# xmengli/H-DenseUNet

Hardware: AMD Instinct MI355X
Metric: CT slices/sec fwd+bwd (2D 512^2) (higher is better)
Workload: dtype bf16

## Files before the change

h-denseunet_amd/csrc/rowops.hip:

```cpp
#include "hdu_host.h"

enum { RED_STATS = 0, RED_BNBWD = 1, RED_COLSUM = 2 };
enum { ROW_UNROLL = 4 };

struct FinK {
  int kind;
  const float* shift_f32;
  const float* gamma; const float* beta; const float* sgamma; const float* sbeta;
  float eps, momentum, invM;
  int batch_stats;
  float* a; float* b; float* rstd; float* mov_mean; float* mov_var;
  const float* rstd_in;
  float* k1; float* k2; float* k3; float* dgamma; float* dbeta; float* dsgamma; float* dsbeta;
  const float* mean_in; float* corr3; float* corr4;
  int skip_lo, skip_hi;
};

__device__ __forceinline__ void fin_reduce32(double& a1, double& a2, double (*red)[4][8]) {
  const int cl = threadIdx.x & 7, wave = threadIdx.x >> 6;
#pragma unroll
  for (int mask = 8; mask < 64; mask <<= 1) {
    a1 += __shfl_xor(a1, mask);
    a2 += __shfl_xor(a2, mask);
  }
// ... 37 lines not shown
  const float sg = sgamma ? sgamma[c] : 1.f;
  const float sb = sbeta ? sbeta[c] : 0.f;
  const float inv = g * r;
  *a = sg * inv;
  *b = sg * (be - mu * inv) + sb;
  *r_out = r;
}

__device__ __forceinline__ void bn_fold_channel(int c, float mu, float v, const float* gamma, const float* beta,
                                                float eps, const float* sgamma, const float* sbeta, float* a, float* b,
                                                float* rstd, float* mov_mean, float* mov_var, float momentum) {
  float ac, bc, r;
  bn_fold_coef(c, mu, v, gamma, beta, eps, sgamma, sbeta, &ac, &bc, &r);
  a[c] = ac;
  b[c] = bc;
  if (rstd) rstd[c] = r;
  if (mov_mean) mov_mean[c] -= (mov_mean[c] - mu) * (1.f - momentum);
  if (mov_var) mov_var[c] -= (mov_var[c] - v) * (1.f - momentum);
}

__device__ __forceinline__ void bn_coef_channel(int c, float invM, int batch_stats, float S1, float S2,
                                                const float* gamma, const float* beta, const float* sgamma,
                                                const float* rstd, float* k1, float* k2, float* k3, float* dgamma,
                                                float* dbeta, float* dsgamma, float* dsbeta) {
  const float g = gamma ? gamma[c] : 1.f;
  const float be = beta ? beta[c] : 0.f;
  const float sg = sgamma ? sgamma[c] : 1.f;
  const float r = rstd[c];
  const float kk = sg * g * r;
  k1[c] = kk;
  k2[c] = batch_stats ? kk * S1 * invM : 0.f;
  k3[c] = batch_stats ? kk * r * S2 * invM : 0.f;
  if (dgamma) dgamma[c] = sg * S2;
  if (dbeta) dbeta[c] = sg * S1;
  if (dsgamma) dsgamma[c] = g * S2 + be * S1;
  if (dsbeta) dsbeta[c] = S1;
}

template <typename T, int MODE>
__device__ __forceinline__ void finalize_channel(int c, double a1, double a2, long long M, const void* x, float* o1,
                                                 float* o2, const FinK& fin, const FinPre& pre) {
  if (MODE == 0) {
    const double shift = fin.shift_f32 ? (double)fin.shift_f32[c] : (double)Chunk<T>::load1((const T*)x + c);
    const double m1 = a1 / (double)M;
    double var = a2 / (double)M - m1 * m1;
    if (var < 0.0) var = 0.0;
    o1[c] = (float)(shift + m1);
    o2[c] = (float)var;
    if (fin.kind == 1) bn_fold_channel_pre(c, (float)(shift + m1), (float)var, fin, pre);
  } else {
    if (o1) o1[c] = (float)a1;
    if (o2) o2[c] = (float)a2;
    if (MODE == 1 && (fin.kind == 2 || fin.kind == 3)) {
      const float S1 = (float)a1, S2 = (float)a2;
      const float kk = pre.sg * pre.g * pre.rs;
      const float k2 = fin.batch_stats ? kk * S1 * fin.invM : 0.f;
      const float k3 = fin.batch_stats ? kk * pre.rs * S2 * fin.invM : 0.f;
      if (fin.dgamma) fin.dgamma[c] = pre.sg * S2;
      if (fin.dbeta) fin.dbeta[c] = pre.sg * S1;
      if (fin.dsgamma) fin.dsgamma[c] = pre.g * S2 + pre.be * S1;
      if (fin.dsbeta) fin.dsbeta[c] = S1;
      if (fin.kind == 2) {
        fin.k1[c] = kk; fin.k2[c] = k2; fin.k3[c] = k3;
      } else if (fin.batch_stats && !(c >= fin.skip_lo && c < fin.skip_hi)) {
        fin.corr3[c] += k3;
        fin.corr4[c] += k3 * pre.mu - k2;
      }
    }
  }
}

struct RedK {
  const void* x;
  const void* dz;
  long long ldx, lddz, M, rows_per_block;
  int C;
  int relu;
  const float* a;
  const float* b;
  const float* mean;
  const float* rstd;
  float* partial;
  int slots;
};

template <typename T, int MODE, int COLS>
__global__ __launch_bounds__(256) void reduce_rows_kernel(RedK p) {
  constexpr int CH = Chunk<T>::CH;
  constexpr int ROWS = 256 / COLS;
  __shared__ float red[2][ROWS][COLS * CH];
  const int tid = threadIdx.x;
  const int cc = tid % COLS;
  const int rl = tid / COLS;
  const int c0 = (blockIdx.y * COLS + cc) * CH;
  const bool active = c0 < p.C;
  const T* __restrict__ xp = (const T*)p.x;
  const T* __restrict__ dzp = (const T*)p.dz;

  float s1[CH], s2[CH], k0[CH], k1[CH], k2[CH], k3[CH];
#pragma unroll
  for (int j = 0; j < CH; ++j) { s1[j] = 0.f; s2[j] = 0.f; k0[j] = 0.f; k1[j] = 0.f; k2[j] = 0.f; k3[j] = 0.f; }
  if (active) {
    if (MODE == RED_STATS) {
      Chunk<T>::unpack(*(const u32x4*)(xp + c0), k0);
    } else if (MODE == RED_BNBWD) {
#pragma unroll
      for (int j = 0; j < CH; ++j) {
        k0[j] = p.a[c0 + j]; k1[j] = p.b[c0 + j]; k2[j] = p.mean[c0 + j]; k3[j] = p.rstd[c0 + j];
      }
    }
    const long long r_begin = (long long)blockIdx.x * p.rows_per_block;
    long long r_end = r_begin + p.rows_per_block;
    if (r_end > p.M) r_end = p.M;
    auto body = [&](const u32x4& xv, const u32x4& gv) {
      float f[CH];
      Chunk<T>::unpack(xv, f);
      if (MODE == RED_STATS) {
#pragma unroll
        for (int j = 0; j < CH; ++j) { const float d = f[j] - k0[j]; s1[j] += d; s2[j] += d * d; }
      } else if (MODE == RED_BNBWD) {
        float g[CH];
        Chunk<T>::unpack(gv, g);
#pragma unroll
        for (int j = 0; j < CH; ++j) {
          const float s = k0[j] * f[j] + k1[j];
          const float gg = (!p.relu || s > 0.f) ? g[j] : 0.f;
          s1[j] += gg;
          s2[j] += gg * ((f[j] - k2[j]) * k3[j]);
        }
      } else {
#pragma unroll
        for (int j = 0; j < CH; ++j) s1[j] += f[j];
      }
    };
    long long r = r_begin + rl;
    for (; r + (ROW_UNROLL - 1) * ROWS < r_end; r += ROW_UNROLL * ROWS) {
      u32x4 xv[ROW_UNROLL], gv[ROW_UNROLL];
#pragma unroll
      for (int u = 0; u < ROW_UNROLL; ++u) xv[u] = *(const u32x4*)(xp + (r + u * ROWS) * p.ldx + c0);
      if (MODE == RED_BNBWD) {
#pragma unroll
        for (int u = 0; u < ROW_UNROLL; ++u) gv[u] = *(const u32x4*)(dzp + (r + u * ROWS) * p.lddz + c0);
      }
      HDU_SCHED_BARRIER();
#pragma unroll
      for (int u = 0; u < ROW_UNROLL; ++u) body(xv[u], gv[u]);
    }
    for (; r < r_end; r += ROWS) {
      u32x4 gv = u32x4{0u, 0u, 0u, 0u};
      if (MODE == RED_BNBWD) gv = *(const u32x4*)(dzp + r * p.lddz + c0);
      body(*(const u32x4*)(xp + r * p.ldx + c0), gv);
    }
  }
#pragma unroll
  for (int j = 0; j < CH; ++j) { red[0][rl][cc * CH + j] = s1[j]; red[1][rl][cc * CH + j] = s2[j]; }
  __syncthreads();
  for (int q = tid; q < 2 * COLS * CH; q += 256) {
    const int s = q / (COLS * CH);
    const int col = q % (COLS * CH);
    const int c = blockIdx.y * COLS * CH + col;
    if (c < p.C) {
      float t = 0.f;
#pragma unroll 4
      for (int r = 0; r < ROWS; ++r) t += red[s][r][col];
      if (p.slots > 0) atomicAdd(p.partial + ((long long)(blockIdx.x % (unsigned)p.slots) * 2 + s) * p.C + c, t);
      else p.partial[((long long)blockIdx.x * 2 + s) * p.C + c] = t;
    }
  }
}

template <typename T, int MODE>
__global__ __launch_bounds__(256) void reduce_finalize_kernel(const float* __restrict__ partial, int nblk, int C,
                                                              long long M, const void* x, float* __restrict__ o1,
                                                              float* __restrict__ o2, FinK fin) {
  __shared__ double red[2][4][8];
  const int cl = threadIdx.x & 7, pl = threadIdx.x >> 3;
  const int c = blockIdx.x * 8 + cl;
  const FinPre pre = fin_prefetch(fin, c < C ? c : 0, pl == 0 && c < C && fin.kind != 0);
  double a1 = 0.0, a2 = 0.0;
  if (c < C) {
    int b = pl;
    for (; b + 7 * 32 < nblk; b += 8 * 32) {
      float v1[8], v2[8];
#pragma unroll
      for (int u = 0; u < 8; ++u) {
        v1[u] = partial[((long long)(b + u * 32) * 2 + 0) * C + c];
        v2[u] = MODE != RED_COLSUM ? partial[((long long)(b + u * 32) * 2 + 1) * C + c] : 0.f;
      }
      HDU_SCHED_BARRIER();
#pragma unroll
      for (int u = 0; u < 8; ++u) { a1 += (double)v1[u]; a2 += (double)v2[u]; }
    }
    for (; b < nblk; b += 32) {
      a1 += (double)partial[((long long)b * 2 + 0) * C + c];
      if (MODE != RED_COLSUM) a2 += (double)partial[((long long)b * 2 + 1) * C + c];
    }
  }
  fin_reduce32(a1, a2, red);
  if (pl == 0 && c < C) finalize_channel<T, MODE>(c, a1, a2, M, x, o1, o2, fin, pre);
}

static int red_cols_for(int nchunks) {
  int cols = 4;
  while (cols < nchunks && cols < 32) cols <<= 1;
  return cols;
}
static void red_geometry(int dtype, long long M, int C, int* cols, unsigned* gx, unsigned* gy, long long* rpb) {
  const int ch = dtype == HDU_BF16 ? 8 : 4;
  const int nchunks = (C + ch - 1) / ch;
  *cols = red_cols_for(nchunks);
  *gy = (unsigned)((nchunks + *cols - 1) / *cols);
  const int rows = 256 / *cols;
  long long want = (g_tuning[HDU_TUNE_RED_WGS] > 0 ? g_tuning[HDU_TUNE_RED_WGS] : 512) / *gy;
  if (want < 1) want = 1;
  long long maxb = (M + (long long)rows * 4 - 1) / ((long long)rows * 4);
  if (maxb < 1) maxb = 1;
  if (want > maxb) want = maxb;
  *rpb = (M + want - 1) / want;
  if (*rpb < 1) *rpb = 1;
  *gx = (unsigned)((M + *rpb - 1) / *rpb);
  if (*gx < 1) *gx = 1;
}

extern "C" size_t hdu_reduce_ws_bytes(int64_t M, int C) {
  size_t best = 0;
  for (int dt = 0; dt < 2; ++dt) {
    int cols; unsigned gx, gy; long long rpb;
    red_geometry(dt, M, C, &cols, &gx, &gy, &rpb);
    size_t b = (size_t)gx * 2 * (size_t)C * sizeof(float);
    if (b > best) best = b;
  }
  return best + 256;
}

template <typename T, int MODE>
static int run_reduce(RedK k, int cols, unsigned gx, unsigned gy, hipStream_t s) {
  switch (cols) {
    case 4: HDU_LAUNCH((reduce_rows_kernel<T, MODE, 4>), dim3(gx, gy), dim3(256), 0, s, k); break;
    case 8: HDU_LAUNCH((reduce_rows_kernel<T, MODE, 8>), dim3(gx, gy), dim3(256), 0, s, k); break;
    case 16: HDU_LAUNCH((reduce_rows_kernel<T, MODE, 16>), dim3(gx, gy), dim3(256), 0, s, k); break;
    default: HDU_LAUNCH((reduce_rows_kernel<T, MODE, 32>), dim3(gx, gy), dim3(256), 0, s, k); break;
  }
  return 0;
}

template <int MODE>
static int reduce_entry(int dtype, RedK k, float* o1, float* o2, void* ws, size_t ws_bytes, hipStream_t s,
                        const char* what, FinK fin = FinK{}) {
  if (dtype != HDU_BF16 && dtype != HDU_F32) return hdu_set_error(HDU_ERR_ARG, "reduce: bad dtype");
  const int ch = dtype == HDU_BF16 ? 8 : 4;
  if (k.C <= 0 || k.C % ch || k.ldx % ch || (k.dz && k.lddz % ch))
    return hdu_set_error(HDU_ERR_ARG, "reduce: C and pixel strides must be multiples of the 16-byte chunk");
  if (k.M <= 0) return hdu_set_error(HDU_ERR_ARG, "reduce: M must be positive");
  int cols; unsigned gx, gy; long long rpb;
  red_geometry(dtype, k.M, k.C, &cols, &gx, &gy, &rpb);
  if (!ws || ws_bytes < (size_t)gx * 2 * (size_t)k.C * sizeof(float))
    return hdu_set_error(HDU_ERR_WORKSPACE, "reduce: workspace too small (see hdu_reduce_ws_bytes)");
  k.rows_per_block = rpb;
  k.partial = (float*)ws;
  const unsigned fb = (unsigned)((k.C + 7) / 8);
  if (dtype == HDU_BF16) {
    run_reduce<bf16_t, MODE>(k, cols, gx, gy, s);
    HDU_LAUNCH((reduce_finalize_kernel<bf16_t, MODE>), dim3(fb), dim3(256), 0, s, (const float*)ws, (int)gx, k.C,
               k.M, k.x, o1, o2, fin);
  } else {
    run_reduce<float, MODE>(k, cols, gx, gy, s);
    HDU_LAUNCH((reduce_finalize_kernel<float, MODE>), dim3(fb), dim3(256), 0, s, (const float*)ws, (int)gx, k.C, k.M,
               k.x, o1, o2, fin);
  }
  return hdu_check_launch(what);
}

extern "C" int hdu_bn_stats(int dtype, const void* x, int64_t ldx, int64_t M, int C, float* mean, float* var,
                            void* ws, size_t ws_bytes, void* stream) {
  if (!x || !mean || !var) return hdu_set_error(HDU_ERR_ARG, "bn_stats: null pointer");
  RedK k{};
  k.x = x; k.ldx = ldx; k.M = M; k.C = C;
  return reduce_entry<RED_STATS>(dtype, k, mean, var, ws, ws_bytes, (hipStream_t)stream, "bn_stats");
}

extern "C" int hdu_bn_stats_fold(int dtype, const void* x, int64_t ldx, int64_t M, int C, float* mean, float* var,
                                 const float* gamma, const float* beta, float eps, const float* sgamma,
                                 const float* sbeta, float* a, float* b, float* rstd, float* mov_mean, float* mov_var,
                                 float momentum, void* ws, size_t ws_bytes, void* stream) {
  if (!x || !mean || !var || !a || !b) return hdu_set_error(HDU_ERR_ARG, "bn_stats_fold: null pointer");
  RedK k{};
  k.x = x; k.ldx = ldx; k.M = M; k.C = C;
  FinK f{};
  f.kind = 1; f.gamma = gamma; f.beta = beta; f.sgamma = sgamma; f.sbeta = sbeta; f.eps = eps; f.momentum = momentum;
  f.a = a; f.b = b; f.rstd = rstd; f.mov_mean = mov_mean; f.mov_var = mov_var;
  return reduce_entry<RED_STATS>(dtype, k, mean, var, ws, ws_bytes, (hipStream_t)stream, "bn_stats_fold", f);
}

extern "C" int hdu_bn_stats_finalize(const float* partial, int slots, int64_t M, int C, const float* shift, float* mean,
                                     float* var, const float* gamma, const float* beta, float eps, const float* sgamma,
                                     const float* sbeta, float* a, float* b, float* rstd, float* mov_mean, float* mov_var,
                                     float momentum, void* stream) {
  if (!partial || slots <= 0 || M <= 0 || C <= 0 || !shift || !mean || !var || ((a == nullptr) != (b == nullptr)))
    return hdu_set_error(HDU_ERR_ARG, "bn_stats_finalize: bad args");
  FinK f{};
  f.shift_f32 = shift;
  if (a) {
    f.kind = 1; f.gamma = gamma; f.beta = beta; f.sgamma = sgamma; f.sbeta = sbeta; f.eps = eps; f.momentum = momentum;
    f.a = a; f.b = b; f.rstd = rstd; f.mov_mean = mov_mean; f.mov_var = mov_var;
  }
  HDU_LAUNCH((reduce_finalize_kernel<float, RED_STATS>), dim3((unsigned)((C + 7) / 8)), dim3(256), 0, (hipStream_t)stream,
             partial, slots, C, (long long)M, (const void*)nullptr, mean, var, f);
  return hdu_check_launch("bn_stats_finalize");
}

__global__ __launch_bounds__(256) void finalize_fold_next_kernel(const float* __restrict__ partial, int slots, int Cseg,
                                                                 int seg_c0, int C_all, long long M,
                                                                 const float* __restrict__ shift_all,
                                                                 float* __restrict__ mean_all, float* __restrict__ var_all,
                                                                 FinK fin) {
  __shared__ double red[2][4][8];
  const int cl = threadIdx.x & 7, pl = threadIdx.x >> 3;
  const int c = blockIdx.x * 8 + cl;
  const bool in_seg = c >= seg_c0 && c < seg_c0 + Cseg;
  const bool wg_has_seg = (int)blockIdx.x * 8 + 7 >= seg_c0 && (int)blockIdx.x * 8 < seg_c0 + Cseg;
  const bool mine = pl == 0 && c < C_all;
  const FinPre pre = fin_prefetch(fin, mine ? c : 0, mine);
  const float mean_old = mine ? (in_seg ? shift_all[c] : mean_all[c]) : 0.f;
  const float var_old = mine ? var_all[c] : 0.f;
// ... 88 lines not shown
                          size_t ws_bytes, void* stream) {
  if (!x || !out) return hdu_set_error(HDU_ERR_ARG, "colsum: null pointer");
  RedK k{};
  k.x = x; k.ldx = ldx; k.M = M; k.C = C;
  return reduce_entry<RED_COLSUM>(dtype, k, out, nullptr, ws, ws_bytes, (hipStream_t)stream, "colsum");
}

__global__ __launch_bounds__(256) void bn_fold_kernel(int C, const float* mean, const float* var, const float* gamma,
                                                      const float* beta, float eps, const float* sgamma,
                                                      const float* sbeta, float* a, float* b, float* rstd,
                                                      float* mov_mean, float* mov_var, float momentum) {
  const int c = blockIdx.x * blockDim.x + threadIdx.x;
  if (c >= C) return;
  bn_fold_channel(c, mean[c], var[c], gamma, beta, eps, sgamma, sbeta, a, b, rstd, mov_mean, mov_var, momentum);
}

extern "C" int hdu_bn_fold(int C, const float* mean, const float* var, const float* gamma, const float* beta,
                           float eps, const float* sgamma, const float* sbeta, float* a, float* b, float* rstd,
                           float* mov_mean, float* mov_var, float momentum, void* stream) {
  if (C <= 0 || !mean || !var || !a || !b) return hdu_set_error(HDU_ERR_ARG, "bn_fold: bad args");
  HDU_LAUNCH(bn_fold_kernel, dim3((unsigned)((C + 255) / 256)), dim3(256), 0, (hipStream_t)stream, C, mean, var,
             gamma, beta, eps, sgamma, sbeta, a, b, rstd, mov_mean, mov_var, momentum);
  return hdu_check_launch("bn_fold");
}

__global__ __launch_bounds__(256) void bn_fold_batched_kernel(const hdu_fold_entry* __restrict__ table,
                                                              const unsigned* __restrict__ begins, int n) {
  int lo = 0, hi = n - 1;
  while (lo < hi) {
    const int mid = (lo + hi + 1) >> 1;
    if (begins[mid] <= blockIdx.x) lo = mid; else hi = mid - 1;
  }
  const hdu_fold_entry e = table[lo];
  const int c = (int)(blockIdx.x - begins[lo]) * 256 + (int)threadIdx.x;
  if (c >= e.C) return;
  bn_fold_channel(c, e.mean[c], e.var[c], e.gamma, e.beta, e.eps, e.sgamma, e.sbeta, e.a, e.b, e.rstd, nullptr, nullptr,
                  0.f);
}

extern "C" int hdu_bn_fold_batched(const hdu_fold_entry* table, const uint32_t* begins, int n, uint32_t total_blocks,
                                   void* stream) {
  if (!table || !begins || n <= 0 || total_blocks == 0) return hdu_set_error(HDU_ERR_ARG, "bn_fold_batched: bad args");
  HDU_LAUNCH(bn_fold_batched_kernel, dim3(total_blocks), dim3(256), 0, (hipStream_t)stream, table, begins, n);
  return hdu_check_launch("bn_fold_batched");
}

__global__ __launch_bounds__(256) void bn_bwd_finalize_batched_kernel(const hdu_bnbwd_entry* __restrict__ table,
                                                                      const unsigned* __restrict__ begins, int n) {
  __shared__ double red[2][4][8];
  int lo = 0, hi = n - 1;
  while (lo < hi) {
    const int mid = (lo + hi + 1) >> 1;
    if (begins[mid] <= blockIdx.x) lo = mid; else hi = mid - 1;
  }
  const hdu_bnbwd_entry e = table[lo];
  const int cl = threadIdx.x & 7, pl = threadIdx.x >> 3;
  const int c = (int)(blockIdx.x - begins[lo]) * 8 + cl;
  const bool mine = pl == 0 && c < e.C;
  const float g = (mine && e.gamma) ? e.gamma[c] : 1.f, be = (mine && e.beta) ? e.beta[c] : 0.f;
  const float sg = (mine && e.sgamma) ? e.sgamma[c] : 1.f;
  double a1 = 0.0, a2 = 0.0;
  if (c < e.C) {
    for (int b = pl; b < e.slots; b += 32) {
      a1 += (double)e.partial[((long long)b * 2 + 0) * e.C + c];
      a2 += (double)e.partial[((long long)b * 2 + 1) * e.C + c];
    }
  }
  fin_reduce32(a1, a2, red);
  if (!mine) return;
  const float S1 = (float)a1, S2 = (float)a2;
  if (e.dgamma) e.dgamma[c] = sg * S2;
  if (e.dbeta) e.dbeta[c] = sg * S1;
  if (e.dsgamma) e.dsgamma[c] = g * S2 + be * S1;
  if (e.dsbeta) e.dsbeta[c] = S1;
}

extern "C" int hdu_bn_bwd_finalize_batched(const hdu_bnbwd_entry* table, const uint32_t* begins, int n, uint32_t total_blocks,
                                           void* stream) {
  if (!table || !begins || n <= 0 || total_blocks == 0) return hdu_set_error(HDU_ERR_ARG, "bn_bwd_finalize_batched: bad args");
  HDU_LAUNCH(bn_bwd_finalize_batched_kernel, dim3(total_blocks), dim3(256), 0, (hipStream_t)stream, table, begins, n);
  return hdu_check_launch("bn_bwd_finalize_batched");
}

__global__ __launch_bounds__(256) void bn_bwd_coef_kernel(int C, float invM, int batch_stats, const float* s1,
                                                          const float* s2, const float* gamma, const float* beta,
                                                          const float* sgamma, const float* rstd, float* k1,
                                                          float* k2, float* k3, float* dgamma, float* dbeta,
                                                          float* dsgamma, float* dsbeta) {
  const int c = blockIdx.x * blockDim.x + threadIdx.x;
  if (c >= C) return;
  bn_coef_channel(c, invM, batch_stats, s1 ? s1[c] : 0.f, s2 ? s2[c] : 0.f, gamma, beta, sgamma, rstd, k1, k2, k3,
                  dgamma, dbeta, dsgamma, dsbeta);
}

extern "C" int hdu_bn_bwd_coef(int C, int64_t M, int batch_stats, const float* s1, const float* s2,
                               const float* gamma, const float* beta, const float* sgamma, const float* rstd,
                               float* k1, float* k2, float* k3, float* dgamma, float* dbeta, float* dsgamma,
                               float* dsbeta, void* stream) {
  if (C <= 0 || M <= 0 || !rstd || !k1 || !k2 || !k3) return hdu_set_error(HDU_ERR_ARG, "bn_bwd_coef: bad args");
  if (batch_stats && (!s1 || !s2)) return hdu_set_error(HDU_ERR_ARG, "bn_bwd_coef: batch_stats needs s1/s2");
  HDU_LAUNCH(bn_bwd_coef_kernel, dim3((unsigned)((C + 255) / 256)), dim3(256), 0, (hipStream_t)stream, C,
             1.0f / (float)M, batch_stats, s1, s2, gamma, beta, sgamma, rstd, k1, k2, k3, dgamma, dbeta, dsgamma,
             dsbeta);
  return hdu_check_launch("bn_bwd_coef");
}

__global__ __launch_bounds__(256) void stats_pack_kernel(int C, const float* mean, const float* var, float n_local, int rank,
                                                         int world, float* buf) {
  const int c = blockIdx.x * blockDim.x + threadIdx.x;
  const int SL = 1 + 2 * C;
  if (c >= C) return;
  for (int r = 0; r < world; ++r) {
    const bool mine = r == rank;
    if (c == 0) buf[r * SL] = mine ? n_local : 0.f;
    buf[r * SL + 1 + c] = mine ? mean[c] : 0.f;
    buf[r * SL + 1 + C + c] = mine ? var[c] : 0.f;
  }
}
__global__ __launch_bounds__(256) void stats_unpack_kernel(int C, const float* buf, int world, float* mean, float* var) {
  const int c = blockIdx.x * blockDim.x + threadIdx.x;
  const int SL = 1 + 2 * C;
  if (c >= C) return;
  float N = 0.f, m = 0.f;
  for (int r = 0; r < world; ++r) { N += buf[r * SL]; m += buf[r * SL] * buf[r * SL + 1 + c]; }
  m /= N;
  float v = 0.f;
  for (int r = 0; r < world; ++r) {
    const float d = buf[r * SL + 1 + c] - m;
    v += buf[r * SL] * (buf[r * SL + 1 + C + c] + d * d);
  }
  mean[c] = m;
  var[c] = v / N;
}
extern "C" size_t hdu_stats_sync_floats(int C, int world) { return (size_t)world * (1 + 2 * (size_t)C); }
extern "C" int hdu_stats_pack(int C, const float* mean, const float* var, int64_t n_local, int rank, int world, float* buf,
                              void* stream) {
  if (C <= 0 || !mean || !var || !buf || n_local <= 0 || world <= 0 || rank < 0 || rank >= world)
    return hdu_set_error(HDU_ERR_ARG, "stats_pack: bad args");
  HDU_LAUNCH(stats_pack_kernel, dim3((unsigned)((C + 255) / 256)), dim3(256), 0, (hipStream_t)stream, C, mean, var,
             (float)n_local, rank, world, buf);
  return hdu_check_launch("stats_pack");
}
extern "C" int hdu_stats_unpack(int C, const float* buf, int world, float* mean, float* var, void* stream) {
  if (C <= 0 || !mean || !var || !buf || world <= 0) return hdu_set_error(HDU_ERR_ARG, "stats_unpack: bad args");
  HDU_LAUNCH(stats_unpack_kernel, dim3((unsigned)((C + 255) / 256)), dim3(256), 0, (hipStream_t)stream, C, buf, world, mean,
             var);
  return hdu_check_launch("stats_unpack");
}

struct RowK {
  const void* x;
  const void* dz;
  void* out;
  long long ldx, lddz, ldo, M, rows_per_block;
  int C;
  int relu, accumulate;
  const float* a;
  const float* b;
  const float* mean;
  const float* k1;
  const float* k2;
  const float* k3;
  float drop_scale;
  unsigned drop_thresh, drop_seed;
  const unsigned* drop_seed_dev;
  const float* sums;
  int slots, batch_stats;
  float invM;
  const float* gamma; const float* beta; const float* sgamma; const float* rstd;
  float* dgamma; float* dbeta; float* dsgamma; float* dsbeta;
};

template <int CH, int COLS>
__device__ __forceinline__ void slot_loads(const float* __restrict__ tbl, int slots, int C, int c0, bool active, int rl,
                                           float (&t1)[CH], float (&t2)[CH]) {
  constexpr int ROWS = 256 / COLS;
  constexpr int IT = 4;
  f32x4 v1[IT][CH / 4], v2[IT][CH / 4];
#pragma unroll
  for (int it = 0; it < IT; ++it) {
    const int sl = rl + it * ROWS;
    const long long row = (active && sl < slots) ? sl : 0;
#pragma unroll
    for (int j = 0; j < CH; j += 4) {
      v1[it][j / 4] = *(const f32x4*)(tbl + (row * 2 + 0) * C + c0 + j);
      v2[it][j / 4] = *(const f32x4*)(tbl + (row * 2 + 1) * C + c0 + j);
    }
  }
#pragma unroll
  for (int j = 0; j < CH; ++j) { t1[j] = 0.f; t2[j] = 0.f; }
#pragma unroll
  for (int it = 0; it < IT; ++it) {
    const bool ok = active && rl + it * ROWS < slots;
#pragma unroll
    for (int j = 0; j < CH; ++j) {
      t1[j] += ok ? v1[it][j / 4][j % 4] : 0.f;
      t2[j] += ok ? v2[it][j / 4][j % 4] : 0.f;
    }
  }
}
template <int CH, int COLS>
__device__ __forceinline__ void slot_reduce(int slots, int cc, int rl, const float (&t1)[CH], const float (&t2)[CH],
                                            float (&s1)[CH], float (&s2)[CH]) {
  constexpr int ROWS = 256 / COLS;
  __shared__ float red[ROWS][2][COLS * CH];
#pragma unroll
  for (int j = 0; j < CH; ++j) { red[rl][0][cc * CH + j] = t1[j]; red[rl][1][cc * CH + j] = t2[j]; }
  HDU_RAW_BARRIER();
  const int nr = slots < ROWS ? slots : ROWS;
#pragma unroll
  for (int j = 0; j < CH; ++j) { s1[j] = 0.f; s2[j] = 0.f; }
  for (int r = 0; r < nr; ++r) {
#pragma unroll
    for (int j = 0; j < CH; ++j) { s1[j] += red[r][0][cc * CH + j]; s2[j] += red[r][1][cc * CH + j]; }
  }
}

template <typename T, int COLS>
__global__ __launch_bounds__(256) void affine_act_kernel(RowK p) {
  constexpr int CH = Chunk<T>::CH;
  constexpr int ROWS = 256 / COLS;
  const int cc = threadIdx.x % COLS, rl = threadIdx.x / COLS;
  const int c0 = (blockIdx.y * COLS + cc) * CH;
  if (c0 >= p.C) return;
  const T* __restrict__ xp = (const T*)p.x;
  T* __restrict__ op = (T*)p.out;
  float a[CH], b[CH];
#pragma unroll
  for (int j = 0; j < CH; ++j) { a[j] = p.a ? p.a[c0 + j] : 1.f; b[j] = p.a ? p.b[c0 + j] : 0.f; }
  const long long r_begin = (long long)blockIdx.x * p.rows_per_block;
  long long r_end = r_begin + p.rows_per_block;
  if (r_end > p.M) r_end = p.M;
  auto body = [&](long long m, const u32x4& xv) {
    float f[CH];
    Chunk<T>::unpack(xv, f);
#pragma unroll
    for (int j = 0; j < CH; ++j) {
      float s = a[j] * f[j] + b[j];
      if (p.relu) s = s > 0.f ? s : 0.f;
      f[j] = s;
    }
    *(u32x4*)(op + m * p.ldo + c0) = Chunk<T>::pack(f);
  };
  long long m = r_begin + rl;
  for (; m + (ROW_UNROLL - 1) * ROWS < r_end; m += ROW_UNROLL * ROWS) {
    u32x4 xv[ROW_UNROLL];
#pragma unroll
    for (int u = 0; u < ROW_UNROLL; ++u) xv[u] = *(const u32x4*)(xp + (m + u * ROWS) * p.ldx + c0);
    HDU_SCHED_BARRIER();
#pragma unroll
    for (int u = 0; u < ROW_UNROLL; ++u) body(m + u * ROWS, xv[u]);
  }
  for (; m < r_end; m += ROWS) body(m, *(const u32x4*)(xp + m * p.ldx + c0));
}

template <typename T, int COLS, bool SUMS = false, bool PRE = false>
__global__ __launch_bounds__(256) void bn_bwd_apply_kernel(RowK p) {
  constexpr int CH = Chunk<T>::CH;
  constexpr int ROWS = 256 / COLS;
  const int cc = threadIdx.x % COLS, rl = threadIdx.x / COLS;
  const int c0 = (blockIdx.y * COLS + cc) * CH;
  const bool active = c0 < p.C;
  if (!SUMS && !active) return;
  const T* __restrict__ xp = (const T*)p.x;
  const T* __restrict__ dzp = (const T*)p.dz;
  T* __restrict__ op = (T*)p.out;
  const unsigned dseed = p.drop_seed + (p.drop_seed_dev ? *p.drop_seed_dev : 0u);
  const long long r_begin = (long long)blockIdx.x * p.rows_per_block;
  long long r_end = r_begin + p.rows_per_block;
  if (r_end > p.M) r_end = p.M;
  const u32x4 z4 = u32x4{0u, 0u, 0u, 0u};
  long long m = r_begin + rl;
  u32x4 pxv[PRE ? ROW_UNROLL : 1], pgv[PRE ? ROW_UNROLL : 1], pov[PRE ? ROW_UNROLL : 1];
  if constexpr (PRE) {
#pragma unroll
    for (int u = 0; u < ROW_UNROLL; ++u) {
      const long long mm = m + u * ROWS;
      const bool ok = active && mm < r_end;
      pxv[u] = ok ? *(const u32x4*)(xp + mm * p.ldx + c0) : z4;
      pgv[u] = ok ? *(const u32x4*)(dzp + mm * p.lddz + c0) : z4;
      pov[u] = (ok && p.accumulate) ? *(const u32x4*)(op + mm * p.ldo + c0) : z4;
    }
  }
  float a[CH], b[CH], k1[CH], k3[CH], k4[CH];
  if constexpr (SUMS) {
    const int cq = active ? c0 : 0;
    float g[CH], be[CH], sg[CH], rs[CH], mu[CH];
#pragma unroll
    for (int j = 0; j < CH; j += 4) {
      const f32x4 va = *(const f32x4*)(p.a + cq + j), vb = *(const f32x4*)(p.b + cq + j);
      const f32x4 vr = *(const f32x4*)(p.rstd + cq + j), vm = *(const f32x4*)(p.mean + cq + j);
      const f32x4 vg = p.gamma ? *(const f32x4*)(p.gamma + cq + j) : f32x4{1.f, 1.f, 1.f, 1.f};
      const f32x4 ve = p.beta ? *(const f32x4*)(p.beta + cq + j) : f32x4{0.f, 0.f, 0.f, 0.f};
      const f32x4 vs = p.sgamma ? *(const f32x4*)(p.sgamma + cq + j) : f32x4{1.f, 1.f, 1.f, 1.f};
#pragma unroll
      for (int r = 0; r < 4; ++r) {
        a[j + r] = va[r]; b[j + r] = vb[r]; rs[j + r] = vr[r]; mu[j + r] = vm[r];
        g[j + r] = vg[r]; be[j + r] = ve[r]; sg[j + r] = vs[r];
      }
    }
    float T1[CH], T2[CH], S1[CH], S2[CH];
    slot_loads<CH, COLS>(p.sums, p.slots, p.C, cq, active, rl, T1, T2);
    slot_reduce<CH, COLS>(p.slots, cc, rl, T1, T2, S1, S2);
    if (!active) return;
#pragma unroll
    for (int j = 0; j < CH; ++j) {
      const float kk = sg[j] * g[j] * rs[j];
      const float k2 = p.batch_stats ? kk * S1[j] * p.invM : 0.f;
      k1[j] = kk;
      k3[j] = p.batch_stats ? kk * rs[j] * S2[j] * p.invM : 0.f;
      k4[j] = k3[j] * mu[j] - k2;
    }
    if (blockIdx.x == 0 && rl == 0) {
#pragma unroll
      for (int j = 0; j < CH; ++j) {
        const int c = c0 + j;
        if (p.dgamma) p.dgamma[c] = sg[j] * S2[j];
        if (p.dbeta) p.dbeta[c] = sg[j] * S1[j];
        if (p.dsgamma) p.dsgamma[c] = g[j] * S2[j] + be[j] * S1[j];
        if (p.dsbeta) p.dsbeta[c] = S1[j];
      }
    }
  } else {
#pragma unroll
    for (int j = 0; j < CH; ++j) {
      const int c = c0 + j;
      a[j] = p.a[c]; b[j] = p.b[c]; k1[j] = p.k1[c]; k3[j] = p.k3[c];
      k4[j] = p.k3[c] * p.mean[c] - p.k2[c];
    }
  }
  auto body = [&](long long m, const u32x4& xv, const u32x4& gv, const u32x4& ov) {
    float f[CH], g[CH], o[CH];
    Chunk<T>::unpack(xv, f);
    Chunk<T>::unpack(gv, g);
#pragma unroll
    for (int j = 0; j < CH; ++j) {
      const float s = a[j] * f[j] + b[j];
      const float gg = (!p.relu || s > 0.f) ? g[j] : 0.f;
      float d = k1[j] * gg - k3[j] * f[j] + k4[j];
      if (p.drop_scale != 0.f) {
        const unsigned h = hdu_hash32((unsigned long long)m * (unsigned)p.C + (unsigned)(c0 + j), dseed);
        d = h < p.drop_thresh ? d * p.drop_scale : 0.f;
      }
      o[j] = d;
    }
    if (p.accumulate) {
      float old[CH];
      Chunk<T>::unpack(ov, old);
#pragma unroll
      for (int j = 0; j < CH; ++j) o[j] += old[j];
    }
    *(u32x4*)(op + m * p.ldo + c0) = Chunk<T>::pack(o);
  };
  if constexpr (PRE) {
#pragma unroll
    for (int u = 0; u < ROW_UNROLL; ++u)
      if (m + u * ROWS < r_end) body(m + u * ROWS, pxv[u], pgv[u], pov[u]);
    return;
  }
  for (; m + (ROW_UNROLL - 1) * ROWS < r_end; m += ROW_UNROLL * ROWS) {
    u32x4 xv[ROW_UNROLL], gv[ROW_UNROLL], ov[ROW_UNROLL];
#pragma unroll
    for (int u = 0; u < ROW_UNROLL; ++u) xv[u] = *(const u32x4*)(xp + (m + u * ROWS) * p.ldx + c0);
#pragma unroll
    for (int u = 0; u < ROW_UNROLL; ++u) gv[u] = *(const u32x4*)(dzp + (m + u * ROWS) * p.lddz + c0);
#pragma unroll
    for (int u = 0; u < ROW_UNROLL; ++u) ov[u] = p.accumulate ? *(const u32x4*)(op + (m + u * ROWS) * p.ldo + c0) : z4;
    HDU_SCHED_BARRIER();
#pragma unroll
    for (int u = 0; u < ROW_UNROLL; ++u) body(m + u * ROWS, xv[u], gv[u], ov[u]);
  }
  for (; m < r_end; m += ROWS)
    body(m, *(const u32x4*)(xp + m * p.ldx + c0), *(const u32x4*)(dzp + m * p.lddz + c0),
         p.accumulate ? *(const u32x4*)(op + m * p.ldo + c0) : z4);
}

template <typename T, int COLS>
__global__ __launch_bounds__(256) void bn_bwd_correct_kernel(RowK p) {
  constexpr int CH = Chunk<T>::CH;
  constexpr int ROWS = 256 / COLS;
  const int cc = threadIdx.x % COLS, rl = threadIdx.x / COLS;
  const int c0 = (blockIdx.y * COLS + cc) * CH;
  if (c0 >= p.C) return;
  const T* __restrict__ xp = (const T*)p.x;
  T* __restrict__ op = (T*)p.out;
  float k3[CH], k4[CH];
#pragma unroll
  for (int j = 0; j < CH; ++j) { k3[j] = p.k3[c0 + j]; k4[j] = p.k2[c0 + j]; }
  const long long r_begin = (long long)blockIdx.x * p.rows_per_block;
  long long r_end = r_begin + p.rows_per_block;
  if (r_end > p.M) r_end = p.M;
  auto body = [&](long long m, const u32x4& xv, const u32x4& ov) {
    float f[CH], o[CH];
    Chunk<T>::unpack(xv, f);
    Chunk<T>::unpack(ov, o);
#pragma unroll
    for (int j = 0; j < CH; ++j) o[j] += k4[j] - k3[j] * f[j];
    *(u32x4*)(op + m * p.ldo + c0) = Chunk<T>::pack(o);
  };
  long long m = r_begin + rl;
  for (; m + (ROW_UNROLL - 1) * ROWS < r_end; m += ROW_UNROLL * ROWS) {
    u32x4 xv[ROW_UNROLL], ov[ROW_UNROLL];
#pragma unroll
    for (int u = 0; u < ROW_UNROLL; ++u) xv[u] = *(const u32x4*)(xp + (m + u * ROWS) * p.ldx + c0);
#pragma unroll
    for (int u = 0; u < ROW_UNROLL; ++u) ov[u] = *(const u32x4*)(op + (m + u * ROWS) * p.ldo + c0);
    HDU_SCHED_BARRIER();
#pragma unroll
    for (int u = 0; u < ROW_UNROLL; ++u) body(m + u * ROWS, xv[u], ov[u]);
  }
  for (; m < r_end; m += ROWS) body(m, *(const u32x4*)(xp + m * p.ldx + c0), *(const u32x4*)(op + m * p.ldo + c0));
}

struct FinCorK {
  const float* partial; int slots; int C; long long M;
  FinK fin;
  int nfin;
  int cs0, Cc;
  const void* u; void* du; long long ldu, lddu, rows_per_block;
};

template <typename T>
__global__ __launch_bounds__(256) void bn_bwd_finalize_correct_kernel(FinCorK p) {
  constexpr int CH = Chunk<T>::CH;
  __shared__ double red[2][4][8];
  __shared__ float slotv[32][8][2 * CH];
  __shared__ float tot[8][2 * CH];
  if ((int)blockIdx.x < p.nfin) {
    if (blockIdx.y != 0) return;
    const int cl = threadIdx.x & 7, pl = threadIdx.x >> 3;
    const int c = blockIdx.x * 8 + cl;
    const FinPre pre = fin_prefetch(p.fin, c < p.C ? c : 0, pl == 0 && c < p.C);
    double a1 = 0.0, a2 = 0.0;
    if (c < p.C)
      for (int b = pl; b < p.slots; b += 32) {
        a1 += (double)p.partial[((long long)b * 2 + 0) * p.C + c];
        a2 += (double)p.partial[((long long)b * 2 + 1) * p.C + c];
      }
    fin_reduce32(a1, a2, red);
    if (pl == 0 && c < p.C) finalize_channel<float, RED_BNBWD>(c, a1, a2, p.M, nullptr, nullptr, nullptr, p.fin, pre);
    return;
  }
  const int cc = threadIdx.x & 7, rl = threadIdx.x >> 3;
  const int c0 = (blockIdx.y * 8 + cc) * CH;
  const bool active = c0 < p.Cc;
  const int cb = p.cs0 + (active ? c0 : 0);
  {
    float v[2 * CH];
#pragma unroll
    for (int j = 0; j < 2 * CH; ++j) v[j] = 0.f;
    if (active && rl < p.slots) {
#pragma unroll
      for (int j = 0; j < CH; j += 4) {
        const f32x4 q1 = *(const f32x4*)(p.partial + ((long long)rl * 2 + 0) * p.C + cb + j);
        const f32x4 q2 = *(const f32x4*)(p.partial + ((long long)rl * 2 + 1) * p.C + cb + j);
#pragma unroll
        for (int r = 0; r < 4; ++r) { v[j + r] = q1[r]; v[CH + j + r] = q2[r]; }
// ... 283 lines not shown
  const int ch = dtype == HDU_BF16 ? 8 : 4;
  if (!x || !out || ((a == nullptr) != (b == nullptr)) || ((ud | uh | uw) & ~1))
    return hdu_set_error(HDU_ERR_ARG, "materialize: bad pointers / upsample shifts");
  if (C <= 0 || C % ch || ldx % ch || ldout % ch || (skip && ldskip % ch) || N <= 0 || D <= 0 || H <= 0 || W <= 0)
    return hdu_set_error(HDU_ERR_ARG, "materialize: C / strides must be multiples of the 16-byte chunk");
  MatK k{};
  k.x = x; k.skip = skip; k.out = out; k.a = a; k.b = b; k.ldx = ldx; k.ldskip = ldskip; k.ldo = ldout;
  k.N = N; k.D = D; k.H = H; k.W = W; k.C = C; k.ud = ud; k.uh = uh; k.uw = uw; k.relu = relu;
  k.Mo = (long long)N * (D << ud) * (H << uh) * (W << uw);
  int cols; unsigned gx, gy;
  row_geometry(dtype, k.Mo, C, &cols, &gx, &gy, &k.rows_per_block);
  if (dtype == HDU_BF16) { HDU_ROW_LAUNCH(materialize_kernel, bf16_t, cols, gx, gy, stream, k); }
  else { HDU_ROW_LAUNCH(materialize_kernel, float, cols, gx, gy, stream, k); }
  return hdu_check_launch("materialize");
}

extern "C" int hdu_materialize_stats(int dtype, const void* x, int64_t ldx, int N, int D, int H, int W, int C,
                                     const hdu_stats_fold_desc* f, int relu, int ud, int uh, int uw, const void* skip,
                                     int64_t ldskip, void* out, int64_t ldout, void* stream) {
  if (dtype != HDU_BF16 && dtype != HDU_F32) return hdu_set_error(HDU_ERR_ARG, "materialize_stats: bad dtype");
  const int ch = dtype == HDU_BF16 ? 8 : 4;
  if (!x || !out || !f || ((ud | uh | uw) & ~1)) return hdu_set_error(HDU_ERR_ARG, "materialize_stats: bad pointers / upsample shifts");
  if (C <= 0 || C % ch || ldx % ch || ldout % ch || (skip && ldskip % ch) || N <= 0 || D <= 0 || H <= 0 || W <= 0)
    return hdu_set_error(HDU_ERR_ARG, "materialize_stats: C / strides must be multiples of the 16-byte chunk");
  if (!f->partial || f->slots <= 0 || f->slots > 32 || f->M <= 0 || f->Cseg <= 0 || f->Cseg % ch || f->seg_c0 < 0 ||
      f->seg_c0 % ch || f->seg_c0 + f->Cseg > C || !f->shift || !f->mean || !f->var || !f->a || !f->b)
    return hdu_set_error(HDU_ERR_ARG, "materialize_stats: bad statistics block (segment bounds are multiples of the 16-byte chunk)");
  if (((uintptr_t)f->partial | (uintptr_t)f->shift | (uintptr_t)f->mean | (uintptr_t)f->var | (uintptr_t)f->gamma |
       (uintptr_t)f->beta | (uintptr_t)f->sgamma | (uintptr_t)f->sbeta | (uintptr_t)f->mov_mean | (uintptr_t)f->mov_var) & 15)
    return hdu_set_error(HDU_ERR_ARG, "materialize_stats: per-channel vectors must be 16-byte aligned");
  MatK k{};
  k.x = x; k.skip = skip; k.out = out; k.ldx = ldx; k.ldskip = ldskip; k.ldo = ldout;
  k.N = N; k.D = D; k.H = H; k.W = W; k.C = C; k.ud = ud; k.uh = uh; k.uw = uw; k.relu = relu;
  k.Mo = (long long)N * (D << ud) * (H << uh) * (W << uw);
  k.st_partial = f->partial; k.st_slots = f->slots; k.Cseg = f->Cseg; k.seg_c0 = f->seg_c0; k.st_M = f->M;
  k.st_shift = f->shift; k.st_mean = f->mean; k.st_var = f->var;
  k.gamma = f->gamma; k.beta = f->beta; k.sgamma = f->sgamma; k.sbeta = f->sbeta; k.eps = f->eps; k.momentum = f->momentum;
  k.fa = f->a; k.fb = f->b; k.frstd = f->rstd; k.mov_mean = f->mov_mean; k.mov_var = f->mov_var;
  int cols; unsigned gx, gy;
  row_geometry(dtype, k.Mo, C, &cols, &gx, &gy, &k.rows_per_block);
  const bool pre = k.rows_per_block <= (long long)ROW_UNROLL * (256 / cols) && !(ud | uh | uw) && skip == nullptr &&
                   !(g_tuning[HDU_TUNE_DEBUG] & 2048);
#define HDU_MAT_STATS(T, PRE)                                                                                                   \
  switch (cols) {                                                                                                               \
    case 4: HDU_LAUNCH((materialize_kernel<T, 4, true, PRE>), dim3(gx, gy), dim3(256), 0, (hipStream_t)stream, k); break;       \
    case 8: HDU_LAUNCH((materialize_kernel<T, 8, true, PRE>), dim3(gx, gy), dim3(256), 0, (hipStream_t)stream, k); break;       \
    case 16: HDU_LAUNCH((materialize_kernel<T, 16, true, PRE>), dim3(gx, gy), dim3(256), 0, (hipStream_t)stream, k); break;     \
    default: HDU_LAUNCH((materialize_kernel<T, 32, true, PRE>), dim3(gx, gy), dim3(256), 0, (hipStream_t)stream, k); break;     \
  }
  if (dtype == HDU_BF16) { if (pre) { HDU_MAT_STATS(bf16_t, true) } else { HDU_MAT_STATS(bf16_t, false) } }
  else { if (pre) { HDU_MAT_STATS(float, true) } else { HDU_MAT_STATS(float, false) } }
#undef HDU_MAT_STATS
  return hdu_check_launch("materialize_stats");
}

extern "C" int hdu_bn_bwd_apply(int dtype, const void* dz, int64_t lddz, const void* x, int64_t ldx, int64_t M,
                                int C, const float* a, const float* b, int relu, const float* mean, const float* k1,
                                const float* k2, const float* k3, void* dx, int64_t lddx, int accumulate,
                                float drop_keep, uint32_t drop_seed, const uint32_t* drop_seed_dev, void* stream) {
  RowK k{};
  k.x = x; k.ldx = ldx; k.dz = dz; k.lddz = lddz; k.out = dx; k.ldo = lddx; k.M = M; k.C = C;
  k.a = a; k.b = b; k.relu = relu; k.mean = mean; k.k1 = k1; k.k2 = k2; k.k3 = k3; k.accumulate = accumulate;
  if (drop_keep > 0.f && drop_keep < 1.f) {
    k.drop_scale = 1.f / drop_keep;
    k.drop_thresh = (unsigned)((double)drop_keep * 4294967296.0);
  }
  k.drop_seed = drop_seed;
  k.drop_seed_dev = drop_seed_dev;
  if (!x || !dz || !dx || !a || !b || !mean || !k1 || !k2 || !k3) return hdu_set_error(HDU_ERR_ARG, "bn_bwd_apply: null pointer");
  if (int e = rowk_check(dtype, k, "bn_bwd_apply: C / strides must be multiples of the 16-byte chunk")) return e;
  if (M == 0) return 0;
  int cols; unsigned gx, gy;
  row_geometry(dtype, M, C, &cols, &gx, &gy, &k.rows_per_block);
  if (dtype == HDU_BF16) { HDU_ROW_LAUNCH(bn_bwd_apply_kernel, bf16_t, cols, gx, gy, stream, k); }
  else { HDU_ROW_LAUNCH(bn_bwd_apply_kernel, float, cols, gx, gy, stream, k); }
  return hdu_check_launch("bn_bwd_apply");
}

static int bn_bwd_fused_impl(bool reduce, int dtype, const void* dz, int64_t lddz, const void* x, int64_t ldx, int64_t M, int C,
                             const float* a, const float* b, int relu, const float* mean, const float* rstd,
                             int batch_stats, const float* gamma, const float* beta, const float* sgamma, float* sums,
                             int slots, float* dgamma, float* dbeta, float* dsgamma, float* dsbeta, void* dx,
                             int64_t lddx, int accumulate, float drop_keep, uint32_t drop_seed,
                             const uint32_t* drop_seed_dev, void* stream) {
  if (!dz || !x || !a || !b || !mean || !rstd || !sums || !dx) return hdu_set_error(HDU_ERR_ARG, "bn_bwd_fused: null pointer");
  if (slots <= 0 || slots > 32) return hdu_set_error(HDU_ERR_ARG, "bn_bwd_fused: 1 <= slots <= 32");
  if (((uintptr_t)sums | (uintptr_t)a | (uintptr_t)b | (uintptr_t)mean | (uintptr_t)rstd | (uintptr_t)gamma | (uintptr_t)beta |
       (uintptr_t)sgamma) & 15)
    return hdu_set_error(HDU_ERR_ARG, "bn_bwd_fused: per-channel vectors must be 16-byte aligned");
  RowK k{};
  k.x = x; k.ldx = ldx; k.dz = dz; k.lddz = lddz; k.out = dx; k.ldo = lddx; k.M = M; k.C = C;
  k.a = a; k.b = b; k.relu = relu; k.mean = mean; k.accumulate = accumulate;
  if (drop_keep > 0.f && drop_keep < 1.f) {
    k.drop_scale = 1.f / drop_keep;
    k.drop_thresh = (unsigned)((double)drop_keep * 4294967296.0);
  }
  k.drop_seed = drop_seed;
  k.drop_seed_dev = drop_seed_dev;
  k.sums = sums; k.slots = slots; k.batch_stats = batch_stats; k.invM = 1.0f / (float)M;
  k.gamma = gamma; k.beta = beta; k.sgamma = sgamma; k.rstd = rstd;
  k.dgamma = dgamma; k.dbeta = dbeta; k.dsgamma = dsgamma; k.dsbeta = dsbeta;
  if (int e = rowk_check(dtype, k, "bn_bwd_fused: C / strides must be multiples of the 16-byte chunk")) return e;
  if (M == 0) return 0;
  if (reduce) {
    RedK r{};
    r.x = x; r.ldx = ldx; r.dz = dz; r.lddz = lddz; r.M = M; r.C = C;
    r.a = a; r.b = b; r.mean = mean; r.rstd = rstd; r.relu = relu;
    r.partial = sums; r.slots = slots;
    int rcols; unsigned rgx, rgy;
    red_geometry(dtype, M, C, &rcols, &rgx, &rgy, &r.rows_per_block);
    if (dtype == HDU_BF16) run_reduce<bf16_t, RED_BNBWD>(r, rcols, rgx, rgy, (hipStream_t)stream);
    else run_reduce<float, RED_BNBWD>(r, rcols, rgx, rgy, (hipStream_t)stream);
  }
  int cols; unsigned gx, gy;
  row_geometry(dtype, M, C, &cols, &gx, &gy, &k.rows_per_block);
  const bool pre = k.rows_per_block <= (long long)ROW_UNROLL * (256 / cols) && !(g_tuning[HDU_TUNE_DEBUG] & 2048);
#define HDU_APPLY_SUMS(T, PRE)                                                                                                    \
  switch (cols) {                                                                                                                 \
    case 4: HDU_LAUNCH((bn_bwd_apply_kernel<T, 4, true, PRE>), dim3(gx, gy), dim3(256), 0, (hipStream_t)stream, k); break;        \
    case 8: HDU_LAUNCH((bn_bwd_apply_kernel<T, 8, true, PRE>), dim3(gx, gy), dim3(256), 0, (hipStream_t)stream, k); break;        \
    case 16: HDU_LAUNCH((bn_bwd_apply_kernel<T, 16, true, PRE>), dim3(gx, gy), dim3(256), 0, (hipStream_t)stream, k); break;      \
    default: HDU_LAUNCH((bn_bwd_apply_kernel<T, 32, true, PRE>), dim3(gx, gy), dim3(256), 0, (hipStream_t)stream, k); break;      \
  }
  if (dtype == HDU_BF16) { if (pre) { HDU_APPLY_SUMS(bf16_t, true) } else { HDU_APPLY_SUMS(bf16_t, false) } }
  else { if (pre) { HDU_APPLY_SUMS(float, true) } else { HDU_APPLY_SUMS(float, false) } }
#undef HDU_APPLY_SUMS
  return hdu_check_launch("bn_bwd_fused");
}

extern "C" int hdu_bn_bwd_fused(int dtype, const void* dz, int64_t lddz, const void* x, int64_t ldx, int64_t M, int C,
                                const float* a, const float* b, int relu, const float* mean, const float* rstd,
                                int batch_stats, const float* gamma, const float* beta, const float* sgamma, float* sums,
                                int slots, float* dgamma, float* dbeta, float* dsgamma, float* dsbeta, void* dx,
                                int64_t lddx, int accumulate, float drop_keep, uint32_t drop_seed,
                                const uint32_t* drop_seed_dev, void* stream) {
  return bn_bwd_fused_impl(true, dtype, dz, lddz, x, ldx, M, C, a, b, relu, mean, rstd, batch_stats, gamma, beta, sgamma, sums, slots,
                           dgamma, dbeta, dsgamma, dsbeta, dx, lddx, accumulate, drop_keep, drop_seed, drop_seed_dev, stream);
}

extern "C" int hdu_bn_bwd_apply_sums(int dtype, const void* dz, int64_t lddz, const void* x, int64_t ldx, int64_t M, int C,
                                     const float* a, const float* b, int relu, const float* mean, const float* rstd,
                                     int batch_stats, const float* gamma, const float* beta, const float* sgamma, float* sums,
                                     int slots, float* dgamma, float* dbeta, float* dsgamma, float* dsbeta, void* dx,
                                     int64_t lddx, int accumulate, float drop_keep, uint32_t drop_seed,
                                     const uint32_t* drop_seed_dev, void* stream) {
  return bn_bwd_fused_impl(false, dtype, dz, lddz, x, ldx, M, C, a, b, relu, mean, rstd, batch_stats, gamma, beta, sgamma, sums, slots,
                           dgamma, dbeta, dsgamma, dsbeta, dx, lddx, accumulate, drop_keep, drop_seed, drop_seed_dev, stream);
}

extern "C" int hdu_bn_bwd_correct(int dtype, const void* u, int64_t ldu, int64_t M, int C, const float* corr3,
                                  const float* corr4, void* du, int64_t lddu, void* stream) {
  RowK k{};
  k.x = u; k.ldx = ldu; k.out = du; k.ldo = lddu; k.M = M; k.C = C;
  k.k3 = corr3; k.k2 = corr4;
  if (!u || !du || !corr3 || !corr4) return hdu_set_error(HDU_ERR_ARG, "bn_bwd_correct: null pointer");
  if (int e = rowk_check(dtype, k, "bn_bwd_correct: C / strides must be multiples of the 16-byte chunk")) return e;
  if (M == 0) return 0;
  int cols; unsigned gx, gy;
  row_geometry(dtype, M, C, &cols, &gx, &gy, &k.rows_per_block);
  if (dtype == HDU_BF16) { HDU_ROW_LAUNCH(bn_bwd_correct_kernel, bf16_t, cols, gx, gy, stream, k); }
  else { HDU_ROW_LAUNCH(bn_bwd_correct_kernel, float, cols, gx, gy, stream, k); }
  return hdu_check_launch("bn_bwd_correct");
}

extern "C" int hdu_bn_bwd_finalize_correct(int dtype, const float* partial, int slots, int64_t M, int C, const float* gamma,
                                           const float* beta, const float* sgamma, const float* mean, const float* rstd,
                                           float* dgamma, float* dbeta, float* dsgamma, float* dsbeta, float* corr3, float* corr4,
                                           int cs0, int Cc, const void* u, int64_t ldu, void* du, int64_t lddu, void* stream) {
  const int ch = dtype == HDU_BF16 ? 8 : 4;
  if ((dtype != HDU_BF16 && dtype != HDU_F32) || !partial || slots <= 0 || slots > 32 || M <= 0 || C <= 0 || !rstd || !mean || !corr3 ||
      !corr4 || !u || !du || cs0 < 0 || Cc <= 0 || cs0 + Cc > C || cs0 % ch || Cc % ch || C % 4 || ldu % ch || lddu % ch ||
      ((uintptr_t)u | (uintptr_t)du | (uintptr_t)partial) % 16)
    return hdu_set_error(HDU_ERR_ARG, "bn_bwd_finalize_correct: bad args (corrected channels inside the BN's, chunk-aligned; <= 32 slots)");
  FinCorK k{};
  k.partial = partial; k.slots = slots; k.C = C; k.M = M;
  k.fin.kind = 3; k.fin.gamma = gamma; k.fin.beta = beta; k.fin.sgamma = sgamma; k.fin.rstd_in = rstd; k.fin.invM = 1.0f / (float)M;
  k.fin.batch_stats = 1; k.fin.dgamma = dgamma; k.fin.dbeta = dbeta; k.fin.dsgamma = dsgamma; k.fin.dsbeta = dsbeta;
  k.fin.mean_in = mean; k.fin.corr3 = corr3; k.fin.corr4 = corr4; k.fin.skip_lo = cs0; k.fin.skip_hi = cs0 + Cc;
  k.nfin = (C + 7) / 8;
  k.cs0 = cs0; k.Cc = Cc; k.u = u; k.du = du; k.ldu = ldu; k.lddu = lddu;
  const unsigned gy = (unsigned)((Cc / ch + 7) / 8);
  long long want = (g_tuning[HDU_TUNE_ROW_WGS] > 0 ? g_tuning[HDU_TUNE_ROW_WGS] : 512) / gy;
  long long maxb = (M + 127) / 128;
  if (want > maxb) want = maxb;
  if (want < 1) want = 1;
  k.rows_per_block = (M + want - 1) / want;
  const unsigned gxc = (unsigned)((M + k.rows_per_block - 1) / k.rows_per_block);
  if (dtype == HDU_BF16) HDU_LAUNCH((bn_bwd_finalize_correct_kernel<bf16_t>), dim3((unsigned)k.nfin + gxc, gy), dim3(256), 0, (hipStream_t)stream, k);
  else HDU_LAUNCH((bn_bwd_finalize_correct_kernel<float>), dim3((unsigned)k.nfin + gxc, gy), dim3(256), 0, (hipStream_t)stream, k);
  return hdu_check_launch("bn_bwd_finalize_correct");
}

struct PoolK {
  const void* x;
  const void* dy;
  void* out;
  unsigned char* idx;
  long long ldx, lddy, ldo;
  int N, D, H, W, C;
  int Do, Ho, Wo;
  int accumulate;
  int ud, uh, uw;
  int pad_d;
};

template <typename T>
__global__ __launch_bounds__(256) void maxpool_fwd_kernel(PoolK p) {
  constexpr int CH = Chunk<T>::CH;
  const int ncc = p.C / CH;
  const long long total = (long long)p.N * p.Do * p.Ho * p.Wo * ncc;
  const T* __restrict__ xp = (const T*)p.x;
  T* __restrict__ op = (T*)p.out;
  const int kdn = p.D == 1 ? 1 : 3, pdd = p.D == 1 ? 0 : p.pad_d, sdd = p.D == 1 ? 1 : 2;
  for (long long q = (long long)blockIdx.x * blockDim.x + threadIdx.x; q < total;
       q += (long long)gridDim.x * blockDim.x) {
    const int c0 = (int)(q % ncc) * CH;
    long long t = q / ncc;
    const long long opix = t;
    const int ow = (int)(t % p.Wo); t /= p.Wo;
    const int oh = (int)(t % p.Ho); t /= p.Ho;
    const int od = (int)(t % p.Do);
    const int n = (int)(t / p.Do);
    float best[CH];
    int bi[CH];
    bool any_pad = false;
#pragma unroll
    for (int j = 0; j < CH; ++j) { best[j] = -3.0e38f; bi[j] = 255; }
    for (int kd = 0; kd < kdn; ++kd) {
      const int id = od * sdd - pdd + kd;
      for (int kh = 0; kh < 3; ++kh) {
// ... 752 lines not shown
```

h-denseunet_amd/engine.py:

```python
import ctypes
import math
import os
from collections import OrderedDict

import numpy as np
import torch

from . import ops
from . import shard as _sh
from .lib import HDU_BF16, HDU_F32


class Param:
    __slots__ = ("layer", "idx", "kind", "keras_shape", "shape", "trainable", "init", "offset", "numel", "ctx", "meta")

    def __init__(self, ctx, layer, idx, kind, keras_shape, shape, trainable, init, meta=None):
        self.ctx, self.layer, self.idx, self.kind = ctx, layer, idx, kind
        self.keras_shape, self.shape, self.trainable, self.init = tuple(keras_shape), tuple(shape), trainable, init
        self.numel = int(np.prod(shape))
        self.offset = None
        self.meta = meta or {}

    @property
    def data(self):
        return self.ctx.P[self.offset:self.offset + self.numel]

    @property
    def grad(self):
        return self.ctx.G[self.offset:self.offset + self.numel]


class Var:

    def __init__(self, ctx, act, root=None, c0=0):
        self.ctx, self.act, self.c0 = ctx, act, c0
        self.root = root or self
        if root is None:
            self.grad_act = None
            self.written = False
            self.mean = None
            self.var = None
            self.shift = None
            self.needs_grad = False
            self.drop = None
            self.corr_off = None
        self.C = act.C

    def slab(self, c0, C):
        return Var(self.ctx, self.act.slab(c0, C), self.root, self.c0 + c0)

    def require_grad(self):
        r = self.root
        if not r.needs_grad:
            r.needs_grad = True
            a = r.act
            r.grad_act = ops.Act.alloc(a.N, a.D, a.H, a.W, a.ld, a.dtype, zero=True)
        return self

    @property
    def grad(self):
        return self.root.grad_act.slab(self.c0, self.C)

    def dy(self):
        r = self.root
        ctx = self.ctx
        if r.corr_off is not None and ctx.corr_acc is not None and ctx.fuse_bn_bwd_now:
            pend = ctx._pending_fin
            ch = ops.CHUNK[self.act.dtype]
            aligned = (self.c0 - (pend["c0"] if pend else 0)) % ch == 0 and self.C % ch == 0 and self.act.ld % ch == 0 \
                and self.grad.ld % ch == 0 and self.act.ptr.value % 16 == 0 and self.grad.ptr.value % 16 == 0
            if pend is not None and pend["root"] is r and pend["c0"] <= self.c0 and self.c0 + self.C <= pend["c0"] + pend["C"] \
                    and self.act.M == pend["M"] and aligned:
                ctx._pending_fin = None
                ops.bn_bwd_finalize_correct(*pend["args"], self.c0 - pend["c0"], self.act, self.grad)
                return self.grad
            ctx.flush_pending_finalize()
            ld = r.act.ld
            base = r.corr_off + self.c0
            acc = ctx.corr_acc
            ops.bn_bwd_correct(self.act, acc[base:base + self.C], acc[base + ld:base + ld + self.C], self.grad)
        return self.grad

    def grad_mode(self):
        r = self.root
        acc = r.written
        if not acc:
            assert self.c0 == 0, "first gradient write into a shared buffer must start at channel 0"
            if self.C != r.act.ld:
                self.ctx.zero_partial_grad(r.grad_act.buf)
        r.written = True
        return acc

    def stats(self):
        r = self.root
        if r.mean is None:
            dev = ops.device()
            r.mean = torch.zeros(r.act.ld, dtype=torch.float32, device=dev)
            r.var = torch.ones(r.act.ld, dtype=torch.float32, device=dev)
            r.shift = torch.zeros(r.act.ld, dtype=torch.float32, device=dev)
            r.ctx.stat_roots.append(r)
        return r.mean[self.c0:self.c0 + self.C], r.var[self.c0:self.c0 + self.C]

    def stats_shift(self):
        self.stats()
        return self.root.shift[self.c0:self.c0 + self.C]


class _BwdList(list):

    def __init__(self, ctx):
        super().__init__()
        self._ctx = ctx
        self.mark = []

    def append(self, fn):
        super().append(fn)
        self.mark.append(len(self._ctx.params))


class Ctx:

    def __init__(self, dtype, batch_shape):
        self.dtype = dtype
        self.ch = ops.CHUNK[dtype]
        self.params = []
        self.by_layer = OrderedDict()
        self.layer_kind = OrderedDict()
        self.fwd = []
        self.bwd = _BwdList(self)
        self.vars = []
        self.learning_phase = 1
        self.pass_id = 0
        self.P = self.G = self.V = None
        self.n_trainable = 0
        self.convs = []
        self.bns = []
        self._fold_plans = {}
        self._prefolded_phase = None
        self.prefolded_pass = -1
        self.batch_fold = os.environ.get("HDU_BATCH_FOLD", "1") == "1"
        self.defer_bnb_finalize = os.environ.get("HDU_DEFER_BNB_FINALIZE", "1") == "1"
        self._bnb_deferred, self._bnb_plan = [], None
        self._pending_fin = None
        self.merge_fin_correct = os.environ.get("HDU_MERGE_FIN_CORRECT", "1") == "1"
        self.absorb_stats = os.environ.get("HDU_ABSORB_STATS", "1") == "1"
        self.bn_bwd_fused = os.environ.get("HDU_BN_BWD_FUSED", "1") == "1"
        self.fuse_bn_bwd_mode = int(os.environ.get("HDU_FUSE_BN_BWD", "1"))
        self.fuse_bn_bwd = self.fuse_bn_bwd_mode > 0
        self.fuse_bn_bwd_pw = os.environ.get("HDU_FUSE_BN_BWD_PW", "1") == "1"
        self.bnb_sums_epilogue = os.environ.get("HDU_BNB_SUMS_EPILOGUE", "1") == "1"
        self.fuse_bn_bwd_now = False
        self.bnb_sinks = []
        self.bnb_acc = None
        self.corr_acc = None
        self._corr_total = 0
        self._scratch = {}
        self.ws_bytes = 1 << 16
        self.ws = None
        self.dev = ops.device()
        self.seed_dev = torch.zeros(1, dtype=torch.int32, device=self.dev)
        self.drop_layers = 0
        self.dropout_enabled = True
        self.grad_enabled = True
        self.fuse_bn_epilogue = os.environ.get("HDU_FUSE_BN_EPILOGUE", "1") == "1"
        self.fuse_bn_epilogue_train = os.environ.get("HDU_FUSE_BN_EPILOGUE_TRAIN", "1") == "1"
        self.fold_next = os.environ.get("HDU_FOLD_NEXT", "1") == "1"
        self.shard = None
        self.fuse_prologue = os.environ.get("HDU_FUSE_PROLOGUE", "0") == "1"
        self.fuse_pw = os.environ.get("HDU_FUSE_PW", "1") == "1"
        self.batch_wgrad = os.environ.get("HDU_BATCH_WGRAD", "1") == "1"
        self.wgrad_plan = None
        self.split_wgrad = os.environ.get("HDU_F32_SPLIT_WGRAD", "1") == "1"
        self._split_plan = None
        self._split_now = False
        self.epilogue_stats = os.environ.get("HDU_EPILOGUE_STATS", "1") == "1"
        self.stats_sinks = []
        self.stat_roots = []
        self.stats_acc = None
        self.finalized = False
        self.arena = None
        self.loss_layers = []
        self._grad_zero = []
        self._grad_zero_ids = set()
        self._zp_arena = self._zp_bwd = self._zp_step = None
        self._zp_keep = []
        self._zeroed_fwd_pass = -1
        self._zeroed_bwd_pass = -1
        self._zeroed_grad_pass = -1

    def add_param(self, layer, kind, idx, keras_shape, shape, trainable, init, meta=None):
        p = Param(self, layer, idx, kind, keras_shape, shape, trainable, init, meta)
        self.params.append(p)
        self.by_layer.setdefault(layer, []).append(p)
        self.layer_kind[layer] = kind
        return p

    def need_ws(self, M, C):
        self.ws_bytes = max(self.ws_bytes, ops.reduce_ws_bytes(M, C))

    def scratch(self, slot, N, D, H, W, C):
        n = N * D * H * W * C
        ent = self._scratch.setdefault(slot, {"n": 0, "buf": None})
        ent["n"] = max(ent["n"], n)
        return lambda: ops.Act(ent["buf"], 0, N, D, H, W, C, C, self.dtype)

    def new_var(self, N, D, H, W, C, ld=None):
        v = Var(self, ops.Act.alloc(N, D, H, W, C, self.dtype, ld=ld, zero=True))
        self.vars.append(v)
        return v

    def fvec(self, C, fill=0.0):
        return torch.full((C,), fill, dtype=torch.float32, device=self.dev)

    def finalize(self, seed=4321):
        order = [p for p in self.params if p.trainable] + [p for p in self.params if not p.trainable]
        off = 0
        for p in order:
            p.offset = off
            off += (p.numel + 3) // 4 * 4
            if p.trainable:
                self.n_trainable = off
        self.P = torch.zeros(off, dtype=torch.float32, device=self.dev)
        self.G = torch.zeros(off, dtype=torch.float32, device=self.dev)
        self.V = torch.zeros(max(self.n_trainable, 4), dtype=torch.float32, device=self.dev)
        self.ws = ops.Workspace(self.ws_bytes)
        tdt = torch.bfloat16 if self.dtype == HDU_BF16 else torch.float32
        for ent in self._scratch.values():
            ent["buf"] = torch.zeros(ent["n"], dtype=tdt, device=self.dev)
        tot = 0
        for cv in self.convs:
            cv.wf_off = tot
            tot += cv.kernel.numel
            if cv.need_dgrad_filter:
                cv.wd_off = tot
                tot += cv.kernel.numel
        self.Wc = torch.zeros(max(tot, 8), dtype=tdt, device=self.dev)
        self.init_weights(seed)
        n_stats = 0
        for st in self.stats_sinks:
            st.acc_off = n_stats
            n_stats += st.SLOTS * 2 * st.var.C
        n_bnb = 0
        for cv in self.convs:
            if cv.bnb_fused:
                cv.bnb_off = n_bnb
                n_bnb += cv.BNB_SLOTS * 2 * cv.bn.C
                r = cv.x.root
                if cv.bn.mode == "batch" and r.corr_off is None:
                    r.corr_off = self._corr_total
                    self._corr_total += 2 * r.act.ld
        n_bsum = 0
        bsum_off = {}
        if self.bn_bwd_fused and self.grad_enabled:
            for bn in self.bns:
                if bn.mode == "batch" or bn.any_trainable():
                    bsum_off[bn] = n_bsum
                    n_bsum += bn.BSUM_SLOTS * 2 * bn.C
        up4 = lambda n: (n + 3) // 4 * 4
        o_loss, n_loss = 0, 4 * max(1, len(self.loss_layers))
        o_stats = o_loss + n_loss
        o_bnb = o_stats + up4(n_stats)
        o_corr = o_bnb + up4(n_bnb)
        o_bsum = o_corr + up4(self._corr_total)
        total = o_bsum + up4(n_bsum)
        self.arena = torch.zeros(total, dtype=torch.float32, device=self.dev)
        for i, ll in enumerate(self.loss_layers):
            ll.loss_sum = self.arena[4 * i:4 * i + 1]
            ll.class_count = self.arena[4 * i + 1:4 * i + 4]
        self.stats_acc = self.arena[o_stats:o_stats + n_stats] if n_stats else None
        self.bnb_acc = self.arena[o_bnb:o_bnb + n_bnb] if n_bnb else None
        self.corr_acc = self.arena[o_corr:o_corr + self._corr_total] if self._corr_total else None
        for bn, o in bsum_off.items():
            bn.bsum = self.arena[o_bsum + o:o_bsum + o + bn.BSUM_SLOTS * 2 * bn.C]
        self._shift_copies = [(r.shift, r.mean) for r in self.stat_roots] if self.stats_sinks else []
        self._zp_arena = ops.ZeroPlan([self.arena], self._shift_copies)
        self._zp_bwd = ops.ZeroPlan([self.arena[o_bnb:total]]) if total > o_bnb else None
        for cv in self.convs:
            cv.bind()
        self._build_prep_table()
        self._build_wgrad_plan()
        self.finalized = True

    def _build_wgrad_plan(self):
        self.wgrad_plan = None
        for cv in self.convs:
            cv.in_plan = False
        if not (self.batch_wgrad and self.dtype == HDU_BF16 and self.grad_enabled and
                (self.shard is None or self.shard.world == 1)):
            return
        plan = ops.WgradPlan(int(os.environ.get("HDU_BATCH_WGRAD_TARGET", "0")))
        for cv in self.convs:
            if not (cv.trainable and cv.out.root.needs_grad):
                continue
            if cv.xin is not None:
                d = self.conv_desc(cv.xin.act, cv.wf_ptr, cv.out.grad, cv.K, cv.stride, cv.pad, cv.conv_up)
            elif cv.bn is None and cv.skip is None:
                d = self.conv_desc(cv.x.act, cv.wf_ptr, cv.out.grad, cv.K, cv.stride, cv.pad, cv.up)
            elif cv.pw_fused:
                d = self.conv_desc(cv.x.act, cv.wf_ptr, cv.out.grad, cv.K, cv.stride, cv.pad, cv.up, None,
                                  (cv.bn.a, cv.bn.b), cv.bn.relu)
            else:
                continue
            if ops.conv_kernel_name(d, 1) == "conv_stem_wgrad_kernel":
                continue
            plan.add(d, cv.kernel.grad)
            cv.in_plan = True
        if len(plan):
            plan.finalize()
            self.wgrad_plan = plan

    def split_wgrad_active(self):
        return bool(self.dtype == HDU_F32 and self.split_wgrad and self.batch_wgrad and self.grad_enabled and self.finalized
                    and ops._l.f32_contraction() != "exact" and (self.shard is None or self.shard.world == 1))

    def _build_split_wgrad_plan(self):
        if torch.cuda.is_available() and torch.cuda.is_current_stream_capturing():
            raise RuntimeError("the split filter-gradient plan is built by the first EAGER backward pass in a split-bf16 mode: run one "
                               "step (or call Ctx._build_split_wgrad_plan) before capturing")
        sp, plan, own = ops.Split3Plan(), ops.WgradPlan(int(os.environ.get("HDU_BATCH_WGRAD_TARGET", "0"))), []
        keep = []
        for cv in self.convs:
            cv.in_split_plan = False
            if not (cv.trainable and cv.out.root.needs_grad) or cv.halo or cv.cin_p % 8 or cv.cout_p % 8:
                continue
            if cv.xin is not None:
                src, pro, relu, up = cv.xin.act, None, False, cv.conv_up
            elif cv.bn is None and cv.skip is None:
                src, pro, relu, up = cv.x.act, None, False, cv.up
            elif cv.pw_fused:
                src, pro, relu, up = cv.x.act, (cv.bn.a, cv.bn.b), cv.bn.relu, cv.up
            else:
                continue
            g = cv.out.grad
            xs = ops.Act.alloc(3 * src.N, src.D, src.H, src.W, src.C, HDU_BF16)
            dys = ops.Act.alloc(3 * g.N, g.D, g.H, g.W, g.C, HDU_BF16)
            d16 = ops.conv_desc(xs, cv.wf_ptr, dys, cv.K, cv.stride, cv.pad, up)
            sp.add(src, ops._l.SPLIT3_OPERAND, xs, pro, relu)
            sp.add(g, ops._l.SPLIT3_GRADIENT, dys)
            if ops.conv_kernel_name(d16, 1) == "conv_stem_wgrad_kernel":
                own.append((d16, cv.kernel.grad))
            else:
                plan.add(d16, cv.kernel.grad)
            keep.append((xs, dys))
            cv.in_split_plan = True
        if len(sp):
            sp.finalize()
        if len(plan):
            plan.finalize()
        self._split_plan = (sp, plan, own, keep)

    def flush_pending_finalize(self):
        pend, self._pending_fin = self._pending_fin, None
        if pend is not None:
            (part, slots, M, C, g, be, sg, mean, rstd, dg, db, dsg, dsb, c3, c4) = pend["args"]
            ops.bn_bwd_finalize(part, slots, M, C, True, g, be, sg, mean, rstd, dg, db, dsg, dsb, c3, c4)

# ... 90 lines not shown
        if key not in self._grad_zero_ids:
            self._grad_zero_ids.add(key)
            self._grad_zero.append(buf)
            self._zp_step = None

    def prep_weights(self):
        if self._prep_n:
            ops.weight_prep_batched(self.dtype, self._prep_table, self._prep_n, self._prep_tiles, self.P, self.Wc)

    def _build_prep_table(self):
        from .lib import PrepEntry
        ents = []
        tiles = 0
        for cv in self.convs:
            wf = -1 if self.dtype == HDU_F32 else cv.wf_off
            wd = cv.wd_off if cv.need_dgrad_filter else -1
            if wf < 0 and wd < 0:
                continue
            ents.append(PrepEntry(cv.kernel.offset, wf, wd, tiles, cv.cout_p, cv.T, cv.cin_p, 0))
            tiles += cv.T * ((cv.cout_p + 63) // 64) * ((cv.cin_p + 63) // 64)
        self._prep_n = len(ents)
        self._prep_tiles = tiles
        if ents:
            arr = (PrepEntry * len(ents))(*ents)
            raw = np.frombuffer(bytes(arr), dtype=np.uint8).copy()
            self._prep_table = torch.from_numpy(raw).to(self.dev)

    def _fold_plan(self, phase):
        if phase not in self._fold_plans:
            ents = []
            for bn in self.bns:
                if bn.mode == "batch" and phase == 1:
                    continue
                ents.append((bn.C, bn.eps, bn.mm.data, bn.mv.data, bn.gamma.data, bn.beta.data,
                             bn.sg.data if bn.sg else None, bn.sb.data if bn.sb else None, bn.a, bn.b, bn.rstd))
            self._fold_plans[phase] = ops.FoldPlan(ents) if ents else None
        return self._fold_plans[phase]

    def shard_world(self):
        return self.shard.world if (self.shard is not None and self.shard.world > 1) else 1

    def conv_desc(self, *a, **k):
        return ops.conv_desc(*a, shard_world=self.shard_world(), **k)

    def prefold(self):
        self._prefolded_phase = None
        if self.batch_fold and self.finalized:
            plan = self._fold_plan(self.learning_phase)
            if plan is not None:
                plan.run()
                self._prefolded_phase = self.learning_phase

    def end_prefold(self):
        self._prefolded_phase = None

    def run_forward(self):
        self.pass_id += 1
        if self.batch_fold and self.finalized:
            plan = self._fold_plan(self.learning_phase)
            if plan is not None:
                if self._prefolded_phase != self.learning_phase:
                    plan.run()
                self.prefolded_pass = self.pass_id
        if self.learning_phase == 1 and self._zeroed_fwd_pass != self.pass_id and self.stats_acc is not None:
            self._zp_arena.run()
        for f in self.fwd:
            f()

    def bnb_fusable(self):
        return self.fuse_bn_bwd and (self.shard is None or self.shard.world == 1)

    def run_backward(self, seg=None):
        lo, hi = seg if seg is not None else (0, len(self.bwd))
        if lo == 0:
            for v in self.vars:
                v.written = False
            self.fuse_bn_bwd_now = self.bnb_fusable()
            if self._zeroed_bwd_pass != self.pass_id and self._zp_bwd is not None:
                self._zp_bwd.run()
                self._zeroed_bwd_pass = self.pass_id
        order = list(reversed(self.bwd))
        if lo == 0:
            self._bnb_deferred = []
            self._split_now = self.split_wgrad_active()
            if self._split_now and self._split_plan is None:
                self._build_split_wgrad_plan()
        split_bwd = self.dtype == HDU_F32 and ops._l.f32_split_in_backward_only()
        if split_bwd:
            ops._l.set_f32_split_now(True)
        try:
            for f in order[lo:hi]:
                f()
            self.flush_pending_finalize()
            if hi == len(self.bwd) and self._bnb_deferred:
                keys = tuple(k for k, _ in self._bnb_deferred)
                if self._bnb_plan is None or self._bnb_plan[0] != keys:
                    self._bnb_plan = (keys, ops.BnBwdPlan([e for _, e in self._bnb_deferred]))
                self._bnb_plan[1].run()
            if hi == len(self.bwd) and self.wgrad_plan is not None:
                self.wgrad_plan.run()
            if hi == len(self.bwd) and self._split_now:
                sp, plan, own, _ = self._split_plan
                sp.run()
                if len(plan):
                    plan.run()
                for d16, dw in own:
                    ops.conv_wgrad(d16, dw)
        finally:
            if split_bwd:
                ops._l.set_f32_split_now(False)

    def grad_buckets(self, fractions):
        n = len(self.bwd)
        tr = [p for p in self.params if p.trainable]
        index_of = {id(p): i for i, p in enumerate(self.params)}
        total = sum(p.numel for p in tr)
        cuts = []
        for f in sorted(fractions):
            want, done, pos, off = f * total, 0, n, self.n_trainable
            for k in range(n - 1, -1, -1):
                first = self.bwd.mark[k - 1] if k > 0 else 0
                own = [p for p in tr if first <= index_of[id(p)]]
                done = sum(p.numel for p in own)
                if done >= want:
                    pos, off = n - k, min([p.offset for p in own] + [self.n_trainable])
                    break
            if 0 < pos < n and (not cuts or pos > cuts[-1][0]):
                cuts.append((pos, off))
        out, prev_pos, prev_off = [], 0, self.n_trainable
        for pos, off in cuts:
            out.append((prev_pos, pos, off, prev_off))
            prev_pos, prev_off = pos, off
        out.append((prev_pos, n, 0, prev_off))
        return out


class BNLayer:
    BSUM_SLOTS = int(os.environ.get("HDU_BSUM_SLOTS", "16"))

    def __init__(self, ctx, name, C, eps=1e-3, momentum=0.99, mode="batch", trainable=True, scale_name=None,
                 scale_trainable=True, relu=True, scale=None):
        if scale is not None:
            scale_name, scale_trainable = scale.name, scale.trainable
        self.scale_layer = scale
        self.ctx, self.name, self.C, self.eps, self.momentum, self.mode, self.relu = ctx, name, C, eps, momentum, mode, relu
        self.trainable = trainable
        self.gamma = ctx.add_param(name, "bn", 0, (C,), (C,), trainable, "ones")
        self.beta = ctx.add_param(name, "bn", 1, (C,), (C,), trainable, "zeros")
        self.mm = ctx.add_param(name, "bn", 2, (C,), (C,), False, "zeros")
        self.mv = ctx.add_param(name, "bn", 3, (C,), (C,), False, "ones")
        self.sg = self.sb = None
        self.scale_trainable = scale_trainable
        if scale_name:
            self.sg = ctx.add_param(scale_name, "scale", 0, (C,), (C,), scale_trainable, "ones")
            self.sb = ctx.add_param(scale_name, "scale", 1, (C,), (C,), scale_trainable, "zeros")
            if scale is not None:
                scale.gamma, scale.beta = self.sg, self.sb
        v = ctx.fvec
        self.a, self.b, self.rstd = v(C), v(C), v(C)
        self.s1, self.s2, self.k1, self.k2, self.k3 = v(C), v(C), v(C), v(C), v(C)
        self.mean_used = None
        self.batch_now = False
        self.folded_pass = -1
        ctx.bns.append(self)
        self.s12 = v(2 * C)
        self.stats_src = None
        self.pending_stats = None
        self.bsum = None
        self._bsum_pass = -1

    def any_trainable(self):
        return self.trainable or (self.sg is not None and self.scale_trainable)

    def needs_stats(self):
        return self.mode == "batch"

    def fold(self, xvar):
        ctx = self.ctx
        sg = self.sg.data if self.sg else None
        sb = self.sb.data if self.sb else None
        self.batch_now = self.mode == "batch" and ctx.learning_phase == 1
        if self.batch_now and self.folded_pass == ctx.pass_id:
            return None
        if not self.batch_now and ctx.prefolded_pass == ctx.pass_id:
            self.mean_used = self.mm.data
            return None
        if self.batch_now:
            mean, var = xvar.stats()
            self.mean_used = mean
            args = (mean, var, self.gamma.data, self.beta.data, self.eps, sg, sb, self.a, self.b, self.rstd,
                    self.mm.data, self.mv.data, self.momentum)
        else:
            self.mean_used = self.mm.data
            args = (self.mm.data, self.mv.data, self.gamma.data, self.beta.data, self.eps, sg, sb, self.a, self.b,
                    self.rstd, None, None, self.momentum)
        ops.bn_fold(self.C, *args)
        return None

    def takes_epilogue_sums(self, xvar):
        ctx = self.ctx
        return bool((self.batch_now or self.any_trainable()) and not (ctx.shard is not None and ctx.shard.world > 1)
                    and self.bsum is not None and xvar.root.needs_grad and ctx._zeroed_bwd_pass == ctx.pass_id
                    and self._bsum_pass != ctx.pass_id)

    def backward(self, xvar, dz_act, sums_ready=False):
        ctx = self.ctx
        x = xvar.act
        need_sums = self.batch_now or self.any_trainable()
        tr_bn = self.trainable
        tr_sc = self.sg is not None and self.scale_trainable
        if ctx.shard is not None and ctx.shard.world > 1 and need_sums:
            ops.bn_bwd_reduce(dz_act, x, self.a, self.b, self.relu, self.mean_used, self.rstd, self.s1, self.s2, ctx.ws)
            ops.bn_bwd_coef(self.C, x.M, False, self.s1, self.s2, self.gamma.data, self.beta.data,
                            self.sg.data if self.sg else None, self.rstd, self.k1, self.k2, self.k3,
                            self.gamma.grad if tr_bn else None, self.beta.grad if tr_bn else None,
                            self.sg.grad if tr_sc else None, self.sb.grad if tr_sc else None)
            if self.batch_now:
                self.s12[:self.C].copy_(self.s1)
                self.s12[self.C:].copy_(self.s2)
                _sh.allreduce_sum(ctx.shard, self.s12)
                ops.bn_bwd_coef(self.C, x.M * ctx.shard.world, True, self.s12[:self.C], self.s12[self.C:],
                                self.gamma.data, self.beta.data, self.sg.data if self.sg else None, self.rstd, self.k1,
                                self.k2, self.k3)
        elif (need_sums and self.bsum is not None and xvar.root.needs_grad and ctx._zeroed_bwd_pass == ctx.pass_id
              and self._bsum_pass != ctx.pass_id):
            self._bsum_pass = ctx.pass_id
            acc = xvar.grad_mode()
            drop = xvar.root.drop if (ctx.dropout_enabled and ctx.learning_phase == 1) else None
            ops.bn_bwd_fused(dz_act, x, self.a, self.b, self.relu, self.mean_used, self.rstd, self.batch_now,
                             self.gamma.data, self.beta.data, self.sg.data if self.sg else None, self.bsum, self.BSUM_SLOTS,
                             self.gamma.grad if tr_bn else None, self.beta.grad if tr_bn else None,
                             self.sg.grad if tr_sc else None, self.sb.grad if tr_sc else None, xvar.grad, acc,
                             drop[0] if drop else 1.0, drop[1] if drop else 0, ctx.seed_dev if drop else None,
                             sums_ready=sums_ready)
            return
        elif need_sums:
            assert not sums_ready
            ops.bn_bwd_reduce_coef(dz_act, x, self.a, self.b, self.relu, self.mean_used, self.rstd, self.batch_now,
                                   self.gamma.data, self.beta.data, self.sg.data if self.sg else None, self.s1,
                                   self.s2, self.k1, self.k2, self.k3, self.gamma.grad if tr_bn else None,
                                   self.beta.grad if tr_bn else None, self.sg.grad if tr_sc else None,
                                   self.sb.grad if tr_sc else None, ctx.ws)
        else:
            ops.bn_bwd_coef(self.C, x.M, False, None, None, self.gamma.data, self.beta.data,
                            self.sg.data if self.sg else None, self.rstd, self.k1, self.k2, self.k3)
        if xvar.root.needs_grad:
            acc = xvar.grad_mode()
            drop = xvar.root.drop if (ctx.dropout_enabled and ctx.learning_phase == 1) else None
            ops.bn_bwd_apply(dz_act, x, self.a, self.b, self.relu, self.mean_used, self.k1, self.k2, self.k3,
                             xvar.grad, acc, drop[0] if drop else 1.0, drop[1] if drop else 0,
                             ctx.seed_dev if drop else None)


class ConvLayer:

    def __init__(self, ctx, name, x, filters, K, stride=(1, 1, 1), pad=(0, 0, 0), bn=None, up=(0, 0, 0), skip=None,
                 use_bias=True, out=None, init="glorot", trainable=True, dropout=0.0, keras_nd=2, cin_logical=None,
                 halo=0, producer=None):
        self.ctx, self.name, self.x, self.bn, self.up, self.skip = ctx, name, x, bn, up, skip
        self.K, self.stride = K, stride
        self.halo = halo
        if halo:
            assert not ctx.fuse_prologue, "halo mode materialises the conv input"
            assert skip is None or up == (0, 0, 0), "a skip add in halo mode must be at the stored resolution"
            pad = (pad[0] - (halo << up[0]), pad[1], pad[2])
        self.pad = pad
        self.trainable = trainable
        dt = ctx.dtype
        xa = x.act
        cin_p = xa.C
        cin = cin_logical or cin_p
        cout_p = ops.cpad(filters, dt)
        De, He, We = (xa.D + 2 * halo) << up[0], xa.H << up[1], xa.W << up[2]
        Do = (De + 2 * pad[0] - K[0]) // stride[0] + 1
        Ho = (He + 2 * pad[1] - K[1]) // stride[1] + 1
        Wo = (We + 2 * pad[2] - K[2]) // stride[2] + 1
        if out is None:
            out = ctx.new_var(xa.N, Do, Ho, Wo, cout_p)
        else:
            assert (out.act.N, out.act.D, out.act.H, out.act.W, out.act.C) == (xa.N, Do, Ho, Wo, cout_p)
        self.out = out
        kshape = ((K[1], K[2]) if keras_nd == 2 else (K[1], K[2], K[0])) + (cin, filters)
        self.kernel = ctx.add_param(name, "conv_kernel", 0, kshape, (cout_p, K[0], K[1], K[2], cin_p), trainable, init)
        self.bias = ctx.add_param(name, "conv_bias", 1, (filters,), (cout_p,), trainable, "zeros") if use_bias else None
        ctx.layer_kind[name] = "conv"
        self.T = K[0] * K[1] * K[2]
        self.cin_p, self.cout_p = cin_p, cout_p
        self.dropout = dropout
        if dropout > 0:
            ctx.drop_layers += 1
            self.drop_seed = 7919 * ctx.drop_layers
            out.root.drop = (1.0 - dropout, self.drop_seed)
        need_input_grad = x.root.needs_grad
        if ctx.grad_enabled:
            out.require_grad()
        self.xin = None
        self.conv_up = up
        self.pw_fused = bool(ctx.fuse_pw and bn is not None and skip is None and not halo and K == (1, 1, 1)
                             and stride == (1, 1, 1) and pad == (0, 0, 0) and up == (0, 0, 0) and cin_p <= ops.PRO_CMAX)
        if self.pw_fused:
            pass
        elif halo:
            self.xin = ctx.new_var(xa.N, xa.D + 2 * halo, xa.H, xa.W, cin_p)
            plane = xa.H * xa.W * cin_p
            self.xin_interior = ops.Act(self.xin.act.buf, halo * plane, xa.N, xa.D, xa.H, xa.W, cin_p, cin_p, dt)
            self._halo_tmp = ctx.scratch("halo_tmp", 1, 2 * halo, xa.H, xa.W, cin_p)
        elif (bn is not None or skip is not None) and not ctx.fuse_prologue:
            if skip is not None:
                self.xin = ctx.new_var(xa.N, De, He, We, cin_p)
                self.conv_up = (0, 0, 0)
            else:
                self.xin = ctx.new_var(xa.N, xa.D, xa.H, xa.W, cin_p)
        st = getattr(bn, "stats_src", None) if bn is not None else None
        if (st is not None and self.xin is not None and not halo and st.producer is not None and st.absorber is None
                and x.root is st.var.root and bn.C == x.C and x.c0 == (0 if bn is st.fold_next else st.var.c0)):
            st.absorber = self
        self.need_input_grad = need_input_grad
        self.epi_consumer = None
        self.epi_producer = None
        if (producer is not None and ctx.fuse_bn_epilogue and bn is not None and self.xin is not None and not halo
                and skip is None and up == (0, 0, 0) and x is producer.out and x.root is x and producer.epi_consumer is None):
            self.epi_producer = producer
            producer.epi_consumer = self
        self.strided = stride != (1, 1, 1)
        pw_stream = bool(ctx.fuse_bn_bwd_pw and dt == HDU_BF16 and K == (1, 1, 1) and pad == (0, 0, 0) and cout_p in (128, 192)
                         and cin_p >= 256 and xa.M >= 64)
        self.bnb_fused = bool(ctx.fuse_bn_bwd and need_input_grad and bn is not None and up == (0, 0, 0) and skip is None
                              and not halo and stride == (1, 1, 1) and not ctx.fuse_prologue and x.root.drop is None
                              and (ctx.fuse_bn_bwd_mode >= 2 or bn.mode != "batch" or pw_stream))
        self.bnb_off = None
        self._sums_kernel_ok = None
        self._s2 = None
        self._s2_ok = (os.environ.get("HDU_STRIDE2_DGRAD", "1") == "1" and all(v in (1, 2) for v in stride)
                       and xa.D % stride[0] == 0 and xa.H % stride[1] == 0 and xa.W % stride[2] == 0 and up == (0, 0, 0)
                       and bn is None and skip is None and not halo)
        self.need_dgrad_filter = need_input_grad and not self.strided
        self.wf_off = self.wd_off = None
        ctx.convs.append(self)
        if bn is not None:
            ctx.need_ws(xa.M, xa.C)
        ctx.need_ws(out.act.M, cout_p)
        if need_input_grad:
            if bn is not None or up != (0, 0, 0) or halo:
                self._dxe = ctx.scratch("dxe", xa.N, De, He, We, cin_p)
            if (bn is not None or halo) and up != (0, 0, 0):
                self._dz = ctx.scratch("dz", xa.N, xa.D + 2 * halo, xa.H, xa.W, cin_p)
        ctx.fwd.append(self.forward)
        ctx.bwd.append(self.backward)

    def bind(self):
        ctx = self.ctx
        esz = ctx.Wc.element_size()
        if ctx.dtype == HDU_F32:
            self.wf_ptr = ctypes.c_void_p(self.kernel.data.data_ptr())
        else:
            self.wf_ptr = ctypes.c_void_p(ctx.Wc.data_ptr() + self.wf_off * esz)
        self.wd_ptr = ctypes.c_void_p(ctx.Wc.data_ptr() + self.wd_off * esz) if self.need_dgrad_filter else None
        x, out = self.x.act, self.out.act
        pro = (self.bn.a, self.bn.b) if self.bn is not None else None
        relu = self.bn.relu if self.bn is not None else False
        skip = self.skip.act if self.skip is not None else None
        up = self.up
        if self.xin is not None:
            x, pro, relu, skip, up = self.xin.act, None, False, None, self.conv_up
        bias = self.bias.data if self.bias is not None else None
        if self.strided and self.need_input_grad and self._s2_ok and self.out.root.needs_grad:
            xa = self.x.act
            self._s2 = ops.Stride2Dgrad(ctx.dtype, self.kernel.data, self.out.grad, (xa.N, xa.D, xa.H, xa.W), xa.C, self.K,
                                        self.stride, self.pad, shard_world=ctx.shard_world())
        self.d_f = ctx.conv_desc(x, self.wf_ptr, out, self.K, self.stride, self.pad, up, skip, pro, relu, bias)
# ... 4 lines not shown
        self.d_f_epi = self.d_f_drop_epi = None
        cons = self.epi_consumer
        if cons is not None:
            epi = (cons.bn.a, cons.bn.b, cons.bn.relu)
            self.d_f_epi = ctx.conv_desc(x, self.wf_ptr, cons.xin.act, self.K, self.stride, self.pad, up, skip, pro, relu, bias,
                                         epi=epi)
            if self.dropout > 0:
                self.d_f_drop_epi = ctx.conv_desc(x, self.wf_ptr, cons.xin.act, self.K, self.stride, self.pad, up, skip, pro,
                                                  relu, bias, False, 1.0 - self.dropout, self.drop_seed, ctx.seed_dev, epi=epi)
        self.d_f_st = self.d_f_drop_st = None
        sink = getattr(self, "stats_sink", None)
        if sink is not None:
            shift = sink.var.stats_shift()
            part = ctypes.c_void_p(ctx.stats_acc.data_ptr() + 4 * sink.acc_off)

            def with_stats(d):
                if d is None:
                    return None
                c = type(d)()
                ctypes.memmove(ctypes.byref(c), ctypes.byref(d), ctypes.sizeof(d))
                c.stats_partial, c.stats_shift, c.stats_slots = part, ctypes.c_void_p(shift.data_ptr()), sink.SLOTS
                return c
            self.d_f_st, self.d_f_drop_st = with_stats(self.d_f), with_stats(self.d_f_drop)

    def prep(self):
        ctx = self.ctx
        if ctx.dtype == HDU_F32 and not self.need_dgrad_filter:
            return
        wf = None if ctx.dtype == HDU_F32 else ctx.Wc[self.wf_off:self.wf_off + self.kernel.numel]
        wd = ctx.Wc[self.wd_off:self.wd_off + self.kernel.numel] if self.need_dgrad_filter else None
        ops.weight_prep(ctx.dtype, self.kernel.data, self.cout_p, self.T, self.cin_p, wf, wd)

    def epi_active(self):
        ctx, bn = self.ctx, self.bn
        if self.epi_producer is None or (bn.mode == "batch" and ctx.learning_phase == 1):
            return False
        if ctx.learning_phase == 0 or not (self.need_input_grad or bn.any_trainable()):
            return True
        return ctx.fuse_bn_epilogue_train and self.bnb_fused and self.need_input_grad and ctx.bnb_fusable()

    def forward(self):
        ctx = self.ctx
        if self.epi_producer is not None and self.epi_active():
            return self._forward_conv()
        if self.bn is not None:
            self.bn.fold(self.x)
        if self.xin is not None:
            bn = self.bn
            up = self.up if self.skip is not None else (0, 0, 0)
            skip = self.skip.act if self.skip is not None else None
            dst = self.xin_interior if self.halo else self.xin.act
            pend = bn.pending_stats if bn is not None else None
            if pend is not None and pend[0] == ctx.pass_id and pend[1].absorber is self:
                ops.materialize_stats(self.x.act, pend[1].stats_block(bn), bn.relu, up, skip, dst)
            else:
                ops.materialize(self.x.act, bn.a if bn else None, bn.b if bn else None, bn.relu if bn else False, up, skip, dst)
            if self.halo:
                _sh.halo_exchange(ctx.shard, self.xin.act, self.halo)
        self._forward_conv()

    def _forward_conv(self):
        ctx = self.ctx
        cons = self.epi_consumer
        if cons is not None and cons.epi_active():
            cons.bn.fold(self.out)
            drop = self.d_f_drop_epi is not None and ctx.learning_phase == 1 and ctx.dropout_enabled
            ops.conv_fprop(self.d_f_drop_epi if drop else self.d_f_epi)
            return
        st = ctx.learning_phase == 1 and self.d_f_st is not None and self.stats_sink.primed
        if self.d_f_drop is not None and ctx.learning_phase == 1 and ctx.dropout_enabled:
            ops.conv_fprop(self.d_f_drop_st if st else self.d_f_drop)
        else:
            ops.conv_fprop(self.d_f_st if st else self.d_f)

    def backward(self):
        ctx = self.ctx
        out = self.out
        if not out.root.needs_grad:
            return
        dy = out.dy()
        x = self.x.act
        if self.trainable and (getattr(self, "in_plan", False) or (ctx._split_now and getattr(self, "in_split_plan", False))):
            if self.bias is not None:
                ops.colsum(dy, self.bias.grad, ctx.ws)
        elif self.trainable:
            if self.xin is not None:
                d = ctx.conv_desc(self.xin.act, self.wf_ptr, dy, self.K, self.stride, self.pad, self.conv_up)
            else:
                d = ctx.conv_desc(x, self.wf_ptr, dy, self.K, self.stride, self.pad, self.up,
                                  self.skip.act if self.skip is not None else None,
                                  (self.bn.a, self.bn.b) if self.bn is not None else None,
                                  self.bn.relu if self.bn is not None else False)
            ops.conv_wgrad(d, self.kernel.grad)
            if self.bias is not None:
                ops.colsum(dy, self.bias.grad, ctx.ws)
        if not self.need_input_grad:
            return
        K, pad = self.K, self.pad
        if self.halo:
            return self._backward_halo(dy)
        if self.bnb_fused and ctx.fuse_bn_bwd_now:
            return self._backward_fused_bn(dy)
        De, He, We = x.D << self.up[0], x.H << self.up[1], x.W << self.up[2]
        direct = self.bn is None and self.up == (0, 0, 0)
        sums_ready = False
        skip_first = self.skip is not None and self.skip.root.needs_grad and not self.skip.root.written \
            and self.skip.c0 == 0
        if direct:
            tgt, acc = self.x.grad, self.x.grad_mode()
        elif skip_first:
            tgt, acc = self.skip.grad, self.skip.grad_mode()
        else:
            tgt, acc = self._dxe(), False
        if self.strided:
            tgt_act = ops.Act(tgt.buf, tgt.off, x.N, x.D, x.H, x.W, x.C, tgt.ld, tgt.dtype)
            if self._s2 is not None:
                self._s2.run(tgt_act, accumulate=acc)
            else:
                d = ctx.conv_desc(tgt_act, self.wf_ptr, dy, K, self.stride, pad, accumulate=acc)
                ops.conv_dgrad_strided(d)
        else:
            d = ctx.conv_desc(dy, self.wd_ptr, ops.Act(tgt.buf, tgt.off, x.N, De, He, We, x.C, tgt.ld, tgt.dtype), K,
                              (1, 1, 1), (K[0] - 1 - pad[0], K[1] - 1 - pad[1], K[2] - 1 - pad[2]), accumulate=acc)
            sums_ready = self._epilogue_sums(d)
            ops.conv_fprop(d)
        if self.skip is not None and self.skip.root.needs_grad and not skip_first:
            ops.upsample_bwd(tgt, self.skip.grad, (0, 0, 0), accumulate=self.skip.grad_mode())
        if direct:
            return
        dz = tgt
        if self.up != (0, 0, 0):
            if self.bn is None:
                ops.upsample_bwd(tgt, self.x.grad, self.up, accumulate=self.x.grad_mode())
                return
            dz = self._dz()
            ops.upsample_bwd(tgt, dz, self.up)
        if self.bn is not None:
            self.bn.backward(self.x, dz, sums_ready=sums_ready)
        else:
            ops.upsample_bwd(dz, self.x.grad, (0, 0, 0), accumulate=self.x.grad_mode())

    def _epilogue_sums(self, d):
        ctx, bn = self.ctx, self.bn
        if not (ctx.bnb_sums_epilogue and bn is not None and self.up == (0, 0, 0) and self.skip is None and not self.halo
                and self.x.root.drop is None and ctx.bnb_fusable() and bn.BSUM_SLOTS <= 32):
            return False
        if self._sums_kernel_ok is None:
            name = ops.conv_kernel_name(d, 0)
            self._sums_kernel_ok = name.startswith("conv_igemm_ring_kernel") or name.startswith("conv_igemm_dma_kernel")
        if not self._sums_kernel_ok or not bn.takes_epilogue_sums(self.x):
            return False
        x = self.x.act
        d.bnb_u, d.bnb_ldu = x.ptr, x.ld
        d.bnb_a, d.bnb_b = bn.a.data_ptr(), bn.b.data_ptr()
        d.bnb_relu = (1 if bn.relu else 0) | 4
        d.bnb_mean, d.bnb_rstd = bn.mean_used.data_ptr(), bn.rstd.data_ptr()
        d.bnb_partial, d.bnb_slots = bn.bsum.data_ptr(), bn.BSUM_SLOTS
        return True


def _conv_backward_fused_bn(self, dy):
    ctx, bn, xv = self.ctx, self.bn, self.x
    x = xv.act
    K, pad = self.K, self.pad
    acc = xv.grad_mode()
    tgt = xv.grad
    d = ctx.conv_desc(dy, self.wd_ptr, ops.Act(tgt.buf, tgt.off, x.N, x.D, x.H, x.W, x.C, tgt.ld, tgt.dtype), K, (1, 1, 1),
                      (K[0] - 1 - pad[0], K[1] - 1 - pad[1], K[2] - 1 - pad[2]), accumulate=acc)
    d.bnb_u, d.bnb_ldu = x.ptr, x.ld
    d.bnb_a, d.bnb_b, d.bnb_relu = bn.a.data_ptr(), bn.b.data_ptr(), 1 if bn.relu else 0
    if self.epi_producer is not None and self.epi_active():
        d.bnb_u, d.bnb_ldu = self.xin.act.ptr, self.xin.act.ld
        d.bnb_relu |= 2
    need_sums = bn.batch_now or bn.any_trainable()
    part = None
    if need_sums:
        n = self.BNB_SLOTS * 2 * bn.C
        part = ctx.bnb_acc[self.bnb_off:self.bnb_off + n]
        d.bnb_mean, d.bnb_rstd = bn.mean_used.data_ptr(), bn.rstd.data_ptr()
        d.bnb_partial, d.bnb_slots = part.data_ptr(), self.BNB_SLOTS
    ops.conv_fprop(d)
    if need_sums:
        tr_bn = bn.trainable
        tr_sc = bn.sg is not None and bn.scale_trainable
        c3 = c4 = None
        if bn.batch_now:
            r = xv.root
            ld = r.act.ld
            base = r.corr_off + xv.c0
            c3, c4 = ctx.corr_acc[base:base + bn.C], ctx.corr_acc[base + ld:base + ld + bn.C]
        if not bn.batch_now and ctx.batch_wgrad and ctx.defer_bnb_finalize:
            ctx._bnb_deferred.append((id(self), (part, self.BNB_SLOTS, bn.C, bn.gamma.data, bn.beta.data,
                                                 bn.sg.data if bn.sg else None, bn.gamma.grad if tr_bn else None,
                                                 bn.beta.grad if tr_bn else None, bn.sg.grad if tr_sc else None,
                                                 bn.sb.grad if tr_sc else None)))
            return
        fin_args = (part, self.BNB_SLOTS, x.M, bn.C, bn.gamma.data, bn.beta.data, bn.sg.data if bn.sg else None, bn.mean_used, bn.rstd,
                    bn.gamma.grad if tr_bn else None, bn.beta.grad if tr_bn else None,
                    bn.sg.grad if tr_sc else None, bn.sb.grad if tr_sc else None, c3, c4)
        if bn.batch_now and ctx.merge_fin_correct and self.BNB_SLOTS <= 32 and bn.C % 4 == 0:
            ctx.flush_pending_finalize()
            ctx._pending_fin = dict(root=xv.root, c0=xv.c0, C=bn.C, M=x.M, args=fin_args)
            return
        ops.bn_bwd_finalize(part, self.BNB_SLOTS, x.M, bn.C, bn.batch_now, bn.gamma.data, bn.beta.data,
                            bn.sg.data if bn.sg else None, bn.mean_used, bn.rstd,
                            bn.gamma.grad if tr_bn else None, bn.beta.grad if tr_bn else None,
                            bn.sg.grad if tr_sc else None, bn.sb.grad if tr_sc else None, c3, c4)


ConvLayer._backward_fused_bn = _conv_backward_fused_bn
ConvLayer.BNB_SLOTS = int(os.environ.get("HDU_BNB_SLOTS", "16"))


def _conv_backward_halo(self, dy):
    ctx = self.ctx
    x = self.x.act
    K, pad, h = self.K, self.pad, self.halo
    De, He, We = (x.D + 2 * h) << self.up[0], x.H << self.up[1], x.W << self.up[2]
    tgt = self._dxe()
    if self.strided:
        d = ctx.conv_desc(ops.Act(tgt.buf, tgt.off, x.N, De, He, We, x.C, tgt.ld, tgt.dtype), self.wf_ptr, dy, K,
                          self.stride, pad)
        ops.conv_dgrad_strided(d)
    else:
        d = ctx.conv_desc(dy, self.wd_ptr, ops.Act(tgt.buf, tgt.off, x.N, De, He, We, x.C, tgt.ld, tgt.dtype), K, (1, 1, 1),
                          (K[0] - 1 - pad[0], K[1] - 1 - pad[1], K[2] - 1 - pad[2]), halo_out=(2 * h) << self.up[0])
        ops.conv_fprop(d)
    dz = tgt
    if self.up != (0, 0, 0):
        dz = self._dz()
        ops.upsample_bwd(tgt, dz, self.up)
    _sh.halo_reduce(ctx.shard, dz, h, self._halo_tmp().buf)
    plane = x.H * x.W * dz.ld
    interior = ops.Act(dz.buf, dz.off + h * plane, x.N, x.D, x.H, x.W, x.C, dz.ld, dz.dtype)
    if self.skip is not None and self.skip.root.needs_grad:
        ops.upsample_bwd(interior, self.skip.grad, (0, 0, 0), accumulate=self.skip.grad_mode())
    if self.bn is not None:
        self.bn.backward(self.x, interior)
    else:
        ops.upsample_bwd(interior, self.x.grad, (0, 0, 0), accumulate=self.x.grad_mode())


ConvLayer._backward_halo = _conv_backward_halo


class StatsOp:

    SLOTS = int(os.environ.get("HDU_STATS_SLOTS", "32"))

    def __init__(self, ctx, var):
        self.ctx, self.var = ctx, var
        self.fused = None
        self.fold_next = None
        self.absorber = None
        world = ctx.shard.world if ctx.shard is not None else 1
        self.sync_buf = ctx.fvec(world * (1 + 2 * var.C)) if world > 1 else None
        ctx.need_ws(var.act.M, var.C)
        var.stats()
        self.producer = None
        prod = ctx.convs[-1] if ctx.convs else None
        sharded = ctx.shard is not None and ctx.shard.world > 1
        if (ctx.epilogue_stats and not sharded and prod is not None and ctx.fwd and ctx.fwd[-1] == prod.forward
                and prod.out.root is var.root and prod.out.c0 == var.c0 and prod.out.C == var.C
                and getattr(prod, "stats_sink", None) is None):
            self.producer = prod
            prod.stats_sink = self
            self.acc_off = None
            self.primed = False
            ctx.stats_sinks.append(self)
        ctx.fwd.append(self.forward)

    def fuse(self, bn):
        assert bn.C == self.var.C and bn.mode == "batch"
        self.fused = bn
        bn.stats_src = self
        return self

    def then_fold(self, bn):
        if self.fused is None and bn.mode == "batch" and self.ctx.fold_next and bn.C == self.var.c0 + self.var.C:
            self.fold_next = bn
            bn.stats_src = self
        return self

    def stats_block(self, bn):
        ctx = self.ctx
        n = self.SLOTS * 2 * self.var.C
        fold = (bn.gamma.data, bn.beta.data, bn.eps, bn.sg.data if bn.sg else None, bn.sb.data if bn.sb else None,
                bn.a, bn.b, bn.rstd, bn.mm.data, bn.mv.data, bn.momentum)
        part = ctx.stats_acc[self.acc_off:self.acc_off + n]
        if bn is self.fused:
            mean, var = self.var.stats()
            return (part, self.SLOTS, self.var.act.M, self.var.C, 0, self.var.stats_shift(), mean, var, fold)
        r = self.var.root
# ... 161 lines not shown
```

h-denseunet_amd/lib.py:

```python
import ctypes
import os

_HERE = os.path.dirname(os.path.abspath(__file__))
_ROOT = os.path.dirname(_HERE)

HDU_BF16 = 0
HDU_F32 = 1

c_int, c_i64, c_f, c_p, c_u32, c_sz = (ctypes.c_int, ctypes.c_int64, ctypes.c_float, ctypes.c_void_p,
                                       ctypes.c_uint32, ctypes.c_size_t)


class ConvDesc(ctypes.Structure):
    _fields_ = [
        ("dtype", c_int),
        ("x", c_p), ("ldx", c_i64),
        ("N", c_int), ("Di", c_int), ("Hi", c_int), ("Wi", c_int), ("Cin", c_int),
        ("ud", c_int), ("uh", c_int), ("uw", c_int),
        ("skip", c_p), ("ldskip", c_i64),
        ("pro_a", c_p), ("pro_b", c_p), ("pro_relu", c_int),
        ("w", c_p),
        ("KD", c_int), ("KH", c_int), ("KW", c_int),
        ("sd", c_int), ("sh", c_int), ("sw", c_int),
        ("pd", c_int), ("ph", c_int), ("pw", c_int),
        ("y", c_p), ("ldy", c_i64),
        ("Do", c_int), ("Ho", c_int), ("Wo", c_int), ("Cout", c_int),
        ("bias", c_p),
        ("epi_a", c_p), ("epi_b", c_p), ("epi_relu", c_int),
        ("accumulate", c_int),
        ("drop_keep", c_f),
        ("drop_seed", c_u32),
        ("drop_seed_dev", c_p),
        ("stats_partial", c_p),
        ("stats_shift", c_p),
        ("stats_slots", c_int),
        ("bnb_u", c_p), ("bnb_ldu", c_i64),
        ("bnb_a", c_p), ("bnb_b", c_p), ("bnb_mean", c_p), ("bnb_rstd", c_p),
        ("bnb_relu", c_int),
        ("bnb_partial", c_p), ("bnb_slots", c_int),
        ("splitk_ws", c_p),
        ("splitk_ws_bytes", c_sz),
        ("splitk_counters", c_p),
        ("layer_rows", ctypes.c_int64),
    ]


class PrepEntry(ctypes.Structure):
    _fields_ = [("master_off", c_i64), ("w_f_off", c_i64), ("w_d_off", c_i64), ("tile_begin", c_i64),
                ("Cout", ctypes.c_int32), ("T", ctypes.c_int32), ("Cin", ctypes.c_int32), ("pad_", ctypes.c_int32)]


class AugSample(ctypes.Structure):
    _fields_ = [("img_off", c_i64), ("vrows", ctypes.c_int32), ("vcols", ctypes.c_int32), ("vslices", ctypes.c_int32),
                ("a0", ctypes.c_int32), ("b0", ctypes.c_int32), ("c0", ctypes.c_int32), ("crop", ctypes.c_int32),
                ("flip", ctypes.c_int32)]


class ZeroEntry(ctypes.Structure):
    _fields_ = [("ptr", c_p), ("bytes", ctypes.c_uint64), ("block_begin", ctypes.c_uint32), ("pad_", ctypes.c_uint32),
                ("src", c_p)]


class BnBwdEntry(ctypes.Structure):
    _fields_ = [("partial", c_p), ("slots", ctypes.c_int32), ("C", ctypes.c_int32), ("gamma", c_p), ("beta", c_p),
                ("sgamma", c_p), ("dgamma", c_p), ("dbeta", c_p), ("dsgamma", c_p), ("dsbeta", c_p)]


class BnStatsFold(ctypes.Structure):
    _fields_ = [("partial", c_p), ("slots", ctypes.c_int32), ("Cseg", ctypes.c_int32), ("seg_c0", ctypes.c_int32),
                ("pad_", ctypes.c_int32), ("M", c_i64), ("shift", c_p), ("mean", c_p), ("var", c_p), ("gamma", c_p),
                ("beta", c_p), ("sgamma", c_p), ("sbeta", c_p), ("eps", c_f), ("momentum", c_f), ("a", c_p), ("b", c_p),
                ("rstd", c_p), ("mov_mean", c_p), ("mov_var", c_p)]


ZERO_BLOCK_BYTES = 65536


class Split3Entry(ctypes.Structure):
    _fields_ = [("src", c_p), ("dst", c_p), ("a", c_p), ("b", c_p), ("ld_src", ctypes.c_uint64), ("rows", ctypes.c_uint64),
                ("C", ctypes.c_uint32), ("relu", ctypes.c_uint32), ("pattern", ctypes.c_uint32), ("cols", ctypes.c_uint32),
                ("col_groups", ctypes.c_uint32), ("block_begin", ctypes.c_uint32), ("iters", ctypes.c_uint32),
                ("chl", ctypes.c_uint32)]


SPLIT3_OPERAND, SPLIT3_GRADIENT = 0, 1


class FoldEntry(ctypes.Structure):
    _fields_ = [("mean", c_p), ("var", c_p), ("gamma", c_p), ("beta", c_p), ("sgamma", c_p), ("sbeta", c_p),
                ("a", c_p), ("b", c_p), ("rstd", c_p), ("C", ctypes.c_int32), ("eps", c_f)]


_SIGS = {
    "hdu_last_error": (ctypes.c_char_p, []),
    "hdu_backend": (ctypes.c_char_p, []),
    "hdu_abi_version": (c_int, []),
    "hdu_sizeof_conv_desc": (c_sz, []),
    "hdu_set_tuning": (c_int, [c_int, c_int]),
    "hdu_conv_fprop": (c_int, [ctypes.POINTER(ConvDesc), c_p]),
    "hdu_bn_bwd_finalize": (c_int, [c_p, c_int, c_i64, c_int, c_int, c_p, c_p, c_p, c_p, c_p, c_p, c_p, c_p, c_p, c_p, c_p, c_p]),
    "hdu_bn_bwd_correct": (c_int, [c_int, c_p, c_i64, c_i64, c_int, c_p, c_p, c_p, c_i64, c_p]),
    "hdu_bn_bwd_finalize_correct": (c_int, [c_int, c_p, c_int, c_i64, c_int, c_p, c_p, c_p, c_p, c_p, c_p, c_p, c_p, c_p, c_p, c_p,
                                            c_int, c_int, c_p, c_i64, c_p, c_i64, c_p]),
    "hdu_conv_splitk_ws_bytes": (c_sz, [ctypes.POINTER(ConvDesc)]),
    "hdu_conv_wgrad": (c_int, [ctypes.POINTER(ConvDesc), c_p, c_p]),
    "hdu_conv_dgrad_strided": (c_int, [ctypes.POINTER(ConvDesc), c_p]),
    "hdu_stride2_dgrad_filters": (c_int, [c_int, c_p, c_int, c_int, c_int, c_int, c_int, c_int, c_int, c_int, c_int, c_int,
                                          c_int, c_p, c_p]),
    "hdu_parity_interleave": (c_int, [c_int, c_p, c_int, c_int, c_int, c_int, c_int, c_int, c_int, c_int, c_p, c_i64, c_int,
                                      c_p]),
    "hdu_conv_kernel_name": (c_int, [ctypes.POINTER(ConvDesc), c_int, ctypes.c_char_p, c_sz]),
    "hdu_weight_prep": (c_int, [c_int, c_p, c_int, c_int, c_int, c_p, c_p, c_p]),
    "hdu_weight_prep_batched": (c_int, [c_int, c_p, c_int, c_i64, c_p, c_p, c_p]),
    "hdu_reduce_ws_bytes": (c_sz, [c_i64, c_int]),
    "hdu_bn_stats": (c_int, [c_int, c_p, c_i64, c_i64, c_int, c_p, c_p, c_p, c_sz, c_p]),
    "hdu_bn_fold": (c_int, [c_int, c_p, c_p, c_p, c_p, c_f, c_p, c_p, c_p, c_p, c_p, c_p, c_p, c_f, c_p]),
    "hdu_augment_batch": (c_int, [c_p, c_p, c_p, c_int, c_int, c_int, c_int, c_f, c_p, c_p, c_i64, c_i64, c_i64, c_p, c_i64,
                                  c_i64, c_p]),
    "hdu_bn_fold_batched": (c_int, [c_p, c_p, c_int, ctypes.c_uint32, c_p]),
    "hdu_bn_stats_fold": (c_int, [c_int, c_p, c_i64, c_i64, c_int, c_p, c_p, c_p, c_p, c_f, c_p, c_p, c_p, c_p, c_p, c_p,
                                  c_p, c_f, c_p, c_sz, c_p]),
    "hdu_bn_bwd_reduce_coef": (c_int, [c_int, c_p, c_i64, c_p, c_i64, c_i64, c_int, c_p, c_p, c_int, c_p, c_p, c_int,
                                       c_p, c_p, c_p, c_p, c_p, c_p, c_p, c_p, c_p, c_p, c_p, c_p, c_p, c_sz, c_p]),
    "hdu_bn_bwd_reduce": (c_int, [c_int, c_p, c_i64, c_p, c_i64, c_i64, c_int, c_p, c_p, c_int, c_p, c_p, c_p, c_p,
                                  c_p, c_sz, c_p]),
    "hdu_bn_bwd_coef": (c_int, [c_int, c_i64, c_int, c_p, c_p, c_p, c_p, c_p, c_p, c_p, c_p, c_p, c_p, c_p, c_p,
                                c_p, c_p]),
    "hdu_bn_bwd_apply": (c_int, [c_int, c_p, c_i64, c_p, c_i64, c_i64, c_int, c_p, c_p, c_int, c_p, c_p, c_p, c_p,
                                 c_p, c_i64, c_int, c_f, c_u32, c_p, c_p]),
    "hdu_bn_bwd_fused": (c_int, [c_int, c_p, c_i64, c_p, c_i64, c_i64, c_int, c_p, c_p, c_int, c_p, c_p, c_int, c_p, c_p,
                                 c_p, c_p, c_int, c_p, c_p, c_p, c_p, c_p, c_i64, c_int, c_f, c_u32, c_p, c_p]),
    "hdu_bn_bwd_apply_sums": (c_int, [c_int, c_p, c_i64, c_p, c_i64, c_i64, c_int, c_p, c_p, c_int, c_p, c_p, c_int, c_p, c_p,
                                      c_p, c_p, c_int, c_p, c_p, c_p, c_p, c_p, c_i64, c_int, c_f, c_u32, c_p, c_p]),
    "hdu_affine_act": (c_int, [c_int, c_p, c_i64, c_i64, c_int, c_p, c_p, c_int, c_p, c_i64, c_p]),
    "hdu_materialize": (c_int, [c_int, c_p, c_i64, c_int, c_int, c_int, c_int, c_int, c_p, c_p, c_int, c_int, c_int, c_int,
                                c_p, c_i64, c_p, c_i64, c_p]),
    "hdu_bn_bwd_finalize_batched": (c_int, [c_p, c_p, c_int, c_u32, c_p]),
    "hdu_materialize_stats": (c_int, [c_int, c_p, c_i64, c_int, c_int, c_int, c_int, c_int, c_p, c_int, c_int, c_int, c_int,
                                      c_p, c_i64, c_p, c_i64, c_p]),
    "hdu_wgrad_plan_entry_bytes": (c_sz, []),
    "hdu_wgrad_plan_fill": (c_int, [ctypes.POINTER(ConvDesc), c_p, c_int, c_int, c_p, ctypes.POINTER(c_int), ctypes.POINTER(ctypes.c_uint32)]),
    "hdu_wgrad_plan_shape": (c_int, [ctypes.POINTER(ConvDesc), ctypes.POINTER(c_int), ctypes.POINTER(ctypes.c_uint32),
                                     ctypes.POINTER(ctypes.c_uint32)]),
    "hdu_wgrad_plan_run": (c_int, [c_int, c_p, c_p, c_int, ctypes.c_uint32, c_p]),
    "hdu_bn_stats_finalize_fold_next": (c_int, [c_p, c_int, c_i64, c_int, c_int, c_int, c_p, c_p, c_p, c_p, c_p, c_f, c_p, c_p,
                                                c_p, c_p, c_p, c_p, c_p, c_f, c_p]),
    "hdu_bn_stats_finalize": (c_int, [c_p, c_int, c_i64, c_int, c_p, c_p, c_p, c_p, c_p, c_f, c_p, c_p, c_p, c_p, c_p, c_p, c_p,
                                      c_f, c_p]),
    "hdu_stats_sync_floats": (c_sz, [c_int, c_int]),
    "hdu_stats_pack": (c_int, [c_int, c_p, c_p, c_i64, c_int, c_int, c_p, c_p]),
    "hdu_stats_unpack": (c_int, [c_int, c_p, c_int, c_p, c_p, c_p]),
    "hdu_colsum": (c_int, [c_int, c_p, c_i64, c_i64, c_int, c_p, c_p, c_sz, c_p]),
    "hdu_maxpool3s2_fwd": (c_int, [c_int, c_p, c_i64, c_int, c_int, c_int, c_int, c_int, c_p, c_i64, c_p, c_int, c_p]),
    "hdu_maxpool3s2_bwd": (c_int, [c_int, c_p, c_p, c_i64, c_int, c_int, c_int, c_int, c_int, c_p, c_i64, c_int, c_int, c_p]),
    "hdu_avgpool2_fwd": (c_int, [c_int, c_p, c_i64, c_int, c_int, c_int, c_int, c_int, c_p, c_i64, c_p]),
    "hdu_avgpool2_bwd": (c_int, [c_int, c_p, c_i64, c_int, c_int, c_int, c_int, c_int, c_p, c_i64, c_int, c_p]),
    "hdu_upsample_bwd": (c_int, [c_int, c_p, c_i64, c_int, c_int, c_int, c_int, c_int, c_int, c_int, c_int, c_p,
                                 c_i64, c_int, c_p]),
    "hdu_wce_loss": (c_int, [c_int, c_p, c_i64, c_p, c_i64, c_f, c_f, c_f, c_f, c_p, c_i64, c_int, c_p, c_p, c_p,
                             c_sz, c_p]),
    "hdu_sgd_nesterov": (c_int, [c_p, c_p, c_p, c_i64, c_f, c_f, c_f, c_p]),
    "hdu_slab25d": (c_int, [c_int, c_p, c_int, c_int, c_int, c_p, c_int, c_p]),
    "hdu_make_input3d": (c_int, [c_int, c_p, c_p, c_i64, c_f, c_int, c_int, c_int, c_p, c_int, c_p]),
    "hdu_make_input3d_bwd": (c_int, [c_int, c_p, c_int, c_f, c_i64, c_p, c_i64, c_int, c_int, c_p]),
    "hdu_cast_pad": (c_int, [c_int, c_p, c_i64, c_int, c_p, c_i64, c_int, c_p]),
    "hdu_cast_out": (c_int, [c_int, c_p, c_i64, c_i64, c_int, c_p, c_p]),
    "hdu_softmax_accumulate": (c_int, [c_int, c_p, c_i64, c_i64, c_int, c_p, c_p]),
    "hdu_sweep_gather": (c_int, [c_p, c_int, c_i64, c_int, c_p, c_int, c_p, c_int, c_f, c_f, c_f, c_p, c_p]),
    "hdu_sweep_accumulate": (c_int, [c_int, c_p, c_i64, c_i64, c_int, c_int, c_int, c_p, c_int, c_p, c_p, c_p, c_p]),
    "hdu_sweep_advance": (c_int, [c_p, c_int, c_p]),
    "hdu_pp_threshold": (c_int, [c_p, c_p, c_int, c_int, c_int, c_int, c_int, c_int, ctypes.c_double, ctypes.c_double, c_p, c_p, c_p]),
    "hdu_pp_dilate": (c_int, [c_p, c_int, c_int, c_int, c_p, c_p]),
    "hdu_pp_label": (c_int, [c_p, c_int, c_int, c_int, c_int, c_int, c_p, c_p]),
    "hdu_pp_largest": (c_int, [c_p, c_int, c_int, c_int, c_p, c_p, c_p, c_p, c_p]),
    "hdu_pp_fill_holes": (c_int, [c_p, c_int, c_int, c_int, c_p, c_p, c_p, c_p]),
    "hdu_pp_bbox": (c_int, [c_p, c_int, c_int, c_int, c_p, c_p]),
    "hdu_pp_merge": (c_int, [c_int, c_p, c_p, c_i64, c_p, c_p]),
    "hdu_zero_regions": (c_int, [c_p, c_int, c_u32, c_p, c_u32, c_p]),
    "hdu_zero": (c_int, [c_p, ctypes.c_uint64, c_p]),
    "hdu_split3_entry_fill": (c_int, [c_p, c_p, c_i64, c_i64, c_int, c_p, c_p, c_int, c_int, c_p, c_u32, ctypes.POINTER(c_u32)]),
    "hdu_split3_batched": (c_int, [c_p, c_int, c_u32, c_int, c_p]),
    "hdu_profile_begin": (c_int, [c_int]),
    "hdu_profile_count": (c_int, []),
    "hdu_profile_end": (c_int, []),
    "hdu_profile_get": (c_int, [c_int, ctypes.c_char_p, c_sz, ctypes.POINTER(c_f)]),
    "hdu_comm_unique_id": (c_int, [c_p]),
    "hdu_comm_init": (c_int, [ctypes.POINTER(c_p), c_int, c_int, c_p]),
    "hdu_comm_destroy": (c_int, [c_p]),
    "hdu_comm_allreduce_f32": (c_int, [c_p, c_p, c_i64, c_p]),
    "hdu_comm_sendrecv": (c_int, [c_p, c_int, c_p, c_p, c_int, c_p, c_p, c_sz, c_p]),
}

EXPORTS = tuple(_SIGS.keys())

_lib = None
_backend = None


class HduError(RuntimeError):
    pass


ABI_VERSION = 9


def product_library_path():
    return os.path.join(_HERE, "libhdu.so")


def _bind(path):
    import torch
    lib = ctypes.CDLL(path)
    for name, (res, args) in _SIGS.items():
        fn = getattr(lib, name)
        fn.restype = res
        fn.argtypes = args
    if lib.hdu_abi_version() != ABI_VERSION or lib.hdu_sizeof_conv_desc() != ctypes.sizeof(ConvDesc):
        raise HduError("%s has ABI version %d / hdu_conv_desc of %d bytes, this binding expects %d / %d -- rebuild it "
                       "(python -c 'import __graft_entry__ as g; g.build()')" %
                       (path, lib.hdu_abi_version(), lib.hdu_sizeof_conv_desc(), ABI_VERSION, ctypes.sizeof(ConvDesc)))
    return lib


def _apply_env_tuning(lib):
    if "HDU_DMA_STAGES" in os.environ:
        lib.hdu_set_tuning(0, int(os.environ["HDU_DMA_STAGES"]))
    if "HDU_SPLITK" in os.environ:
        lib.hdu_set_tuning(13, int(os.environ["HDU_SPLITK"]))
    if "HDU_BM64_MAX_M" in os.environ:
        lib.hdu_set_tuning(18, int(os.environ["HDU_BM64_MAX_M"]))
    if "HDU_SPLITK_TARGET" in os.environ:
        lib.hdu_set_tuning(16, int(os.environ["HDU_SPLITK_TARGET"]))
    if "HDU_SPLITK_MIN_STEPS" in os.environ:
        lib.hdu_set_tuning(17, int(os.environ["HDU_SPLITK_MIN_STEPS"]))
    if "HDU_HALO_MIN_TILES" in os.environ:
        lib.hdu_set_tuning(15, int(os.environ["HDU_HALO_MIN_TILES"]))
    if "HDU_RING_MIN_K" in os.environ:
        lib.hdu_set_tuning(14, int(os.environ["HDU_RING_MIN_K"]))
    if "HDU_RED_WGS" in os.environ:
        lib.hdu_set_tuning(11, int(os.environ["HDU_RED_WGS"]))
    if "HDU_ROW_WGS" in os.environ:
        lib.hdu_set_tuning(12, int(os.environ["HDU_ROW_WGS"]))
    if "HDU_NO_HALO_FPROP" in os.environ:
        lib.hdu_set_tuning(9, int(os.environ["HDU_NO_HALO_FPROP"]))
    if "HDU_NO_HALO" in os.environ:
        lib.hdu_set_tuning(8, int(os.environ["HDU_NO_HALO"]))
    if "HDU_HALO_WIDE" in os.environ:
        lib.hdu_set_tuning(29, int(os.environ["HDU_HALO_WIDE"]))
    if "HDU_HALO_MIN_W" in os.environ:
        lib.hdu_set_tuning(28, int(os.environ["HDU_HALO_MIN_W"]))
    if "HDU_HALO_TARGET" in os.environ:
        lib.hdu_set_tuning(7, int(os.environ["HDU_HALO_TARGET"]))
    if "HDU_MAX_BN" in os.environ:
        lib.hdu_set_tuning(6, int(os.environ["HDU_MAX_BN"]))
    if "HDU_NO_FAST" in os.environ:
        lib.hdu_set_tuning(5, int(os.environ["HDU_NO_FAST"]))
    if "HDU_DEBUG_FLAGS" in os.environ:
        lib.hdu_set_tuning(4, int(os.environ["HDU_DEBUG_FLAGS"]))
    if "HDU_XCD_SWIZZLE" in os.environ:
        lib.hdu_set_tuning(3, int(os.environ["HDU_XCD_SWIZZLE"]))
    if "HDU_WGRAD_TARGET" in os.environ:
        lib.hdu_set_tuning(2, int(os.environ["HDU_WGRAD_TARGET"]))
    if "HDU_NO_PW_BSTAT" in os.environ:
        lib.hdu_set_tuning(19, int(os.environ["HDU_NO_PW_BSTAT"]))
    if "HDU_PW_BSTAT_WGS" in os.environ:
        lib.hdu_set_tuning(20, int(os.environ["HDU_PW_BSTAT_WGS"]))
    if "HDU_PW_BSTAT_FORM" in os.environ:
        lib.hdu_set_tuning(30, int(os.environ["HDU_PW_BSTAT_FORM"]))
    if "HDU_SPLIT3_FORM" in os.environ:
        lib.hdu_set_tuning(31, int(os.environ["HDU_SPLIT3_FORM"]))
    if "HDU_WGRAD_NCT" in os.environ:
        lib.hdu_set_tuning(21, int(os.environ["HDU_WGRAD_NCT"]))
    if "HDU_NO_PRO_DMA" in os.environ:
        lib.hdu_set_tuning(22, int(os.environ["HDU_NO_PRO_DMA"]))
    if "HDU_PERS" in os.environ:
        lib.hdu_set_tuning(23, int(os.environ["HDU_PERS"]))
    if "HDU_NO_PW_BSTAT_BNB" in os.environ:
        lib.hdu_set_tuning(26, int(os.environ["HDU_NO_PW_BSTAT_BNB"]))
    lib.hdu_set_tuning(TUNE_F32_SPLIT, _F32_MODES[_f32_contraction])
    if "HDU_PERS_MIN_ITEMS" in os.environ:
        lib.hdu_set_tuning(24, int(os.environ["HDU_PERS_MIN_ITEMS"]))
    if "HDU_WGRAD_MIN_STEPS" in os.environ:
        lib.hdu_set_tuning(1, int(os.environ["HDU_WGRAD_MIN_STEPS"]))


def load(path=None):
# ... 117 lines not shown
```

h-denseunet_amd/ops.py:

```python
import ctypes

import torch

from . import lib as _l
from .lib import HDU_BF16, HDU_F32, ConvDesc, check

_TORCH_DT = {HDU_BF16: torch.bfloat16, HDU_F32: torch.float32}
CHUNK = {HDU_BF16: 8, HDU_F32: 4}


def device():
    if _l.is_emulator():
        return torch.device("cpu")
    if not torch.cuda.is_available():
        raise _l.HduError("libhdu.so (gfx950) is bound but no GPU is visible; there is no CPU fallback")
    return torch.device("cuda", torch.cuda.current_device())


def stream():
    if _l.is_emulator():
        return None
    return ctypes.c_void_p(torch.cuda.current_stream().cuda_stream)


# ... 365 lines not shown

    def __init__(self, entries):
        import numpy as np
        self.keep = entries
        n = len(entries)
        tab = (_l.FoldEntry * n)()
        begins = np.zeros(n, dtype=np.uint32)
        tot = 0
        for i, (C, eps, mean, var, g, be, sg, sb, a, b, r) in enumerate(entries):
            p = lambda t: t.data_ptr() if t is not None else None
            tab[i] = _l.FoldEntry(p(mean), p(var), p(g), p(be), p(sg), p(sb), p(a), p(b), p(r), C, eps)
            begins[i] = tot
            tot += (C + 255) // 256
        self.n, self.total = n, tot
        self.table = torch.from_numpy(np.frombuffer(bytes(tab), dtype=np.uint8).copy()).to(device())
        self.begins = torch.from_numpy(begins.view(np.int32)).to(device())

    def run(self):
        check(_l.get().hdu_bn_fold_batched(ctypes.c_void_p(self.table.data_ptr()), ctypes.c_void_p(self.begins.data_ptr()),
                                           self.n, self.total, stream()), "hdu_bn_fold_batched")


class BnBwdPlan:

    def __init__(self, entries):
        import numpy as np
        self.keep = entries
        n = len(entries)
        tab = (_l.BnBwdEntry * n)()
        begins = np.zeros(n, dtype=np.uint32)
        tot = 0
        p = lambda t: t.data_ptr() if t is not None else None
        for i, (part, slots, C, g, be, sg, dg, db, dsg, dsb) in enumerate(entries):
            tab[i] = _l.BnBwdEntry(p(part), slots, C, p(g), p(be), p(sg), p(dg), p(db), p(dsg), p(dsb))
            begins[i] = tot
            tot += (C + 7) // 8
        self.n, self.total = n, tot
        self.table = torch.from_numpy(np.frombuffer(bytes(tab), dtype=np.uint8).copy()).to(device())
        self.begins = torch.from_numpy(begins.view(np.int32)).to(device())

    def run(self):
        check(_l.get().hdu_bn_bwd_finalize_batched(ctypes.c_void_p(self.table.data_ptr()), ctypes.c_void_p(self.begins.data_ptr()),
                                                   self.n, self.total, stream()), "hdu_bn_bwd_finalize_batched")


def bn_stats_fold(x, mean, var, gamma, beta, eps, sgamma, sbeta, a, b, rstd, mov_mean, mov_var, momentum, ws):
    check(_l.get().hdu_bn_stats_fold(x.dtype, x.ptr, x.ld, x.M, x.C, fptr(mean), fptr(var), fptr(gamma), fptr(beta), eps,
                                     fptr(sgamma), fptr(sbeta), fptr(a), fptr(b), fptr(rstd), fptr(mov_mean),
                                     fptr(mov_var), momentum, ws.ptr, ws.nbytes, stream()), "hdu_bn_stats_fold")


def bn_bwd_reduce_coef(dz, x, a, b, relu, mean, rstd, batch_stats, gamma, beta, sgamma, s1, s2, k1, k2, k3, dgamma,
                       dbeta, dsgamma, dsbeta, ws):
    check(_l.get().hdu_bn_bwd_reduce_coef(x.dtype, dz.ptr, dz.ld, x.ptr, x.ld, x.M, x.C, fptr(a), fptr(b),
                                          1 if relu else 0, fptr(mean), fptr(rstd), 1 if batch_stats else 0,
                                          fptr(gamma), fptr(beta), fptr(sgamma), fptr(s1), fptr(s2), fptr(k1), fptr(k2),
                                          fptr(k3), fptr(dgamma), fptr(dbeta), fptr(dsgamma), fptr(dsbeta), ws.ptr,
                                          ws.nbytes, stream()), "hdu_bn_bwd_reduce_coef")


def bn_bwd_reduce(dz, x, a, b, relu, mean, rstd, s1, s2, ws):
    check(_l.get().hdu_bn_bwd_reduce(x.dtype, dz.ptr, dz.ld, x.ptr, x.ld, x.M, x.C, fptr(a), fptr(b), 1 if relu else 0,
                                     fptr(mean), fptr(rstd), fptr(s1), fptr(s2), ws.ptr, ws.nbytes, stream()),
          "hdu_bn_bwd_reduce")


def bn_bwd_coef(C, M, batch_stats, s1, s2, gamma, beta, sgamma, rstd, k1, k2, k3, dgamma=None, dbeta=None,
                dsgamma=None, dsbeta=None):
    check(_l.get().hdu_bn_bwd_coef(C, M, 1 if batch_stats else 0, fptr(s1), fptr(s2), fptr(gamma), fptr(beta),
                                   fptr(sgamma), fptr(rstd), fptr(k1), fptr(k2), fptr(k3), fptr(dgamma), fptr(dbeta),
                                   fptr(dsgamma), fptr(dsbeta), stream()), "hdu_bn_bwd_coef")


def bn_bwd_apply(dz, x, a, b, relu, mean, k1, k2, k3, dx, accumulate=False, drop_keep=1.0, drop_seed=0,
                 drop_seed_dev=None):
    check(_l.get().hdu_bn_bwd_apply(x.dtype, dz.ptr, dz.ld, x.ptr, x.ld, x.M, x.C, fptr(a), fptr(b), 1 if relu else 0,
                                    fptr(mean), fptr(k1), fptr(k2), fptr(k3), dx.ptr, dx.ld, 1 if accumulate else 0,
                                    drop_keep, drop_seed,
                                    ctypes.c_void_p(drop_seed_dev.data_ptr()) if drop_seed_dev is not None else None,
                                    stream()), "hdu_bn_bwd_apply")


def bn_bwd_fused(dz, x, a, b, relu, mean, rstd, batch_stats, gamma, beta, sgamma, sums, slots, dgamma, dbeta, dsgamma,
                 dsbeta, dx, accumulate=False, drop_keep=1.0, drop_seed=0, drop_seed_dev=None, sums_ready=False):
    fn = _l.get().hdu_bn_bwd_apply_sums if sums_ready else _l.get().hdu_bn_bwd_fused
    check(fn(x.dtype, dz.ptr, dz.ld, x.ptr, x.ld, x.M, x.C, fptr(a), fptr(b), 1 if relu else 0,
             fptr(mean), fptr(rstd), 1 if batch_stats else 0, fptr(gamma), fptr(beta), fptr(sgamma),
             fptr(sums), slots, fptr(dgamma), fptr(dbeta), fptr(dsgamma), fptr(dsbeta), dx.ptr, dx.ld,
             1 if accumulate else 0, drop_keep, drop_seed,
             ctypes.c_void_p(drop_seed_dev.data_ptr()) if drop_seed_dev is not None else None,
             stream()), "hdu_bn_bwd_fused")


def bn_bwd_finalize(partial, slots, M, C, batch_stats, gamma, beta, sgamma, mean, rstd, dgamma, dbeta, dsgamma, dsbeta,
                    corr3, corr4):
    check(_l.get().hdu_bn_bwd_finalize(fptr(partial), slots, M, C, 1 if batch_stats else 0, fptr(gamma), fptr(beta),
                                       fptr(sgamma), fptr(mean), fptr(rstd), fptr(dgamma), fptr(dbeta), fptr(dsgamma),
                                       fptr(dsbeta), fptr(corr3), fptr(corr4), stream()), "hdu_bn_bwd_finalize")


def bn_bwd_finalize_correct(partial, slots, M, C, gamma, beta, sgamma, mean, rstd, dgamma, dbeta, dsgamma, dsbeta, corr3, corr4,
                            cs0, u, du):
    check(_l.get().hdu_bn_bwd_finalize_correct(u.dtype, fptr(partial), slots, M, C, fptr(gamma), fptr(beta), fptr(sgamma), fptr(mean),
                                               fptr(rstd), fptr(dgamma), fptr(dbeta), fptr(dsgamma), fptr(dsbeta), fptr(corr3),
                                               fptr(corr4), cs0, u.C, u.ptr, u.ld, du.ptr, du.ld, stream()),
          "hdu_bn_bwd_finalize_correct")


def bn_bwd_correct(u, corr3, corr4, du):
    check(_l.get().hdu_bn_bwd_correct(u.dtype, u.ptr, u.ld, u.M, u.C, fptr(corr3), fptr(corr4), du.ptr, du.ld, stream()),
          "hdu_bn_bwd_correct")


def affine_act(x, a, b, relu, z):
    check(_l.get().hdu_affine_act(x.dtype, x.ptr, x.ld, x.M, x.C, fptr(a), fptr(b), 1 if relu else 0, z.ptr, z.ld,
                                  stream()), "hdu_affine_act")


def materialize(x, a, b, relu, up, skip, out):
    check(_l.get().hdu_materialize(x.dtype, x.ptr, x.ld, x.N, x.D, x.H, x.W, x.C, fptr(a), fptr(b), 1 if relu else 0,
                                   up[0], up[1], up[2], skip.ptr if skip is not None else None,
                                   skip.ld if skip is not None else 0, out.ptr, out.ld, stream()), "hdu_materialize")


def bn_stats_finalize(partial, slots, M, C, shift, mean, var, fold=None):
    g, be, eps, sg, sb, a, b, r, mm, mv, mom = fold if fold is not None else (None, None, 0.0, None, None, None, None,
                                                                                 None, None, None, 0.0)
    check(_l.get().hdu_bn_stats_finalize(fptr(partial), slots, M, C, fptr(shift), fptr(mean), fptr(var), fptr(g), fptr(be),
                                         eps, fptr(sg), fptr(sb), fptr(a), fptr(b), fptr(r), fptr(mm), fptr(mv), mom,
                                         stream()), "hdu_bn_stats_finalize")


def bn_stats_finalize_fold_next(partial, slots, M, Cseg, seg_c0, C_all, shift_all, mean_all, var_all, fold):
    g, be, eps, sg, sb, a, b, r, mm, mv, mom = fold
    check(_l.get().hdu_bn_stats_finalize_fold_next(fptr(partial), slots, M, Cseg, seg_c0, C_all, fptr(shift_all),
                                                   fptr(mean_all), fptr(var_all), fptr(g), fptr(be), eps, fptr(sg), fptr(sb),
                                                   fptr(a), fptr(b), fptr(r), fptr(mm), fptr(mv), mom, stream()),
          "hdu_bn_stats_finalize_fold_next")


def materialize_stats(x, stats, relu, up, skip, out):
    partial, slots, M, Cseg, seg_c0, shift, mean, var, fold = stats
    g, be, eps, sg, sb, a, b, r, mm, mv, mom = fold
    f = _l.BnStatsFold()
    f.partial, f.slots, f.Cseg, f.seg_c0, f.M = fptr(partial), slots, Cseg, seg_c0, M
    f.shift, f.mean, f.var = fptr(shift), fptr(mean), fptr(var)
    f.gamma, f.beta, f.sgamma, f.sbeta, f.eps, f.momentum = fptr(g), fptr(be), fptr(sg), fptr(sb), eps, mom
    f.a, f.b, f.rstd, f.mov_mean, f.mov_var = fptr(a), fptr(b), fptr(r), fptr(mm), fptr(mv)
    check(_l.get().hdu_materialize_stats(x.dtype, x.ptr, x.ld, x.N, x.D, x.H, x.W, x.C, ctypes.byref(f), 1 if relu else 0,
                                         up[0], up[1], up[2], skip.ptr if skip is not None else None,
                                         skip.ld if skip is not None else 0, out.ptr, out.ld, stream()), "hdu_materialize_stats")


def colsum(x, out, ws):
    check(_l.get().hdu_colsum(x.dtype, x.ptr, x.ld, x.M, x.C, fptr(out), ws.ptr, ws.nbytes, stream()), "hdu_colsum")


def maxpool_fwd(x, y, argmax=None, pad_d=1):
    check(_l.get().hdu_maxpool3s2_fwd(x.dtype, x.ptr, x.ld, x.N, x.D, x.H, x.W, x.C, y.ptr, y.ld,
                                      ctypes.c_void_p(argmax.data_ptr()) if argmax is not None else None, pad_d,
                                      stream()),
          "hdu_maxpool3s2_fwd")


def maxpool_bwd(argmax, dy, dx, accumulate=False, pad_d=1):
    check(_l.get().hdu_maxpool3s2_bwd(dx.dtype, ctypes.c_void_p(argmax.data_ptr()), dy.ptr, dy.ld, dx.N, dx.D, dx.H,
                                      dx.W, dx.C, dx.ptr, dx.ld, 1 if accumulate else 0, pad_d, stream()),
          "hdu_maxpool3s2_bwd")


def avgpool_fwd(x, y):
    check(_l.get().hdu_avgpool2_fwd(x.dtype, x.ptr, x.ld, x.N, x.D, x.H, x.W, x.C, y.ptr, y.ld, stream()),
          "hdu_avgpool2_fwd")

# ... 125 lines not shown
```

include/hdu.h:

```cpp
#ifndef HDU_H_
#define HDU_H_

#include <stddef.h>
#include <stdint.h>

#ifdef __cplusplus
extern "C" {
#endif

#define HDU_BF16 0
#define HDU_F32 1

#define HDU_OK 0
#define HDU_ERR_ARG (-1)
#define HDU_ERR_LAUNCH (-2)
#define HDU_ERR_WORKSPACE (-3)

const char* hdu_last_error(void);
const char* hdu_backend(void);
#define HDU_ABI_VERSION 9
int hdu_abi_version(void);
size_t hdu_sizeof_conv_desc(void);
int hdu_profile_begin(int max_records);
int hdu_profile_count(void);
int hdu_profile_end(void);
int hdu_profile_get(int i, char* name_buf, size_t buflen, float* ms);
#define HDU_TUNE_DMA_STAGES 0
#define HDU_TUNE_HALO_TARGET_WGS 7
#define HDU_TUNE_MAX_BN 6
#define HDU_TUNE_NO_FAST 5
#define HDU_TUNE_DEBUG 4
#define HDU_TUNE_XCD_SWIZZLE 3
#define HDU_TUNE_RED_WGS 11
#define HDU_TUNE_ROW_WGS 12
#define HDU_TUNE_NO_HALO_FPROP 9
#define HDU_TUNE_NO_HALO 8
#define HDU_TUNE_WGRAD_TARGET_WGS 2
#define HDU_TUNE_SPLITK 13
#define HDU_TUNE_BM64_MAX_M 18
#define HDU_TUNE_SPLITK_TARGET 16
#define HDU_TUNE_SPLITK_MIN_STEPS 17
#define HDU_TUNE_HALO_MIN_TILES 15
#define HDU_TUNE_RING_MIN_K 14
#define HDU_TUNE_WGRAD_MIN_STEPS 1
#define HDU_TUNE_NO_PW_BSTAT 19
#define HDU_TUNE_PW_BSTAT_WGS 20
#define HDU_TUNE_PW_BSTAT_FORM 30
#define HDU_TUNE_NO_PRO_DMA 22
#define HDU_TUNE_PERS 23
#define HDU_TUNE_NO_PW_BSTAT_BNB 26
#define HDU_TUNE_PERS_MIN_ITEMS 24
#define HDU_TUNE_HALO_MIN_W 28
#define HDU_TUNE_F32_SPLIT 27
#define HDU_TUNE_HALO_WIDE 29
#define HDU_TUNE_SPLIT3_FORM 31
#define HDU_TUNE_WGRAD_NCT 21
int hdu_set_tuning(int key, int value);

typedef struct hdu_conv_desc {
  int dtype;
  const void* x;      int64_t ldx;
  int N, Di, Hi, Wi, Cin;
  int ud, uh, uw;
  const void* skip;   int64_t ldskip;
  const float* pro_a; const float* pro_b; int pro_relu;
  const void* w;
  int KD, KH, KW;
  int sd, sh, sw;
  int pd, ph, pw;
  void* y;            int64_t ldy;
  int Do, Ho, Wo, Cout;
  const float* bias;
  const float* epi_a; const float* epi_b; int epi_relu;
  int accumulate;
  float drop_keep;
  uint32_t drop_seed;
  const uint32_t* drop_seed_dev;
  float* stats_partial;
  const float* stats_shift;
  int stats_slots;
  const void* bnb_u;  int64_t bnb_ldu;
  const float* bnb_a; const float* bnb_b; const float* bnb_mean; const float* bnb_rstd;
  int bnb_relu;
  float* bnb_partial; int bnb_slots;
  void* splitk_ws;
  size_t splitk_ws_bytes;
  uint32_t* splitk_counters;
  int64_t layer_rows;
} hdu_conv_desc;

int hdu_bn_bwd_finalize(const float* partial, int slots, int64_t M, int C, int batch_stats, const float* gamma,
                        const float* beta, const float* sgamma, const float* mean, const float* rstd, float* dgamma,
                        float* dbeta, float* dsgamma, float* dsbeta, float* corr3, float* corr4, void* stream);

typedef struct hdu_bnbwd_entry {
  const float* partial;
  int32_t slots, C;
  const float* gamma; const float* beta; const float* sgamma;
  float* dgamma; float* dbeta; float* dsgamma; float* dsbeta;
} hdu_bnbwd_entry;
int hdu_bn_bwd_finalize_batched(const hdu_bnbwd_entry* table, const uint32_t* begins, int n, uint32_t total_blocks, void* stream);

int hdu_bn_bwd_correct(int dtype, const void* u, int64_t ldu, int64_t M, int C, const float* corr3, const float* corr4,
                       void* du, int64_t lddu, void* stream);
int hdu_bn_bwd_finalize_correct(int dtype, const float* partial, int slots, int64_t M, int C, const float* gamma, const float* beta,
                                const float* sgamma, const float* mean, const float* rstd, float* dgamma, float* dbeta,
                                float* dsgamma, float* dsbeta, float* corr3, float* corr4, int cs0, int Cc, const void* u,
                                int64_t ldu, void* du, int64_t lddu, void* stream);

size_t hdu_conv_splitk_ws_bytes(const hdu_conv_desc* d);

int hdu_conv_fprop(const hdu_conv_desc* d, void* stream);

int hdu_conv_wgrad(const hdu_conv_desc* d, float* dw, void* stream);

size_t hdu_wgrad_plan_entry_bytes(void);
int hdu_wgrad_plan_fill(const hdu_conv_desc* d, float* dw, int target_wgs, int min_steps, void* entry, int* variant,
                        uint32_t* nblocks);
int hdu_wgrad_plan_shape(const hdu_conv_desc* d, int* variant, uint32_t* tiles, uint32_t* steps);
int hdu_wgrad_plan_run(int variant, const void* dev_entries, const uint32_t* dev_begins, int n, uint32_t total_blocks,
                       void* stream);

int hdu_conv_dgrad_strided(const hdu_conv_desc* d, void* stream);

int hdu_stride2_dgrad_filters(int dtype, const float* w_master, int Cout, int KD, int KH, int KW, int Cin, int sd, int sh,
                              int sw, int pd, int ph, int pw, void* w_out, void* stream);
int hdu_parity_interleave(int dtype, const void* cls, int N, int Di, int Hi, int Wi, int C, int sd, int sh, int sw, void* dx,
                          int64_t lddx, int accumulate, void* stream);

int hdu_conv_kernel_name(const hdu_conv_desc* d, int op, char* buf, size_t buflen);

int hdu_weight_prep(int dtype, const float* w_master, int Cout, int T, int Cin, void* w_f, void* w_d, void* stream);

#define HDU_PREP_TILE 64
typedef struct hdu_prep_entry {
  int64_t master_off, w_f_off, w_d_off, tile_begin;
  int32_t Cout, T, Cin, pad_;
} hdu_prep_entry;
int hdu_weight_prep_batched(int dtype, const hdu_prep_entry* table, int n, int64_t total_tiles,
                            const float* master_base, void* wc_base, void* stream);

typedef struct hdu_aug_sample {
  int64_t img_off;
  int32_t vrows, vcols, vslices;
  int32_t a0, b0, c0;
  int32_t crop, flip;
} hdu_aug_sample;
int hdu_augment_batch(const float* img, const uint8_t* lab, const hdu_aug_sample* samples, int n, int size, int nslices,
                      int lab_slice, float mean, float* minmax_ws, float* x_out, int64_t x_sample, int64_t x_pix,
                      int64_t x_slice, uint8_t* y_out, int64_t y_sample, int64_t y_slice, void* stream);

size_t hdu_reduce_ws_bytes(int64_t M, int C);

typedef struct hdu_fold_entry {
  const float* mean; const float* var; const float* gamma; const float* beta; const float* sgamma; const float* sbeta;
  float* a; float* b; float* rstd;
  int32_t C; float eps;
} hdu_fold_entry;
int hdu_bn_fold_batched(const hdu_fold_entry* table, const uint32_t* begins, int n, uint32_t total_blocks, void* stream);

int hdu_bn_stats(int dtype, const void* x, int64_t ldx, int64_t M, int C, float* mean, float* var, void* ws,
                 size_t ws_bytes, void* stream);

int hdu_bn_fold(int C, const float* mean, const float* var, const float* gamma, const float* beta, float eps,
                const float* sgamma, const float* sbeta, float* a, float* b, float* rstd, float* mov_mean,
                float* mov_var, float momentum, void* stream);

int hdu_bn_stats_fold(int dtype, const void* x, int64_t ldx, int64_t M, int C, float* mean, float* var,
                      const float* gamma, const float* beta, float eps, const float* sgamma, const float* sbeta,
                      float* a, float* b, float* rstd, float* mov_mean, float* mov_var, float momentum, void* ws,
                      size_t ws_bytes, void* stream);

int hdu_bn_bwd_reduce_coef(int dtype, const void* dz, int64_t lddz, const void* x, int64_t ldx, int64_t M, int C,
                           const float* a, const float* b, int relu, const float* mean, const float* rstd,
                           int batch_stats, const float* gamma, const float* beta, const float* sgamma, float* s1,
                           float* s2, float* k1, float* k2, float* k3, float* dgamma, float* dbeta, float* dsgamma,
                           float* dsbeta, void* ws, size_t ws_bytes, void* stream);

int hdu_bn_bwd_reduce(int dtype, const void* dz, int64_t lddz, const void* x, int64_t ldx, int64_t M, int C,
                      const float* a, const float* b, int relu, const float* mean, const float* rstd, float* s1,
                      float* s2, void* ws, size_t ws_bytes, void* stream);

int hdu_bn_bwd_coef(int C, int64_t M, int batch_stats, const float* s1, const float* s2, const float* gamma,
                    const float* beta, const float* sgamma, const float* rstd, float* k1, float* k2, float* k3,
                    float* dgamma, float* dbeta, float* dsgamma, float* dsbeta, void* stream);

int hdu_bn_bwd_apply(int dtype, const void* dz, int64_t lddz, const void* x, int64_t ldx, int64_t M, int C,
                     const float* a, const float* b, int relu, const float* mean, const float* k1,
                     const float* k2, const float* k3, void* dx, int64_t lddx, int accumulate, float drop_keep,
                     uint32_t drop_seed, const uint32_t* drop_seed_dev, void* stream);

int hdu_bn_bwd_fused(int dtype, const void* dz, int64_t lddz, const void* x, int64_t ldx, int64_t M, int C, const float* a,
                     const float* b, int relu, const float* mean, const float* rstd, int batch_stats, const float* gamma,
                     const float* beta, const float* sgamma, float* sums, int slots, float* dgamma, float* dbeta,
                     float* dsgamma, float* dsbeta, void* dx, int64_t lddx, int accumulate, float drop_keep,
                     uint32_t drop_seed, const uint32_t* drop_seed_dev, void* stream);

int hdu_bn_bwd_apply_sums(int dtype, const void* dz, int64_t lddz, const void* x, int64_t ldx, int64_t M, int C, const float* a,
                          const float* b, int relu, const float* mean, const float* rstd, int batch_stats, const float* gamma,
                          const float* beta, const float* sgamma, float* sums, int slots, float* dgamma, float* dbeta,
                          float* dsgamma, float* dsbeta, void* dx, int64_t lddx, int accumulate, float drop_keep,
                          uint32_t drop_seed, const uint32_t* drop_seed_dev, void* stream);

int hdu_affine_act(int dtype, const void* x, int64_t ldx, int64_t M, int C, const float* a, const float* b,
                   int relu, void* z, int64_t ldz, void* stream);

int hdu_materialize(int dtype, const void* x, int64_t ldx, int N, int D, int H, int W, int C, const float* a,
                    const float* b, int relu, int ud, int uh, int uw, const void* skip, int64_t ldskip, void* out,
                    int64_t ldout, void* stream);

int hdu_bn_stats_finalize(const float* partial, int slots, int64_t M, int C, const float* shift, float* mean, float* var,
                          const float* gamma, const float* beta, float eps, const float* sgamma, const float* sbeta,
                          float* a, float* b, float* rstd, float* mov_mean, float* mov_var, float momentum, void* stream);

int hdu_bn_stats_finalize_fold_next(const float* partial, int slots, int64_t M, int Cseg, int seg_c0, int C_all,
                                    const float* shift_all, float* mean_all, float* var_all, const float* gamma,
                                    const float* beta, float eps, const float* sgamma, const float* sbeta, float* a, float* b,
                                    float* rstd, float* mov_mean, float* mov_var, float momentum, void* stream);

typedef struct hdu_stats_fold_desc {
  const float* partial;
  int32_t slots, Cseg, seg_c0, pad_;
  int64_t M;
  const float* shift;
  float* mean;
  float* var;
  const float* gamma; const float* beta; const float* sgamma; const float* sbeta;
  float eps, momentum;
  float* a; float* b; float* rstd; float* mov_mean; float* mov_var;
} hdu_stats_fold_desc;
int hdu_materialize_stats(int dtype, const void* x, int64_t ldx, int N, int D, int H, int W, int C, const hdu_stats_fold_desc* f,
                          int relu, int ud, int uh, int uw, const void* skip, int64_t ldskip, void* out, int64_t ldout,
                          void* stream);

size_t hdu_stats_sync_floats(int C, int world);
int hdu_stats_pack(int C, const float* mean, const float* var, int64_t n_local, int rank, int world, float* buf, void* stream);
int hdu_stats_unpack(int C, const float* buf, int world, float* mean, float* var, void* stream);

int hdu_colsum(int dtype, const void* x, int64_t ldx, int64_t M, int C, float* out, void* ws, size_t ws_bytes,
               void* stream);

int hdu_maxpool3s2_fwd(int dtype, const void* x, int64_t ldx, int N, int D, int H, int W, int C, void* y,
                       int64_t ldy, uint8_t* argmax ,
                       int pad_d ,
                       void* stream);
int hdu_maxpool3s2_bwd(int dtype, const uint8_t* argmax, const void* dy, int64_t lddy, int N, int D, int H, int W,
                       int C, void* dx, int64_t lddx, int accumulate, int pad_d, void* stream);
int hdu_avgpool2_fwd(int dtype, const void* x, int64_t ldx, int N, int D, int H, int W, int C, void* y,
                     int64_t ldy, void* stream);
int hdu_avgpool2_bwd(int dtype, const void* dy, int64_t lddy, int N, int D, int H, int W, int C, void* dx,
                     int64_t lddx, int accumulate, void* stream);
int hdu_upsample_bwd(int dtype, const void* dxe, int64_t lddxe, int N, int D, int H, int W, int C, int ud, int uh,
                     int uw, void* dz, int64_t lddz, int accumulate, void* stream);

int hdu_wce_loss(int dtype, const void* logits, int64_t ldl, const uint8_t* labels, int64_t M, float w0, float w1,
                 float w2, float grad_scale, void* dlogits, int64_t lddl, int C_pad, float* loss_sum,
                 float* class_count, void* ws, size_t ws_bytes, void* stream);

int hdu_sgd_nesterov(float* p, float* v, const float* g, int64_t n, float lr, float momentum, float grad_scale,
                     void* stream);

int hdu_slab25d(int dtype, const float* vol, int D, int H, int W, void* out, int Cpad, void* stream);
int hdu_make_input3d(int dtype, const float* vol, const void* logits2d, int64_t ldl, float scale, int D, int H,
                     int W, void* out, int Cpad, void* stream);
int hdu_make_input3d_bwd(int dtype, const void* dinput3d, int Cpad, float scale, int64_t M, void* dlogits2d,
                         int64_t lddl, int Cpad_l, int accumulate, void* stream);

int hdu_cast_pad(int dtype, const float* src, int64_t M, int C, void* dst, int64_t lddst, int Cpad, void* stream);
int hdu_cast_out(int dtype, const void* src, int64_t ldsrc, int64_t M, int C, float* dst, void* stream);

int hdu_softmax_accumulate(int dtype, const void* logits, int64_t ldl, int64_t M, int num, float* score, void* stream);

int hdu_sweep_gather(const float* vol, int z, int64_t plane, int win_planes, const int32_t* starts, int nwin,
                     const int32_t* cursor, int preprocess, float lo, float hi, float mean, float* dst, void* stream);
int hdu_sweep_accumulate(int dtype, const void* logits, int64_t ldl, int64_t plane, int win_planes, int z, int num,
                         const int32_t* starts, int nwin, const int32_t* cursor, float* score, float* count, void* stream);
int hdu_sweep_advance(int32_t* cursor, int nwin, void* stream);

#define HDU_ZERO_BLOCK_BYTES 65536
typedef struct hdu_zero_entry {
  void* ptr;
  uint64_t bytes;
  uint32_t block_begin;
  uint32_t pad_;
  const void* src;
// ... 52 lines not shown
```

Before: 537.1.

## Fuse pointwise-conv input gradient and bias column sums into BN backward

```diff
diff --git a/h-denseunet_amd/csrc/rowops.hip b/h-denseunet_amd/csrc/rowops.hip
--- a/h-denseunet_amd/csrc/rowops.hip
+++ b/h-denseunet_amd/csrc/rowops.hip
@@ -143,10 +143,39 @@
   const float* rstd;
   float* partial;
   int slots;
+  const void* pw_w;
+  int pw_K;
 };
 
-template <typename T, int MODE, int COLS>
+template <typename T, int CH>
+__device__ __forceinline__ void pw_load_filter(const void* w, int c0, int K, bool active, float (&wk)[4][CH]) {
+  const T* __restrict__ wp = (const T*)w;
+#pragma unroll
+  for (int j = 0; j < CH; ++j) {
+    float t[CH];
+    Chunk<T>::unpack(*(const u32x4*)(wp + (long long)(active ? c0 + j : 0) * CH), t);
+#pragma unroll
+    for (int k = 0; k < 4; ++k) wk[k][j] = k < K ? t[k] : 0.f;
+  }
+}
+template <typename T, int CH>
+__device__ __forceinline__ u32x4 pw_dz_chunk(const u32x4& dyv, const float (&wk)[4][CH], int K) {
+  float d[CH], g[CH];
+  Chunk<T>::unpack(dyv, d);
+#pragma unroll
+  for (int j = 0; j < CH; ++j) {
+    float acc = 0.f;
+#pragma unroll
+    for (int k = 0; k < 4; ++k)
+      if (k < K) acc += d[k] * wk[k][j];
+    g[j] = acc;
+  }
+  return Chunk<T>::pack(g);
+}
+
+template <typename T, int MODE, int COLS, bool PW = false>
 __global__ __launch_bounds__(256) void reduce_rows_kernel(RedK p) {
+  static_assert(!PW || MODE == RED_BNBWD, "PW: the BN-backward sums only");
   constexpr int CH = Chunk<T>::CH;
   constexpr int ROWS = 256 / COLS;
   __shared__ float red[2][ROWS][COLS * CH];
@@ -161,7 +190,10 @@
   float s1[CH], s2[CH], k0[CH], k1[CH], k2[CH], k3[CH];
 #pragma unroll
   for (int j = 0; j < CH; ++j) { s1[j] = 0.f; s2[j] = 0.f; k0[j] = 0.f; k1[j] = 0.f; k2[j] = 0.f; k3[j] = 0.f; }
+  float wk[PW ? 4 : 1][CH];
+  const long long gc0 = PW ? 0 : c0;
   if (active) {
+    if constexpr (PW) pw_load_filter<T, CH>(p.pw_w, c0, p.pw_K, true, wk);
     if (MODE == RED_STATS) {
       Chunk<T>::unpack(*(const u32x4*)(xp + c0), k0);
     } else if (MODE == RED_BNBWD) {
@@ -181,7 +213,8 @@
         for (int j = 0; j < CH; ++j) { const float d = f[j] - k0[j]; s1[j] += d; s2[j] += d * d; }
       } else if (MODE == RED_BNBWD) {
         float g[CH];
-        Chunk<T>::unpack(gv, g);
+        if constexpr (PW) Chunk<T>::unpack(pw_dz_chunk<T, CH>(gv, wk, p.pw_K), g);
+        else Chunk<T>::unpack(gv, g);
 #pragma unroll
         for (int j = 0; j < CH; ++j) {
           const float s = k0[j] * f[j] + k1[j];
@@ -201,7 +234,7 @@
       for (int u = 0; u < ROW_UNROLL; ++u) xv[u] = *(const u32x4*)(xp + (r + u * ROWS) * p.ldx + c0);
       if (MODE == RED_BNBWD) {
 #pragma unroll
-        for (int u = 0; u < ROW_UNROLL; ++u) gv[u] = *(const u32x4*)(dzp + (r + u * ROWS) * p.lddz + c0);
+        for (int u = 0; u < ROW_UNROLL; ++u) gv[u] = *(const u32x4*)(dzp + (r + u * ROWS) * p.lddz + gc0);
       }
       HDU_SCHED_BARRIER();
 #pragma unroll
@@ -209,7 +242,7 @@
     }
     for (; r < r_end; r += ROWS) {
       u32x4 gv = u32x4{0u, 0u, 0u, 0u};
-      if (MODE == RED_BNBWD) gv = *(const u32x4*)(dzp + r * p.lddz + c0);
+      if (MODE == RED_BNBWD) gv = *(const u32x4*)(dzp + r * p.lddz + gc0);
       body(*(const u32x4*)(xp + r * p.ldx + c0), gv);
     }
   }
@@ -301,6 +334,17 @@
     case 8: HDU_LAUNCH((reduce_rows_kernel<T, MODE, 8>), dim3(gx, gy), dim3(256), 0, s, k); break;
     case 16: HDU_LAUNCH((reduce_rows_kernel<T, MODE, 16>), dim3(gx, gy), dim3(256), 0, s, k); break;
     default: HDU_LAUNCH((reduce_rows_kernel<T, MODE, 32>), dim3(gx, gy), dim3(256), 0, s, k); break;
+  }
+  return 0;
+}
+
+template <typename T>
+static int run_reduce_pw(RedK k, int cols, unsigned gx, unsigned gy, hipStream_t s) {
+  switch (cols) {
+    case 4: HDU_LAUNCH((reduce_rows_kernel<T, RED_BNBWD, 4, true>), dim3(gx, gy), dim3(256), 0, s, k); break;
+    case 8: HDU_LAUNCH((reduce_rows_kernel<T, RED_BNBWD, 8, true>), dim3(gx, gy), dim3(256), 0, s, k); break;
+    case 16: HDU_LAUNCH((reduce_rows_kernel<T, RED_BNBWD, 16, true>), dim3(gx, gy), dim3(256), 0, s, k); break;
+    default: HDU_LAUNCH((reduce_rows_kernel<T, RED_BNBWD, 32, true>), dim3(gx, gy), dim3(256), 0, s, k); break;
   }
   return 0;
 }
@@ -555,6 +599,31 @@
   return hdu_check_launch("bn_bwd_finalize_batched");
 }
 
+__global__ __launch_bounds__(256) void colsum_fold_batched_kernel(const hdu_colsum_entry* __restrict__ table,
+                                                                  const unsigned* __restrict__ begins, int n) {
+  __shared__ double red[2][4][8];
+  int lo = 0, hi = n - 1;
+  while (lo < hi) {
+    const int mid = (lo + hi + 1) >> 1;
+    if (begins[mid] <= blockIdx.x) lo = mid; else hi = mid - 1;
+  }
+  const hdu_colsum_entry e = table[lo];
+  const int cl = threadIdx.x & 7, pl = threadIdx.x >> 3;
+  const int c = (int)(blockIdx.x - begins[lo]) * 8 + cl;
+  double a1 = 0.0, a2 = 0.0;
+  if (c < e.C)
+    for (int b = pl; b < e.slots; b += 32) a1 += (double)e.partial[(long long)b * e.C + c];
+  fin_reduce32(a1, a2, red);
+  if (pl == 0 && c < e.C) e.out[c] = (float)a1;
+}
+
+extern "C" int hdu_colsum_fold_batched(const hdu_colsum_entry* table, const uint32_t* begins, int n, uint32_t total_blocks,
+                                       void* stream) {
+  if (!table || !begins || n <= 0 || total_blocks == 0) return hdu_set_error(HDU_ERR_ARG, "colsum_fold_batched: bad args");
+  HDU_LAUNCH(colsum_fold_batched_kernel, dim3(total_blocks), dim3(256), 0, (hipStream_t)stream, table, begins, n);
+  return hdu_check_launch("colsum_fold_batched");
+}
+
 __global__ __launch_bounds__(256) void bn_bwd_coef_kernel(int C, float invM, int batch_stats, const float* s1,
                                                           const float* s2, const float* gamma, const float* beta,
                                                           const float* sgamma, const float* rstd, float* k1,
@@ -642,6 +711,10 @@
   float invM;
   const float* gamma; const float* beta; const float* sgamma; const float* rstd;
   float* dgamma; float* dbeta; float* dsgamma; float* dsbeta;
+  const void* pw_w;
+  int pw_K;
+  float* csum;
+  int csum_slots;
 };
 
 template <int CH, int COLS>
@@ -727,8 +800,9 @@
   for (; m < r_end; m += ROWS) body(m, *(const u32x4*)(xp + m * p.ldx + c0));
 }
 
-template <typename T, int COLS, bool SUMS = false, bool PRE = false>
+template <typename T, int COLS, bool SUMS = false, bool PRE = false, bool PW = false, bool CSUM = false>
 __global__ __launch_bounds__(256) void bn_bwd_apply_kernel(RowK p) {
+  static_assert(!(PW || CSUM) || (SUMS && !PRE), "PW / CSUM: forms of the SUMS launch without the rows-first prologue");
   constexpr int CH = Chunk<T>::CH;
   constexpr int ROWS = 256 / COLS;
   const int cc = threadIdx.x % COLS, rl = threadIdx.x / COLS;
@@ -775,7 +849,8 @@
     float T1[CH], T2[CH], S1[CH], S2[CH];
     slot_loads<CH, COLS>(p.sums, p.slots, p.C, cq, active, rl, T1, T2);
     slot_reduce<CH, COLS>(p.slots, cc, rl, T1, T2, S1, S2);
-    if (!active) return;
+    if constexpr (CSUM) { if (!active) r_end = m; }
+    else if (!active) return;
 #pragma unroll
     for (int j = 0; j < CH; ++j) {
       const float kk = sg[j] * g[j] * rs[j];
@@ -784,7 +859,7 @@
       k3[j] = p.batch_stats ? kk * rs[j] * S2[j] * p.invM : 0.f;
       k4[j] = k3[j] * mu[j] - k2;
     }
-    if (blockIdx.x == 0 && rl == 0) {
+    if (blockIdx.x == 0 && rl == 0 && active) {
 #pragma unroll
       for (int j = 0; j < CH; ++j) {
         const int c = c0 + j;
@@ -802,10 +877,18 @@
       k4[j] = p.k3[c] * p.mean[c] - p.k2[c];
     }
   }
+  float wk[PW ? 4 : 1][CH], cs[CSUM ? CH : 1];
+  if constexpr (PW) pw_load_filter<T, CH>(p.pw_w, c0, p.pw_K, active, wk);
+  if constexpr (CSUM) {
+#pragma unroll
+    for (int j = 0; j < CH; ++j) cs[j] = 0.f;
+  }
+  const long long gc0 = PW ? 0 : c0;
   auto body = [&](long long m, const u32x4& xv, const u32x4& gv, const u32x4& ov) {
     float f[CH], g[CH], o[CH];
     Chunk<T>::unpack(xv, f);
-    Chunk<T>::unpack(gv, g);
+    if constexpr (PW) Chunk<T>::unpack(pw_dz_chunk<T, CH>(gv, wk, p.pw_K), g);
+    else Chunk<T>::unpack(gv, g);
 #pragma unroll
     for (int j = 0; j < CH; ++j) {
       const float s = a[j] * f[j] + b[j];
@@ -823,7 +906,14 @@
 #pragma unroll
       for (int j = 0; j < CH; ++j) o[j] += old[j];
     }
-    *(u32x4*)(op + m * p.ldo + c0) = Chunk<T>::pack(o);
+    const u32x4 stored = Chunk<T>::pack(o);
+    *(u32x4*)(op + m * p.ldo + c0) = stored;
+    if constexpr (CSUM) {
+      float sv[CH];
+      Chunk<T>::unpack(stored, sv);
+#pragma unroll
+      for (int j = 0; j < CH; ++j) cs[j] += sv[j];
+    }
   };
   if constexpr (PRE) {
 #pragma unroll
@@ -836,7 +926,7 @@
 #pragma unroll
     for (int u = 0; u < ROW_UNROLL; ++u) xv[u] = *(const u32x4*)(xp + (m + u * ROWS) * p.ldx + c0);
 #pragma unroll
-    for (int u = 0; u < ROW_UNROLL; ++u) gv[u] = *(const u32x4*)(dzp + (m + u * ROWS) * p.lddz + c0);
+    for (int u = 0; u < ROW_UNROLL; ++u) gv[u] = *(const u32x4*)(dzp + (m + u * ROWS) * p.lddz + gc0);
 #pragma unroll
     for (int u = 0; u < ROW_UNROLL; ++u) ov[u] = p.accumulate ? *(const u32x4*)(op + (m + u * ROWS) * p.ldo + c0) : z4;
     HDU_SCHED_BARRIER();
@@ -844,8 +934,23 @@
     for (int u = 0; u < ROW_UNROLL; ++u) body(m + u * ROWS, xv[u], gv[u], ov[u]);
   }
   for (; m < r_end; m += ROWS)
-    body(m, *(const u32x4*)(xp + m * p.ldx + c0), *(const u32x4*)(dzp + m * p.lddz + c0),
+    body(m, *(const u32x4*)(xp + m * p.ldx + c0), *(const u32x4*)(dzp + m * p.lddz + gc0),
          p.accumulate ? *(const u32x4*)(op + m * p.ldo + c0) : z4);
+  if constexpr (CSUM) {
+    __shared__ float cred[ROWS][COLS * CH];
+#pragma unroll
+    for (int j = 0; j < CH; ++j) cred[rl][cc * CH + j] = cs[j];
+    __syncthreads();
+    for (int col = threadIdx.x; col < COLS * CH; col += 256) {
+      const int c = blockIdx.y * COLS * CH + col;
+      if (c < p.C) {
+        float t = 0.f;
+#pragma unroll 4
+        for (int r = 0; r < ROWS; ++r) t += cred[r][col];
+        atomicAdd(p.csum + (long long)(blockIdx.x % (unsigned)p.csum_slots) * p.C + c, t);
+      }
+    }
+  }
 }
 
 template <typename T, int COLS>
@@ -1295,9 +1400,14 @@
                              int batch_stats, const float* gamma, const float* beta, const float* sgamma, float* sums,
                              int slots, float* dgamma, float* dbeta, float* dsgamma, float* dsbeta, void* dx,
                              int64_t lddx, int accumulate, float drop_keep, uint32_t drop_seed,
-                             const uint32_t* drop_seed_dev, void* stream) {
+                             const uint32_t* drop_seed_dev, void* stream, float* csum, int csum_slots,
+                             const void* pw_w = nullptr, int pw_K = 0) {
+  const bool pw = pw_w != nullptr;
   if (!dz || !x || !a || !b || !mean || !rstd || !sums || !dx) return hdu_set_error(HDU_ERR_ARG, "bn_bwd_fused: null pointer");
   if (slots <= 0 || slots > 32) return hdu_set_error(HDU_ERR_ARG, "bn_bwd_fused: 1 <= slots <= 32");
+  if (csum && (csum_slots <= 0 || ((uintptr_t)csum & 3))) return hdu_set_error(HDU_ERR_ARG, "bn_bwd_fused: column-sum table needs slots >= 1");
+  if (pw && (pw_K < 1 || pw_K > 4 || (((uintptr_t)pw_w | (uintptr_t)dz) & 15)))
+    return hdu_set_error(HDU_ERR_ARG, "bn_bwd_fused_pw: 1 <= K <= 4, dy and the filter 16-byte aligned");
   if (((uintptr_t)sums | (uintptr_t)a | (uintptr_t)b | (uintptr_t)mean | (uintptr_t)rstd | (uintptr_t)gamma | (uintptr_t)beta |
        (uintptr_t)sgamma) & 15)
     return hdu_set_error(HDU_ERR_ARG, "bn_bwd_fused: per-channel vectors must be 16-byte aligned");
@@ -1313,21 +1423,25 @@
   k.sums = sums; k.slots = slots; k.batch_stats = batch_stats; k.invM = 1.0f / (float)M;
   k.gamma = gamma; k.beta = beta; k.sgamma = sgamma; k.rstd = rstd;
   k.dgamma = dgamma; k.dbeta = dbeta; k.dsgamma = dsgamma; k.dsbeta = dsbeta;
+  k.pw_w = pw_w; k.pw_K = pw_K; k.csum = csum; k.csum_slots = csum_slots;
   if (int e = rowk_check(dtype, k, "bn_bwd_fused: C / strides must be multiples of the 16-byte chunk")) return e;
   if (M == 0) return 0;
   if (reduce) {
     RedK r{};
     r.x = x; r.ldx = ldx; r.dz = dz; r.lddz = lddz; r.M = M; r.C = C;
     r.a = a; r.b = b; r.mean = mean; r.rstd = rstd; r.relu = relu;
-    r.partial = sums; r.slots = slots;
+    r.partial = sums; r.slots = slots; r.pw_w = pw_w; r.pw_K = pw_K;
     int rcols; unsigned rgx, rgy;
     red_geometry(dtype, M, C, &rcols, &rgx, &rgy, &r.rows_per_block);
-    if (dtype == HDU_BF16) run_reduce<bf16_t, RED_BNBWD>(r, rcols, rgx, rgy, (hipStream_t)stream);
+    if (pw) {
+      if (dtype == HDU_BF16) run_reduce_pw<bf16_t>(r, rcols, rgx, rgy, (hipStream_t)stream);
+      else run_reduce_pw<float>(r, rcols, rgx, rgy, (hipStream_t)stream);
+    } else if (dtype == HDU_BF16) run_reduce<bf16_t, RED_BNBWD>(r, rcols, rgx, rgy, (hipStream_t)stream);
     else run_reduce<float, RED_BNBWD>(r, rcols, rgx, rgy, (hipStream_t)stream);
   }
   int cols; unsigned gx, gy;
   row_geometry(dtype, M, C, &cols, &gx, &gy, &k.rows_per_block);
-  const bool pre = k.rows_per_block <= (long long)ROW_UNROLL * (256 / cols) && !(g_tuning[HDU_TUNE_DEBUG] & 2048);
+  const bool pre = k.rows_per_block <= (long long)ROW_UNROLL * (256 / cols) && !(g_tuning[HDU_TUNE_DEBUG] & 2048) && !pw && !csum;
 #define HDU_APPLY_SUMS(T, PRE)                                                                                                    \
   switch (cols) {                                                                                                                 \
     case 4: HDU_LAUNCH((bn_bwd_apply_kernel<T, 4, true, PRE>), dim3(gx, gy), dim3(256), 0, (hipStream_t)stream, k); break;        \
@@ -1335,10 +1449,24 @@
     case 16: HDU_LAUNCH((bn_bwd_apply_kernel<T, 16, true, PRE>), dim3(gx, gy), dim3(256), 0, (hipStream_t)stream, k); break;      \
     default: HDU_LAUNCH((bn_bwd_apply_kernel<T, 32, true, PRE>), dim3(gx, gy), dim3(256), 0, (hipStream_t)stream, k); break;      \
   }
-  if (dtype == HDU_BF16) { if (pre) { HDU_APPLY_SUMS(bf16_t, true) } else { HDU_APPLY_SUMS(bf16_t, false) } }
+#define HDU_APPLY_FORM(T, PW, CSUM)                                                                                                        \
+  switch (cols) {                                                                                                                         \
+    case 4: HDU_LAUNCH((bn_bwd_apply_kernel<T, 4, true, false, PW, CSUM>), dim3(gx, gy), dim3(256), 0, (hipStream_t)stream, k); break;    \
+    case 8: HDU_LAUNCH((bn_bwd_apply_kernel<T, 8, true, false, PW, CSUM>), dim3(gx, gy), dim3(256), 0, (hipStream_t)stream, k); break;    \
+    case 16: HDU_LAUNCH((bn_bwd_apply_kernel<T, 16, true, false, PW, CSUM>), dim3(gx, gy), dim3(256), 0, (hipStream_t)stream, k); break;  \
+    default: HDU_LAUNCH((bn_bwd_apply_kernel<T, 32, true, false, PW, CSUM>), dim3(gx, gy), dim3(256), 0, (hipStream_t)stream, k); break;  \
+  }
+  if (pw || csum) {
+    if (dtype == HDU_BF16) {
+      if (pw && csum) { HDU_APPLY_FORM(bf16_t, true, true) } else if (pw) { HDU_APPLY_FORM(bf16_t, true, false) } else { HDU_APPLY_FORM(bf16_t, false, true) }
+    } else {
+      if (pw && csum) { HDU_APPLY_FORM(float, true, true) } else if (pw) { HDU_APPLY_FORM(float, true, false) } else { HDU_APPLY_FORM(float, false, true) }
+    }
+  } else if (dtype == HDU_BF16) { if (pre) { HDU_APPLY_SUMS(bf16_t, true) } else { HDU_APPLY_SUMS(bf16_t, false) } }
   else { if (pre) { HDU_APPLY_SUMS(float, true) } else { HDU_APPLY_SUMS(float, false) } }
+#undef HDU_APPLY_FORM
 #undef HDU_APPLY_SUMS
-  return hdu_check_launch("bn_bwd_fused");
+  return hdu_check_launch(pw ? "bn_bwd_fused_pw" : "bn_bwd_fused");
 }
 
 extern "C" int hdu_bn_bwd_fused(int dtype, const void* dz, int64_t lddz, const void* x, int64_t ldx, int64_t M, int C,
@@ -1346,9 +1474,22 @@
                                 int batch_stats, const float* gamma, const float* beta, const float* sgamma, float* sums,
                                 int slots, float* dgamma, float* dbeta, float* dsgamma, float* dsbeta, void* dx,
                                 int64_t lddx, int accumulate, float drop_keep, uint32_t drop_seed,
-                                const uint32_t* drop_seed_dev, void* stream) {
+                                const uint32_t* drop_seed_dev, void* stream, float* colsum, int colsum_slots) {
   return bn_bwd_fused_impl(true, dtype, dz, lddz, x, ldx, M, C, a, b, relu, mean, rstd, batch_stats, gamma, beta, sgamma, sums, slots,
-                           dgamma, dbeta, dsgamma, dsbeta, dx, lddx, accumulate, drop_keep, drop_seed, drop_seed_dev, stream);
+                           dgamma, dbeta, dsgamma, dsbeta, dx, lddx, accumulate, drop_keep, drop_seed, drop_seed_dev, stream, colsum,
+                           colsum_slots);
+}
+
+extern "C" int hdu_bn_bwd_fused_pw(int dtype, const void* dy, int64_t lddy, const void* w, int K, const void* x, int64_t ldx, int64_t M,
+                                   int C, const float* a, const float* b, int relu, const float* mean, const float* rstd,
+                                   int batch_stats, const float* gamma, const float* beta, const float* sgamma, float* sums,
+                                   int slots, float* dgamma, float* dbeta, float* dsgamma, float* dsbeta, void* dx, int64_t lddx,
+                                   int accumulate, float drop_keep, uint32_t drop_seed, const uint32_t* drop_seed_dev, void* stream,
+                                   float* colsum, int colsum_slots) {
+  if (!w) return hdu_set_error(HDU_ERR_ARG, "bn_bwd_fused_pw: null filter");
+  return bn_bwd_fused_impl(true, dtype, dy, lddy, x, ldx, M, C, a, b, relu, mean, rstd, batch_stats, gamma, beta, sgamma, sums, slots,
+                           dgamma, dbeta, dsgamma, dsbeta, dx, lddx, accumulate, drop_keep, drop_seed, drop_seed_dev, stream, colsum,
+                           colsum_slots, w, K);
 }
 
 extern "C" int hdu_bn_bwd_apply_sums(int dtype, const void* dz, int64_t lddz, const void* x, int64_t ldx, int64_t M, int C,
@@ -1356,9 +1497,10 @@
                                      int batch_stats, const float* gamma, const float* beta, const float* sgamma, float* sums,
                                      int slots, float* dgamma, float* dbeta, float* dsgamma, float* dsbeta, void* dx,
                                      int64_t lddx, int accumulate, float drop_keep, uint32_t drop_seed,
-                                     const uint32_t* drop_seed_dev, void* stream) {
+                                     const uint32_t* drop_seed_dev, void* stream, float* colsum, int colsum_slots) {
   return bn_bwd_fused_impl(false, dtype, dz, lddz, x, ldx, M, C, a, b, relu, mean, rstd, batch_stats, gamma, beta, sgamma, sums, slots,
-                           dgamma, dbeta, dsgamma, dsbeta, dx, lddx, accumulate, drop_keep, drop_seed, drop_seed_dev, stream);
+                           dgamma, dbeta, dsgamma, dsbeta, dx, lddx, accumulate, drop_keep, drop_seed, drop_seed_dev, stream, colsum,
+                           colsum_slots);
 }
 
 extern "C" int hdu_bn_bwd_correct(int dtype, const void* u, int64_t ldu, int64_t M, int C, const float* corr3,
diff --git a/h-denseunet_amd/engine.py b/h-denseunet_amd/engine.py
--- a/h-denseunet_amd/engine.py
+++ b/h-denseunet_amd/engine.py
@@ -44,6 +44,9 @@
             self.needs_grad = False
             self.drop = None
             self.corr_off = None
+            self.n_writes = 0
+            self.bias_sink = None
+            self.csum_pass = -1
         self.C = act.C
 
     def slab(self, c0, C):
@@ -89,6 +92,7 @@
             if self.C != r.act.ld:
                 self.ctx.zero_partial_grad(r.grad_act.buf)
         r.written = True
+        r.n_writes = r.n_writes + 1 if acc else 1
         return acc
 
     def stats(self):
@@ -149,6 +153,9 @@
         self.fuse_bn_bwd = self.fuse_bn_bwd_mode > 0
         self.fuse_bn_bwd_pw = os.environ.get("HDU_FUSE_BN_BWD_PW", "1") == "1"
         self.bnb_sums_epilogue = os.environ.get("HDU_BNB_SUMS_EPILOGUE", "1") == "1"
+        self.head_dz_fused = os.environ.get("HDU_HEAD_DZ_FUSED", "1") == "1"
+        self.bias_sums_in_apply = os.environ.get("HDU_BIAS_SUMS_IN_APPLY", "1") == "1"
+        self._csum_deferred, self._csum_plan = [], None
         self.fuse_bn_bwd_now = False
         self.bnb_sinks = []
         self.bnb_acc = None
@@ -256,13 +263,22 @@
                 if bn.mode == "batch" or bn.any_trainable():
                     bsum_off[bn] = n_bsum
                     n_bsum += bn.BSUM_SLOTS * 2 * bn.C
+        n_csum = 0
+        csum_off = {}
+        if self.bias_sums_in_apply and n_bsum and (self.shard is None or self.shard.world == 1):
+            for cv in self.convs:
+                if cv.trainable and cv.bias is not None and cv.out.root is cv.out and cv.out.root.needs_grad \
+                        and cv.out.C == cv.out.act.ld:
+                    csum_off[cv] = n_csum
+                    n_csum += cv.CSUM_SLOTS * cv.cout_p
         up4 = lambda n: (n + 3) // 4 * 4
         o_loss, n_loss = 0, 4 * max(1, len(self.loss_layers))
         o_stats = o_loss + n_loss
         o_bnb = o_stats + up4(n_stats)
         o_corr = o_bnb + up4(n_bnb)
         o_bsum = o_corr + up4(self._corr_total)
-        total = o_bsum + up4(n_bsum)
+        o_csum = o_bsum + up4(n_bsum)
+        total = o_csum + up4(n_csum)
         self.arena = torch.zeros(total, dtype=torch.float32, device=self.dev)
         for i, ll in enumerate(self.loss_layers):
             ll.loss_sum = self.arena[4 * i:4 * i + 1]
@@ -272,6 +288,9 @@
         self.corr_acc = self.arena[o_corr:o_corr + self._corr_total] if self._corr_total else None
         for bn, o in bsum_off.items():
             bn.bsum = self.arena[o_bsum + o:o_bsum + o + bn.BSUM_SLOTS * 2 * bn.C]
+        for cv, o in csum_off.items():
+            cv.csum = self.arena[o_csum + o:o_csum + o + cv.CSUM_SLOTS * cv.cout_p]
+            cv.out.root.bias_sink = cv
         self._shift_copies = [(r.shift, r.mean) for r in self.stat_roots] if self.stats_sinks else []
         self._zp_arena = ops.ZeroPlan([self.arena], self._shift_copies)
         self._zp_bwd = ops.ZeroPlan([self.arena[o_bnb:total]]) if total > o_bnb else None
@@ -528,6 +547,7 @@
         order = list(reversed(self.bwd))
         if lo == 0:
             self._bnb_deferred = []
+            self._csum_deferred = []
             self._split_now = self.split_wgrad_active()
             if self._split_now and self._split_plan is None:
                 self._build_split_wgrad_plan()
@@ -543,6 +563,11 @@
                 if self._bnb_plan is None or self._bnb_plan[0] != keys:
                     self._bnb_plan = (keys, ops.BnBwdPlan([e for _, e in self._bnb_deferred]))
                 self._bnb_plan[1].run()
+            if hi == len(self.bwd) and self._csum_deferred:
+                keys = tuple(k for k, _ in self._csum_deferred)
+                if self._csum_plan is None or self._csum_plan[0] != keys:
+                    self._csum_plan = (keys, ops.ColsumPlan([e for _, e in self._csum_deferred]))
+                self._csum_plan[1].run()
             if hi == len(self.bwd) and self.wgrad_plan is not None:
                 self.wgrad_plan.run()
             if hi == len(self.bwd) and self._split_now:
@@ -649,9 +674,10 @@
                     and self.bsum is not None and xvar.root.needs_grad and ctx._zeroed_bwd_pass == ctx.pass_id
                     and self._bsum_pass != ctx.pass_id)
 
-    def backward(self, xvar, dz_act, sums_ready=False):
+    def backward(self, xvar, dz_act, sums_ready=False, pw=None):
         ctx = self.ctx
         x = xvar.act
+        assert pw is None or self.takes_epilogue_sums(xvar)
         need_sums = self.batch_now or self.any_trainable()
         tr_bn = self.trainable
         tr_sc = self.sg is not None and self.scale_trainable
@@ -673,12 +699,17 @@
             self._bsum_pass = ctx.pass_id
             acc = xvar.grad_mode()
             drop = xvar.root.drop if (ctx.dropout_enabled and ctx.learning_phase == 1) else None
+            r, sink, csum = xvar.root, xvar.root.bias_sink, None
+            if (sink is not None and ctx.bias_sums_in_apply and ctx.batch_wgrad and not acc and xvar.c0 == 0 and xvar.C == r.act.ld
+                    and not (r.corr_off is not None and ctx.corr_acc is not None and ctx.fuse_bn_bwd_now)):
+                csum = sink.csum
+                r.csum_pass = ctx.pass_id
             ops.bn_bwd_fused(dz_act, x, self.a, self.b, self.relu, self.mean_used, self.rstd, self.batch_now,
                              self.gamma.data, self.beta.data, self.sg.data if self.sg else None, self.bsum, self.BSUM_SLOTS,
                              self.gamma.grad if tr_bn else None, self.beta.grad if tr_bn else None,
                              self.sg.grad if tr_sc else None, self.sb.grad if tr_sc else None, xvar.grad, acc,
                              drop[0] if drop else 1.0, drop[1] if drop else 0, ctx.seed_dev if drop else None,
-                             sums_ready=sums_ready)
+                             sums_ready=sums_ready, colsum=csum, colsum_slots=sink.CSUM_SLOTS if csum is not None else 0, pw=pw)
             return
         elif need_sums:
             assert not sums_ready
@@ -732,6 +763,8 @@
         ctx.layer_kind[name] = "conv"
         self.T = K[0] * K[1] * K[2]
         self.cin_p, self.cout_p = cin_p, cout_p
+        self.filters = filters
+        self.csum = None
         self.dropout = dropout
         if dropout > 0:
             ctx.drop_layers += 1
@@ -902,7 +935,7 @@
         x = self.x.act
         if self.trainable and (getattr(self, "in_plan", False) or (ctx._split_now and getattr(self, "in_split_plan", False))):
             if self.bias is not None:
-                ops.colsum(dy, self.bias.grad, ctx.ws)
+                self._bias_grad(dy)
         elif self.trainable:
             if self.xin is not None:
                 d = ctx.conv_desc(self.xin.act, self.wf_ptr, dy, self.K, self.stride, self.pad, self.conv_up)
@@ -913,7 +946,7 @@
                                   self.bn.relu if self.bn is not None else False)
             ops.conv_wgrad(d, self.kernel.grad)
             if self.bias is not None:
-                ops.colsum(dy, self.bias.grad, ctx.ws)
+                self._bias_grad(dy)
         if not self.need_input_grad:
             return
         K, pad = self.K, self.pad
@@ -921,6 +954,8 @@
             return self._backward_halo(dy)
         if self.bnb_fused and ctx.fuse_bn_bwd_now:
             return self._backward_fused_bn(dy)
+        if self._head_dz_fused():
+            return self.bn.backward(self.x, dy, pw=(self.wd_ptr, self.filters))
         De, He, We = x.D << self.up[0], x.H << self.up[1], x.W << self.up[2]
         direct = self.bn is None and self.up == (0, 0, 0)
         sums_ready = False
@@ -959,6 +994,21 @@
             self.bn.backward(self.x, dz, sums_ready=sums_ready)
         else:
             ops.upsample_bwd(dz, self.x.grad, (0, 0, 0), accumulate=self.x.grad_mode())
+
+    def _bias_grad(self, dy):
+        ctx, r = self.ctx, self.out.root
+        if self.csum is not None and r.csum_pass == ctx.pass_id and r.n_writes == 1:
+            ctx._csum_deferred.append((id(self), (self.csum, self.CSUM_SLOTS, self.cout_p, self.bias.grad)))
+        else:
+            ops.colsum(dy, self.bias.grad, ctx.ws)
+
+    def _head_dz_fused(self):
+        ctx, bn = self.ctx, self.bn
+        return bool(ctx.head_dz_fused and bn is not None and self.K == (1, 1, 1) and self.stride == (1, 1, 1)
+                    and self.pad == (0, 0, 0) and self.up == (0, 0, 0) and self.skip is None and not self.halo
+                    and self.cout_p == ops.CHUNK[ctx.dtype] and self.filters <= 4 and self.wd_ptr is not None
+                    and self.wd_ptr.value % 16 == 0 and self.out.grad.ptr.value % 16 == 0
+                    and not (ctx.shard is not None and ctx.shard.world > 1) and bn.takes_epilogue_sums(self.x))
 
     def _epilogue_sums(self, d):
         ctx, bn = self.ctx, self.bn
@@ -1029,6 +1079,7 @@
 
 
 ConvLayer._backward_fused_bn = _conv_backward_fused_bn
+ConvLayer.CSUM_SLOTS = int(os.environ.get("HDU_CSUM_SLOTS", "16"))
 ConvLayer.BNB_SLOTS = int(os.environ.get("HDU_BNB_SLOTS", "16"))
 
 
diff --git a/h-denseunet_amd/lib.py b/h-denseunet_amd/lib.py
--- a/h-denseunet_amd/lib.py
+++ b/h-denseunet_amd/lib.py
@@ -64,6 +64,10 @@
 class BnBwdEntry(ctypes.Structure):
     _fields_ = [("partial", c_p), ("slots", ctypes.c_int32), ("C", ctypes.c_int32), ("gamma", c_p), ("beta", c_p),
                 ("sgamma", c_p), ("dgamma", c_p), ("dbeta", c_p), ("dsgamma", c_p), ("dsbeta", c_p)]
+
+
+class ColsumEntry(ctypes.Structure):
+    _fields_ = [("partial", c_p), ("out", c_p), ("slots", ctypes.c_int32), ("C", ctypes.c_int32)]
 
 
 class BnStatsFold(ctypes.Structure):
@@ -129,9 +133,12 @@
     "hdu_bn_bwd_apply": (c_int, [c_int, c_p, c_i64, c_p, c_i64, c_i64, c_int, c_p, c_p, c_int, c_p, c_p, c_p, c_p,
                                  c_p, c_i64, c_int, c_f, c_u32, c_p, c_p]),
     "hdu_bn_bwd_fused": (c_int, [c_int, c_p, c_i64, c_p, c_i64, c_i64, c_int, c_p, c_p, c_int, c_p, c_p, c_int, c_p, c_p,
-                                 c_p, c_p, c_int, c_p, c_p, c_p, c_p, c_p, c_i64, c_int, c_f, c_u32, c_p, c_p]),
+                                 c_p, c_p, c_int, c_p, c_p, c_p, c_p, c_p, c_i64, c_int, c_f, c_u32, c_p, c_p, c_p, c_int]),
     "hdu_bn_bwd_apply_sums": (c_int, [c_int, c_p, c_i64, c_p, c_i64, c_i64, c_int, c_p, c_p, c_int, c_p, c_p, c_int, c_p, c_p,
-                                      c_p, c_p, c_int, c_p, c_p, c_p, c_p, c_p, c_i64, c_int, c_f, c_u32, c_p, c_p]),
+                                      c_p, c_p, c_int, c_p, c_p, c_p, c_p, c_p, c_i64, c_int, c_f, c_u32, c_p, c_p, c_p, c_int]),
+    "hdu_bn_bwd_fused_pw": (c_int, [c_int, c_p, c_i64, c_p, c_int, c_p, c_i64, c_i64, c_int, c_p, c_p, c_int, c_p, c_p, c_int, c_p,
+                                    c_p, c_p, c_p, c_int, c_p, c_p, c_p, c_p, c_p, c_i64, c_int, c_f, c_u32, c_p, c_p, c_p, c_int]),
+    "hdu_colsum_fold_batched": (c_int, [c_p, c_p, c_int, c_u32, c_p]),
     "hdu_affine_act": (c_int, [c_int, c_p, c_i64, c_i64, c_int, c_p, c_p, c_int, c_p, c_i64, c_p]),
     "hdu_materialize": (c_int, [c_int, c_p, c_i64, c_int, c_int, c_int, c_int, c_int, c_p, c_p, c_int, c_int, c_int, c_int,
                                 c_p, c_i64, c_p, c_i64, c_p]),
@@ -201,7 +208,7 @@
     pass
 
 
-ABI_VERSION = 9
+ABI_VERSION = 10
 
 
 def product_library_path():
diff --git a/h-denseunet_amd/ops.py b/h-denseunet_amd/ops.py
--- a/h-denseunet_amd/ops.py
+++ b/h-denseunet_amd/ops.py
@@ -471,14 +471,43 @@
 
 
 def bn_bwd_fused(dz, x, a, b, relu, mean, rstd, batch_stats, gamma, beta, sgamma, sums, slots, dgamma, dbeta, dsgamma,
-                 dsbeta, dx, accumulate=False, drop_keep=1.0, drop_seed=0, drop_seed_dev=None, sums_ready=False):
+                 dsbeta, dx, accumulate=False, drop_keep=1.0, drop_seed=0, drop_seed_dev=None, sums_ready=False, colsum=None,
+                 colsum_slots=0, pw=None):
+    tail = (fptr(a), fptr(b), 1 if relu else 0,
+            fptr(mean), fptr(rstd), 1 if batch_stats else 0, fptr(gamma), fptr(beta), fptr(sgamma),
+            fptr(sums), slots, fptr(dgamma), fptr(dbeta), fptr(dsgamma), fptr(dsbeta), dx.ptr, dx.ld,
+            1 if accumulate else 0, drop_keep, drop_seed,
+            ctypes.c_void_p(drop_seed_dev.data_ptr()) if drop_seed_dev is not None else None,
+            stream(), fptr(colsum), colsum_slots if colsum is not None else 0)
+    if pw is not None:
+        assert not sums_ready and dz.C == CHUNK[x.dtype] and dz.M == x.M
+        check(_l.get().hdu_bn_bwd_fused_pw(x.dtype, dz.ptr, dz.ld, pw[0], pw[1], x.ptr, x.ld, x.M, x.C, *tail), "hdu_bn_bwd_fused_pw")
+        return
     fn = _l.get().hdu_bn_bwd_apply_sums if sums_ready else _l.get().hdu_bn_bwd_fused
-    check(fn(x.dtype, dz.ptr, dz.ld, x.ptr, x.ld, x.M, x.C, fptr(a), fptr(b), 1 if relu else 0,
-             fptr(mean), fptr(rstd), 1 if batch_stats else 0, fptr(gamma), fptr(beta), fptr(sgamma),
-             fptr(sums), slots, fptr(dgamma), fptr(dbeta), fptr(dsgamma), fptr(dsbeta), dx.ptr, dx.ld,
-             1 if accumulate else 0, drop_keep, drop_seed,
-             ctypes.c_void_p(drop_seed_dev.data_ptr()) if drop_seed_dev is not None else None,
-             stream()), "hdu_bn_bwd_fused")
+    check(fn(x.dtype, dz.ptr, dz.ld, x.ptr, x.ld, x.M, x.C, *tail), "hdu_bn_bwd_fused")
+
+
+class ColsumPlan:
+
+    def __init__(self, entries):
+        import numpy as np
+        self.keep = entries
+        n = len(entries)
+        tab = (_l.ColsumEntry * n)()
+        begins = np.zeros(n, dtype=np.uint32)
+        tot = 0
+        for i, (part, slots, C, out) in enumerate(entries):
+            assert part.numel() == slots * C and out.numel() >= C
+            tab[i] = _l.ColsumEntry(part.data_ptr(), out.data_ptr(), slots, C)
+            begins[i] = tot
+            tot += (C + 7) // 8
+        self.n, self.total = n, tot
+        self.table = torch.from_numpy(np.frombuffer(bytes(tab), dtype=np.uint8).copy()).to(device())
+        self.begins = torch.from_numpy(begins.view(np.int32)).to(device())
+
+    def run(self):
+        check(_l.get().hdu_colsum_fold_batched(ctypes.c_void_p(self.table.data_ptr()), ctypes.c_void_p(self.begins.data_ptr()),
+                                               self.n, self.total, stream()), "hdu_colsum_fold_batched")
 
 
 def bn_bwd_finalize(partial, slots, M, C, batch_stats, gamma, beta, sgamma, mean, rstd, dgamma, dbeta, dsgamma, dsbeta,
diff --git a/include/hdu.h b/include/hdu.h
--- a/include/hdu.h
+++ b/include/hdu.h
@@ -18,7 +18,7 @@
 
 const char* hdu_last_error(void);
 const char* hdu_backend(void);
-#define HDU_ABI_VERSION 9
+#define HDU_ABI_VERSION 10
 int hdu_abi_version(void);
 size_t hdu_sizeof_conv_desc(void);
 int hdu_profile_begin(int max_records);
@@ -101,6 +101,13 @@
 } hdu_bnbwd_entry;
 int hdu_bn_bwd_finalize_batched(const hdu_bnbwd_entry* table, const uint32_t* begins, int n, uint32_t total_blocks, void* stream);
 
+typedef struct hdu_colsum_entry {
+  const float* partial;
+  float* out;
+  int32_t slots, C;
+} hdu_colsum_entry;
+int hdu_colsum_fold_batched(const hdu_colsum_entry* table, const uint32_t* begins, int n, uint32_t total_blocks, void* stream);
+
 int hdu_bn_bwd_correct(int dtype, const void* u, int64_t ldu, int64_t M, int C, const float* corr3, const float* corr4,
                        void* du, int64_t lddu, void* stream);
 int hdu_bn_bwd_finalize_correct(int dtype, const float* partial, int slots, int64_t M, int C, const float* gamma, const float* beta,
@@ -194,13 +201,19 @@
                      const float* b, int relu, const float* mean, const float* rstd, int batch_stats, const float* gamma,
                      const float* beta, const float* sgamma, float* sums, int slots, float* dgamma, float* dbeta,
                      float* dsgamma, float* dsbeta, void* dx, int64_t lddx, int accumulate, float drop_keep,
-                     uint32_t drop_seed, const uint32_t* drop_seed_dev, void* stream);
+                     uint32_t drop_seed, const uint32_t* drop_seed_dev, void* stream, float* colsum, int colsum_slots);
+
+int hdu_bn_bwd_fused_pw(int dtype, const void* dy, int64_t lddy, const void* w, int K, const void* x, int64_t ldx, int64_t M, int C,
+                        const float* a, const float* b, int relu, const float* mean, const float* rstd, int batch_stats,
+                        const float* gamma, const float* beta, const float* sgamma, float* sums, int slots, float* dgamma,
+                        float* dbeta, float* dsgamma, float* dsbeta, void* dx, int64_t lddx, int accumulate, float drop_keep,
+                        uint32_t drop_seed, const uint32_t* drop_seed_dev, void* stream, float* colsum, int colsum_slots);
 
 int hdu_bn_bwd_apply_sums(int dtype, const void* dz, int64_t lddz, const void* x, int64_t ldx, int64_t M, int C, const float* a,
                           const float* b, int relu, const float* mean, const float* rstd, int batch_stats, const float* gamma,
                           const float* beta, const float* sgamma, float* sums, int slots, float* dgamma, float* dbeta,
                           float* dsgamma, float* dsbeta, void* dx, int64_t lddx, int accumulate, float drop_keep,
-                          uint32_t drop_seed, const uint32_t* drop_seed_dev, void* stream);
+                          uint32_t drop_seed, const uint32_t* drop_seed_dev, void* stream, float* colsum, int colsum_slots);
 
 int hdu_affine_act(int dtype, const void* x, int64_t ldx, int64_t M, int C, const float* a, const float* b,
                    int relu, void* z, int64_t ldz, void* stream);
```

After: 543.8 (median of 6 runs). 1.01x the previous value.
